# Tencent/PocketFlow

Hardware: AMD Instinct MI355X
Metric: images/sec ResNet-50 INT8 quant-aware fine-tune (whole job; per GPU = value / n_gpus) (higher is better)
Workload: dtype bf16

## Files before the change

include/pocketflow_hip.h:

```cpp
#ifndef POCKETFLOW_HIP_H_
#define POCKETFLOW_HIP_H_

#include <stdint.h>

#ifdef __cplusplus
extern "C" {
#endif

enum { PF_F32 = 0, PF_BF16 = 1 };
enum { PF_ACT_NONE = 0, PF_ACT_RELU = 1, PF_ACT_RELU6 = 2 };
enum { PF_BUCKET_TENSOR = 0, PF_BUCKET_CHANNEL = 1, PF_BUCKET_SPLIT = 2 };

typedef struct PfSeg {
  int64_t offset;
  int64_t len;
  int32_t RS;
  int32_t layout;
  int32_t I, O;
  int32_t mode;
  int32_t bits;
  int32_t bucket_size;
  int32_t n_bucket;
  int64_t slot_offset;
  int64_t cb_offset;
} PfSeg;

typedef struct PfBlock { int32_t seg; int32_t chunk; int32_t row0; int32_t nrows; } PfBlock;

#define PF_CHUNK 4096

const char* pf_error_string(int err);
int pf_version(void);
int pf_tuning_reload(void);

int pf_minmax_slots_init(uint32_t* slots, int64_t n_pairs, void* stream);
int pf_minmax_tensor(const void* x, int64_t n, int dtype, int act, uint32_t* slot, void* stream);
int pf_minmax_decode(const uint32_t* slots, int64_t n_pairs, float* alpha_beta, void* stream);

int pf_uq_apply(const void* x, void* y, int64_t n, int in_dtype, int out_dtype, int act,
                const uint32_t* slot, int bits, void* stream);
int pf_act_grad(const void* g, const void* u, void* dx, int64_t n, int dtype, int act,
                void* stream);

int pf_seg_minmax(const float* w_flat, const PfSeg* segs, const PfBlock* blocks, int n_blocks,
                  uint32_t* slots, void* stream);
int pf_seg_uq_apply(const float* w_flat, void* qw_flat, int out_dtype, const PfSeg* segs,
                    const PfBlock* blocks, int n_blocks, const uint32_t* slots, void* stream);

int pf_seg_nuq_apply(const float* w_flat, void* qw_flat, int out_dtype, uint8_t* idx_flat,
                     const float* codebooks, const PfSeg* segs, const PfBlock* blocks,
                     int n_blocks, const uint32_t* slots, void* stream);
int pf_seg_nuq_codebook_grad(const void* g_flat, int g_dtype, const uint8_t* idx_flat,
                             float* dcodebooks, int64_t* acc_ws, int64_t n_codebook, const PfSeg* segs,
                             const PfBlock* blocks, int n_blocks, const uint32_t* slots, void* stream);
int pf_seg_normalize(const float* w_flat, float* xn_out, const PfSeg* segs, int seg_index,
                     const uint32_t* slots, void* stream);

int pf_ws_bkup_merge_abs(const float* var, float* bkup, const float* mask, float* abs_out,
                         int64_t n, void* stream);
int pf_kth_largest_nonneg(const float* a, int64_t n, int64_t k_desc_index, float* out,
                          uint32_t* workspace, void* stream);
int pf_ws_mask_apply(float* var, const float* bkup, float* mask, const float* thr, int64_t n,
                     void* stream);
int pf_count_nonzero(const float* x, int64_t n, unsigned long long* out, void* stream);

int pf_cp_build_mask(float* mask, const uint8_t* keep_in, const uint8_t* keep_out, int O, int RS,
                     int I, void* stream);
int pf_cp_mask_grad(float* g, const uint8_t* keep_in, const uint8_t* keep_out, int O, int RS,
                    int I, void* stream);

int pf_adam_flat(float* p, const void* g, int g_dtype, float* m, float* v, const float* mask,
                 int64_t n, int64_t n_decay, float wd, float g_scale, float lr, float beta1,
                 float beta2, float eps, float beta1_power, float beta2_power, void* stream);
int pf_momentum_flat(float* p, const void* g, int g_dtype, float* acc, const float* mask,
                     int64_t n, int64_t n_decay, float wd, float g_scale, float lr, float momentum,
                     void* stream);
int pf_adam_flat_dev(float* p, const void* g, int g_dtype, float* m, float* v, const float* mask,
                     int64_t n, int64_t n_decay, float wd, float g_scale, const float* hp, float beta1,
                     float beta2, float eps, void* stream);
int pf_momentum_flat_dev(float* p, const void* g, int g_dtype, float* acc, const float* mask,
                         int64_t n, int64_t n_decay, float wd, float g_scale, const float* hp,
                         float momentum, void* stream);
int pf_set_floats(float* dst, float a, float b, float c, float d, void* stream);

int pf_ce_distill_fwd_bwd(const void* z_s, int zs_dtype, const float* labels, const void* z_t,
                          int zt_dtype, int B, int C, float tempr, float loss_w, float* losses,
                          void* dz_s, int dz_dtype, float* row_ws, void* stream);

int pf_bn_stats(const void* x, int dtype, int64_t rows, int C, float* partial ,
                int n_blocks, void* stream);
int pf_bn_finalize(const float* partial, int n_blocks, int64_t rows, int C, const void* x_row0,
                   int dtype, const float* gamma, const float* beta, float* moving_mean,
                   float* moving_var, float momentum, float eps, int training ,
                   int act, float* scale_shift , float* mean_invstd ,
                   uint32_t* slot , void* stream);
int pf_bn_act_quant_apply(const void* x, void* q, int dtype, int64_t rows, int C,
                          const float* scale_shift, int act, const uint32_t* slot, int bits,
                          int quantize, void* stream);
int pf_bn_bwd_stats(const void* dq, const void* x, int dtype, int64_t rows, int C,
                    const float* scale_shift, const float* mean_invstd, int act,
                    float* partial , int n_blocks, void* stream);
int pf_bn_bwd_finalize(const float* partial, int n_blocks, int C, float* dgamma, float* dbeta,
                       void* stream);
int pf_bn_bwd_apply(const void* dq, const void* x, void* dx, int dtype, int64_t rows, int C,
                    const float* scale_shift, const float* mean_invstd,
                    const float* dgamma, const float* dbeta, int act, void* stream);
int pf_bn_bwd_apply_add(const void* dq, const void* x, const void* addend, void* dx, int dtype,
                        int64_t rows, int C, const float* scale_shift, const float* mean_invstd,
                        const float* dgamma, const float* dbeta, int act, void* stream);
int pf_bn_eval_scale_shift(const float* gamma, const float* beta, const float* moving_mean,
                           const float* moving_var, float eps, int C, float* scale_shift,
                           void* stream);

int pf_conv1x1_stats_groups_k(int M, int N, int K, int prologue);
int pf_conv1x1_fwd(const void* X, const void* W, void* Y, const void* R, const float* scale_shift,
                   int act, const uint32_t* slot, int bits, float* partial, int M, int N, int K,
                   int Ho, int Wo, int H, int Wd, int stride, int ymap, void* stream);
int pf_conv1x1_fwd_affine(const void* X, const void* W, void* Y, const float* scale_shift, int act,
                          const float* out_scale_shift, int out_act, int M, int N, int K, int Ho, int Wo, int H, int Wd,
                          int stride, void* stream);
int pf_conv1x1_bwd_data_bnstats(const void* dY, const void* Wt, void* dQ, const void* bn_x,
                                const float* bn_scale_shift, const float* bn_mean_invstd, int bn_act,
                                float* partial, int M, int N, int K, void* stream);
int pf_conv1x1_join_plan(int M, int N, int K, int with_stats);
int pf_conv1x1_bwd_data_join(const void* dY, const void* Wt, void* dQ, const void* R, int r_Ho, int r_Wo, int r_H, int r_W,
                             int r_stride, const void* bn_x, const float* bn_scale_shift, const float* bn_mean_invstd,
                             int bn_act, float* partial, int M, int N, int K, void* stream);
int pf_conv1x1_wrw_splits(int M, int N, int K);
int pf_conv1x1_wrw(const void* dY, const void* X, void* dW, int dw_dtype, float* workspace,
                   const float* scale_shift, int act, const uint32_t* slot, int bits, int M, int N,
                   int K, int Ho, int Wo, int H, int Wd, int stride, void* stream);

int pf_conv2d_stats_groups_geom(int imgs, int H, int Wd, int C, int N, int th, int tw, int stride, int pad_h, int pad_w,
                                int Ho, int Wo);
int pf_conv2d_fwd(const void* X, const void* W, void* Y, const void* zero, const void* R, float* partial,
                  const void* bn_x, const float* bn_scale_shift, const float* bn_mean_invstd, int bn_act,
                  int imgs, int H, int Wd, int C, int N, int th, int tw, int stride, int pad_h, int pad_w,
                  int Ho, int Wo, void* stream);
int pf_conv2d_fwd_affine(const void* X, const void* W, void* Y, const void* zero, const float* out_scale_shift, int out_act,
                         int imgs, int H, int Wd, int C, int N, int th, int tw, int stride, int pad_h, int pad_w, int Ho, int Wo,
                         void* stream);

int pf_conv2d_wrw_splits(int M, int N, int C, int taps);
int pf_conv2d_wrw(const void* dY, const void* X, void* dW, int dw_dtype, float* workspace, int imgs, int H, int Wd, int C,
                  int N, int th, int tw, int stride, int pad_h, int pad_w, int Ho, int Wo, void* stream);

typedef struct PfTransposeTile {
  int64_t src_off, dst_off;
  int32_t O, I, src_ld, dst_ld;
  int32_t o0, i0;
  int32_t reserved0, reserved1;
} PfTransposeTile;
int pf_seg_transpose(const void* src_flat, void* dst_flat, int dtype, const void* tiles, int n_tiles, void* stream);

int pf_maxpool_fwd(const void* x, void* y, void* idx, int dtype, int B, int H, int W, int C, int k, int stride,
                   int pad_h, int pad_w, int Ho, int Wo, void* stream);
int pf_maxpool_bwd(const void* dy, const void* idx, void* dx, int dtype, int B, int H, int W, int C, int k, int stride,
                   int pad_h, int pad_w, int Ho, int Wo, void* stream);

int pf_conv_stem_supported(int H, int Wd, int C, int N, int k, int stride, int pad);
int pf_conv_stem_fwd(const void* X, const void* W, void* Y, int imgs, int H, int Wd, void* stream);
int pf_conv_stem_wrw_slabs(int imgs, int H, int Wd);
int pf_conv_stem_wrw(const void* dY, const void* X, void* dW, int dw_dtype, float* workspace, int imgs, int H, int Wd,
                     void* stream);

int pf_conv_stem3_supported(int H, int Wd, int C, int N, int k, int stride, int pad_h, int pad_w, int Ho, int Wo);
int pf_conv_stem3_fwd(const void* X, const void* W, void* Y, int imgs, int H, int Wd, int N, int pad_h, int pad_w, int Ho, int Wo,
                      void* stream);
int pf_conv_stem3_wrw_slabs(int imgs, int H, int Wd, int N, int pad_h, int pad_w, int Ho, int Wo);
int pf_conv_stem3_wrw(const void* dY, const void* X, void* dW, int dw_dtype, float* workspace, int imgs, int H, int Wd, int N,
                      int pad_h, int pad_w, int Ho, int Wo, void* stream);

int pf_depthwise_supported(int C, int k, int stride);
int pf_depthwise_groups(int B, int Ho, int Wo, int C);
int pf_depthwise_fwd(const void* X, const void* W, void* Y, int dtype, float* partial, int B, int H, int Wd, int C, int k,
                     int stride, int pad_h, int pad_w, int Ho, int Wo, void* stream);
int pf_depthwise_bwd_data(const void* dY, const void* W, void* dX, int dtype, int B, int H, int Wd, int C, int k,
                          int stride, int pad_h, int pad_w, int Ho, int Wo, void* stream);
int pf_depthwise_wrw(const void* dY, const void* X, void* dW, int dtype, int dw_dtype, float* slabs, int B, int H, int Wd,
                     int C, int k, int stride, int pad_h, int pad_w, int Ho, int Wo, void* stream);

typedef struct PfImageDesc {
  int64_t offset;
  int32_t h, w;
  float scale_y, scale_x;
  int32_t off_y, off_x;
  int32_t flip;
  int32_t reserved;
} PfImageDesc;
int pf_image_resize_bilinear(const void* src, const PfImageDesc* desc, void* out, int out_dtype, int B, int OH,
                             int OW, float mean_r, float mean_g, float mean_b, void* stream);

int pf_conv2d_bwd_data_strided(const void* dY, const void* Wt, void* dX, const void* zero, int imgs, int H, int Wd, int C, int N,
                               int R, int S, int stride, int pad_h, int pad_w, int Ho, int Wo, void* stream);
int pf_conv2d_bwd_data_strided_stats_groups(int imgs, int H, int Wd, int C, int stride);
int pf_conv2d_bwd_data_strided_bnstats(const void* dY, const void* Wt, void* dX, const void* zero, const void* bn_x,
                                       const float* bn_scale_shift, const float* bn_mean_invstd, int bn_act, float* partial,
                                       int imgs, int H, int Wd, int C, int N, int R, int S, int stride, int pad_h, int pad_w,
                                       int Ho, int Wo, void* stream);

int pf_convg_small_splits(int M, int Nc, int K);
int pf_convg_fwd(const void* x, const void* w, const float* bias, void* y, int dtype, int imgs, int H, int W, int C, int N, int R,
                 int S, int stride, int pad_h, int pad_w, int Ho, int Wo, float* slab, int64_t slab_elems, void* stream);
int pf_convg_bwd_data(const void* dy, const void* w, void* dx, int dtype, int imgs, int H, int W, int C, int N, int R, int S,
                      int stride, int pad_h, int pad_w, int Ho, int Wo, float* slab, int64_t slab_elems, void* stream);
int pf_convg_wrw_splits(int imgs, int C, int N, int R, int S, int Ho, int Wo);
int pf_convg_wrw(const void* dy, const void* x, void* dw, int dtype, int dw_dtype, float* slab, int imgs, int H, int W, int C, int N,
                 int R, int S, int stride, int pad_h, int pad_w, int Ho, int Wo, void* stream);

int pf_conv_gather_fwd(const void* x, const void* w, const int32_t* gather, const float* bias, const void* res,
                       const float* scale_shift, int act, void* y, int dtype, int imgs, int H, int W, int C, int Ck, int N, int R,
                       int S, int stride, int pad_h, int pad_w, int Ho, int Wo, void* stream);

int pf_im2col(const void* x, void* xcol, int imgs, int H, int W, int C, int R, int S, int stride, int pad_h, int pad_w, int Ho, int Wo,
              void* stream);
int pf_col2im(const void* dxcol, void* dx, int imgs, int H, int W, int C, int R, int S, int stride, int pad_h, int pad_w, int Ho, int Wo,
              void* stream);

int pf_prox_groups(int64_t rows, int I);
int pf_prox_norms(const float* w, const void* g, int g_dtype, float lr, int64_t rows, int I, float* partial, float* norms, void* stream);
int pf_prox_apply(float* w, const void* g, int g_dtype, float lr, int64_t rows, int I, const float* norms, const float* thr, void* stream);

int pf_cpr_gather(const void* x, int x_dtype, const void* y, int y_dtype, const int* pos, int crops, int B, int H, int W, int C, int OH, int OW,
                  int Co, int kh, int kw, int stride, int pad_t, int pad_l, float* P, float* Y, int64_t row0, void* stream);
int64_t pf_cpr_gram_ws(int C);
int pf_cpr_gram(const float* P, const float* Y, const int* idx, int64_t n, int kk, int C, int Co, const float* w, double* ws, int64_t ws_elems,
                float* xtx, float* xty, void* stream);
int pf_cpr_ista(const float* A, const float* b, const float* m0, float* m_ws, float* mask, int C, float gamma, float lr, int iters, int* nnz,
                void* stream);
int pf_cpr_lstsq_splits(int64_t N, int Kp, int Co);
int pf_cpr_lstsq_step(const float* P, int K, const int* kidx, const int* pos, int Kp, const float* Y, float* R, int64_t N, int Co, float* W,
                      float* m, float* v, float* part, float wd, float lr_t, float beta1, float beta2, float c1, float c2, float eps,
                      void* stream);
int pf_cpr_lstsq_resid(const float* P, int K, const int* kidx, int Kp, const float* W, const float* Y, float* R, int64_t N, int Co,
                       void* stream);

#ifdef __cplusplus
}
#endif
#endif
```

pocketflow_amd/csrc/pf_optim.hip:

```cpp
#include "pf_common.h"

template <typename TG> __device__ __forceinline__ void load4g(const TG* p, float* g);
template <> __device__ __forceinline__ void load4g<float>(const float* p, float* g) {
  float4 v = *reinterpret_cast<const float4*>(p);
  g[0] = v.x; g[1] = v.y; g[2] = v.z; g[3] = v.w;
}
template <> __device__ __forceinline__ void load4g<bf16_t>(const bf16_t* p, float* g) {
  uint2 v = *reinterpret_cast<const uint2*>(p);
  g[0] = __uint_as_float(v.x << 16); g[1] = __uint_as_float(v.x & 0xFFFF0000u);
  g[2] = __uint_as_float(v.y << 16); g[3] = __uint_as_float(v.y & 0xFFFF0000u);
}

__device__ __forceinline__ float eff_grad(float g, float p, float mask, bool decay, float wd,
                                          float g_scale) {
  float ge = g * g_scale;
  if (decay) ge = ge + wd * p;
  return ge * mask;
}

template <typename TG, bool MASK>
__global__ __launch_bounds__(PF_THREADS) void k_adam_flat(float* __restrict__ p, const TG* __restrict__ g,
                                                          float* __restrict__ m, float* __restrict__ v,
                                                          const float* __restrict__ mask, int64_t n,
                                                          int64_t n_decay, float wd, float g_scale,
                                                          float alpha_t, float omb1, float omb2,
                                                          float eps, const float* __restrict__ hp) {
  if (hp != nullptr) alpha_t = hp[0];
  const int64_t nv = n >> 2;
  for (int64_t i = (int64_t)blockIdx.x * PF_THREADS + threadIdx.x; i < nv;
       i += (int64_t)gridDim.x * PF_THREADS) {
    const int64_t e = i << 2;
    float gg[4], mk[4] = {1.f, 1.f, 1.f, 1.f};
    load4g<TG>(g + e, gg);
    float4 pp = *reinterpret_cast<float4*>(p + e);
    float4 mm = *reinterpret_cast<float4*>(m + e);
    float4 vv = *reinterpret_cast<float4*>(v + e);
    if (MASK) { float4 t = *reinterpret_cast<const float4*>(mask + e); mk[0] = t.x; mk[1] = t.y; mk[2] = t.z; mk[3] = t.w; }
    float pa[4] = {pp.x, pp.y, pp.z, pp.w}, ma[4] = {mm.x, mm.y, mm.z, mm.w}, va[4] = {vv.x, vv.y, vv.z, vv.w};
#pragma unroll
    for (int j = 0; j < 4; ++j) {
      const float ge = eff_grad(gg[j], pa[j], mk[j], (e + j) < n_decay, wd, g_scale);
      ma[j] = ma[j] + (ge - ma[j]) * omb1;
      va[j] = va[j] + (ge * ge - va[j]) * omb2;
      pa[j] = pa[j] - (ma[j] * alpha_t) / (sqrtf(va[j]) + eps);
    }
    *reinterpret_cast<float4*>(p + e) = make_float4(pa[0], pa[1], pa[2], pa[3]);
    *reinterpret_cast<float4*>(m + e) = make_float4(ma[0], ma[1], ma[2], ma[3]);
    *reinterpret_cast<float4*>(v + e) = make_float4(va[0], va[1], va[2], va[3]);
  }
  if (blockIdx.x == 0) {
    for (int64_t e = (nv << 2) + threadIdx.x; e < n; e += PF_THREADS) {
      const float mk = MASK ? mask[e] : 1.0f;
      const float ge = eff_grad(load_one<TG>(g + e), p[e], mk, e < n_decay, wd, g_scale);
      const float mn = m[e] + (ge - m[e]) * omb1;
      const float vn = v[e] + (ge * ge - v[e]) * omb2;
      m[e] = mn; v[e] = vn;
      p[e] = p[e] - (mn * alpha_t) / (sqrtf(vn) + eps);
    }
  }
}

static int adam_launch(float* p, const void* g, int g_dtype, float* m, float* v,
                       const float* mask, int64_t n, int64_t n_decay, float wd, float g_scale,
                       float lr, float beta1, float beta2, float eps, float beta1_power,
                       float beta2_power, const float* hp, void* stream) {
  if (n <= 0) return 0;
  if (!pf_aligned16(p) || !pf_aligned16(g) || !pf_aligned16(m) || !pf_aligned16(v) ||
      (mask && !pf_aligned16(mask)))
    return (int)hipErrorInvalidValue;
  const float alpha_t = lr * sqrtf(1.0f - beta2_power) / (1.0f - beta1_power);
  const float omb1 = 1.0f - beta1, omb2 = 1.0f - beta2;
  hipStream_t st = (hipStream_t)stream;
  const int grid = pf_grid_for(n, PF_THREADS * 4);
#define PF_AD(TG, MK) k_adam_flat<TG, MK><<<grid, PF_THREADS, 0, st>>>(p, (const TG*)g, m, v, mask, n, n_decay, wd, g_scale, alpha_t, omb1, omb2, eps, hp)
  if (g_dtype == PF_F32) { if (mask) PF_AD(float, true); else PF_AD(float, false); }
  else if (g_dtype == PF_BF16) { if (mask) PF_AD(bf16_t, true); else PF_AD(bf16_t, false); }
  else return (int)hipErrorInvalidValue;
#undef PF_AD
  PF_LAUNCH_CHECK();
  return 0;
}

extern "C" int pf_adam_flat(float* p, const void* g, int g_dtype, float* m, float* v,
                            const float* mask, int64_t n, int64_t n_decay, float wd, float g_scale,
                            float lr, float beta1, float beta2, float eps, float beta1_power,
                            float beta2_power, void* stream) {
  return adam_launch(p, g, g_dtype, m, v, mask, n, n_decay, wd, g_scale, lr, beta1, beta2, eps, beta1_power, beta2_power, nullptr,
                     stream);
}

extern "C" int pf_adam_flat_dev(float* p, const void* g, int g_dtype, float* m, float* v,
                                const float* mask, int64_t n, int64_t n_decay, float wd, float g_scale,
                                const float* hp, float beta1, float beta2, float eps, void* stream) {
  if (hp == nullptr) return (int)hipErrorInvalidValue;
  return adam_launch(p, g, g_dtype, m, v, mask, n, n_decay, wd, g_scale, 0.f, beta1, beta2, eps, 0.5f, 0.5f, hp, stream);
}

template <typename TG, bool MASK>
__global__ __launch_bounds__(PF_THREADS) void k_momentum_flat(float* __restrict__ p, const TG* __restrict__ g,
                                                              float* __restrict__ acc,
                                                              const float* __restrict__ mask, int64_t n,
                                                              int64_t n_decay, float wd, float g_scale,
                                                              float lr, float mu, const float* __restrict__ hp) {
  if (hp != nullptr) lr = hp[1];
  const int64_t nv = n >> 2;
  for (int64_t i = (int64_t)blockIdx.x * PF_THREADS + threadIdx.x; i < nv;
       i += (int64_t)gridDim.x * PF_THREADS) {
    const int64_t e = i << 2;
    float gg[4], mk[4] = {1.f, 1.f, 1.f, 1.f};
    load4g<TG>(g + e, gg);
    float4 pp = *reinterpret_cast<float4*>(p + e);
    float4 aa = *reinterpret_cast<float4*>(acc + e);
    if (MASK) { float4 t = *reinterpret_cast<const float4*>(mask + e); mk[0] = t.x; mk[1] = t.y; mk[2] = t.z; mk[3] = t.w; }
    float pa[4] = {pp.x, pp.y, pp.z, pp.w}, ac[4] = {aa.x, aa.y, aa.z, aa.w};
#pragma unroll
    for (int j = 0; j < 4; ++j) {
      const float ge = eff_grad(gg[j], pa[j], mk[j], (e + j) < n_decay, wd, g_scale);
      ac[j] = mu * ac[j] + ge;
      pa[j] = pa[j] - lr * ac[j];
    }
    *reinterpret_cast<float4*>(p + e) = make_float4(pa[0], pa[1], pa[2], pa[3]);
    *reinterpret_cast<float4*>(acc + e) = make_float4(ac[0], ac[1], ac[2], ac[3]);
  }
  if (blockIdx.x == 0) {
    for (int64_t e = (nv << 2) + threadIdx.x; e < n; e += PF_THREADS) {
      const float mk = MASK ? mask[e] : 1.0f;
      const float ge = eff_grad(load_one<TG>(g + e), p[e], mk, e < n_decay, wd, g_scale);
      const float a = mu * acc[e] + ge;
      acc[e] = a;
      p[e] = p[e] - lr * a;
    }
  }
}

static int momentum_launch(float* p, const void* g, int g_dtype, float* acc, const float* mask,
                           int64_t n, int64_t n_decay, float wd, float g_scale, float lr,
                           float momentum, const float* hp, void* stream) {
  if (n <= 0) return 0;
  if (!pf_aligned16(p) || !pf_aligned16(g) || !pf_aligned16(acc) || (mask && !pf_aligned16(mask)))
    return (int)hipErrorInvalidValue;
  hipStream_t st = (hipStream_t)stream;
  const int grid = pf_grid_for(n, PF_THREADS * 4);
#define PF_MO(TG, MK) k_momentum_flat<TG, MK><<<grid, PF_THREADS, 0, st>>>(p, (const TG*)g, acc, mask, n, n_decay, wd, g_scale, lr, momentum, hp)
  if (g_dtype == PF_F32) { if (mask) PF_MO(float, true); else PF_MO(float, false); }
  else if (g_dtype == PF_BF16) { if (mask) PF_MO(bf16_t, true); else PF_MO(bf16_t, false); }
  else return (int)hipErrorInvalidValue;
#undef PF_MO
  PF_LAUNCH_CHECK();
  return 0;
}

extern "C" int pf_momentum_flat(float* p, const void* g, int g_dtype, float* acc, const float* mask,
                                int64_t n, int64_t n_decay, float wd, float g_scale, float lr,
                                float momentum, void* stream) {
  return momentum_launch(p, g, g_dtype, acc, mask, n, n_decay, wd, g_scale, lr, momentum, nullptr, stream);
}

extern "C" int pf_momentum_flat_dev(float* p, const void* g, int g_dtype, float* acc, const float* mask,
                                    int64_t n, int64_t n_decay, float wd, float g_scale, const float* hp,
                                    float momentum, void* stream) {
  if (hp == nullptr) return (int)hipErrorInvalidValue;
  return momentum_launch(p, g, g_dtype, acc, mask, n, n_decay, wd, g_scale, 0.f, momentum, hp, stream);
}

__global__ void k_set_floats(float* __restrict__ dst, float a, float b, float c, float d) {
  if (threadIdx.x == 0) { dst[0] = a; dst[1] = b; dst[2] = c; dst[3] = d; }
}

extern "C" int pf_set_floats(float* dst, float a, float b, float c, float d, void* stream) {
  if (dst == nullptr) return (int)hipErrorInvalidValue;
  k_set_floats<<<1, 64, 0, (hipStream_t)stream>>>(dst, a, b, c, d);
  PF_LAUNCH_CHECK();
  return 0;
}
```

pocketflow_amd/csrc/pf_stem.hip:

```cpp
#include "pf_conv_common.h"

#define LDS_PTR(p) ((__attribute__((address_space(3))) void*)(p))
typedef short st_v4s __attribute__((ext_vector_type(4)));
typedef short st_v8s __attribute__((ext_vector_type(8)));
#if defined(__HIP_DEVICE_COMPILE__)
typedef __amdgpu_buffer_rsrc_t st_rsrc_t;
#define ST_MAKE_RSRC(p, bytes) __builtin_amdgcn_make_buffer_rsrc((void*)(p), (short)0, (int)(bytes), 0x00020000)
#define ST_BUFFER_LOAD_LDS16(rs, lds, voff) __builtin_amdgcn_raw_ptr_buffer_load_lds(rs, LDS_PTR(lds), 16, voff, 0, 0, 0)
#else
typedef int st_rsrc_t;
#define ST_MAKE_RSRC(p, bytes) 0
#define ST_BUFFER_LOAD_LDS16(rs, lds, voff) ((void)(rs), (void)(lds), (void)(voff))
#endif

#define ST_THREADS 256
#define ST_OROWS 8
#define ST_IROWS (2 * ST_OROWS + 5)
#define ST_N 64
#define ST_R 7
#define ST_WL_BYTES (ST_N * ST_R * 32 * 2)

struct StemArgs {
  const bf16_t* X;
  const bf16_t* W;
  bf16_t* Y;
  int imgs, H, Wd, Ho, Wo;
  int strips, n_items;
  int rsb;
};

__global__ __launch_bounds__(ST_THREADS) void k_stem7x7_fwd(StemArgs a) {
  extern __shared__ __attribute__((aligned(16))) unsigned char smem[];
  unsigned char* wl = smem;
  unsigned char* xs = smem + ST_WL_BYTES;
  const int tid = threadIdx.x, lane = tid & 63, wave = __builtin_amdgcn_readfirstlane(tid >> 6);
  const int l16 = lane & 15, g = lane >> 4;

  for (int ch = tid; ch < ST_N * ST_R * 4; ch += ST_THREADS) {
    const int q = ch & 3, nr = ch >> 2;
    const bf16_t* src = a.W + ((int64_t)nr * 7 + 2 * q) * 3;
    uint32_t v[4];
    const uint32_t e0 = src[0], e1 = src[1], e2 = src[2];
    v[0] = e0 | (e1 << 16); v[1] = e2;
    if (q < 3) {
      const uint32_t f0 = src[3], f1 = src[4], f2 = src[5];
      v[2] = f0 | (f1 << 16); v[3] = f2;
    } else {
      v[2] = 0u; v[3] = 0u;
    }
    *reinterpret_cast<uint4*>(wl + ((int64_t)nr * 32 + q * 8) * 2) = make_uint4(v[0], v[1], v[2], v[3]);
  }
  for (int t = tid; t < ST_IROWS * 8; t += ST_THREADS) {
    const int row = t >> 3, h = t & 7;
    const int pp = h < 3 ? h : a.Wd + h;
    *reinterpret_cast<uint2*>(xs + (int64_t)row * a.rsb + pp * 8) = make_uint2(0u, 0u);
  }
  __syncthreads();
  bf16x8 wf[4][ST_R];
#pragma unroll
  for (int nb = 0; nb < 4; ++nb) {
    const int n = 16 * (l16 >> 2) + 4 * nb + (l16 & 3);
#pragma unroll
    for (int r = 0; r < ST_R; ++r)
      wf[nb][r] = *reinterpret_cast<const bf16x8*>(wl + ((n * ST_R + r) * 32 + g * 8) * 2);
  }

  const int pairs = a.Wd >> 1;
  const int pblocks = a.Wo >> 4;
  const int units = ST_OROWS * pblocks;
  for (int item = blockIdx.x; item < a.n_items; item += gridDim.x) {
    const int img = item / a.strips, strip = item - img * a.strips;
    const int oy0 = strip * ST_OROWS, iy0 = 2 * oy0 - 3;
    __syncthreads();
    for (int row = tid >> 7; row < ST_IROWS; row += 2) {
      const int iy = iy0 + row;
      unsigned char* dst = xs + (int64_t)row * a.rsb + 3 * 8;
      const bool live = iy >= 0 && iy < a.H;
      const uint32_t* src = reinterpret_cast<const uint32_t*>(a.X + ((int64_t)img * a.H + (live ? iy : 0)) * a.Wd * 3);
      for (int j = tid & 127; j < pairs; j += 128) {
        uint32_t d0 = 0u, d1 = 0u, d2 = 0u;
        if (live) { d0 = src[3 * j]; d1 = src[3 * j + 1]; d2 = src[3 * j + 2]; }
        *reinterpret_cast<uint2*>(dst + j * 16) = make_uint2(d0, d1 & 0xFFFFu);
        *reinterpret_cast<uint2*>(dst + j * 16 + 8) = make_uint2((d1 >> 16) | (d2 << 16), d2 >> 16);
      }
    }
    __syncthreads();
    for (int u = wave; u < units; u += ST_THREADS / 64) {
      const int orow = u / pblocks, pb = u - orow * pblocks;
      const int oy = oy0 + orow;
      if (oy >= a.Ho) continue;
      const int ox = pb * 16 + l16;
      const unsigned char* base = xs + (int64_t)(2 * orow) * a.rsb + (2 * ox + 2 * g) * 8;
      f32x4 acc[4];
#pragma unroll
      for (int nb = 0; nb < 4; ++nb) acc[nb] = f32x4{0.f, 0.f, 0.f, 0.f};
#pragma unroll
      for (int r = 0; r < ST_R; ++r) {
        const bf16x8 xf = *reinterpret_cast<const bf16x8*>(base + (int64_t)r * a.rsb);
#pragma unroll
        for (int nb = 0; nb < 4; ++nb)
          acc[nb] = __builtin_amdgcn_mfma_f32_16x16x32_bf16(wf[nb][r], xf, acc[nb], 0, 0, 0);
      }
      bf16_t* out = a.Y + (((int64_t)img * a.Ho + oy) * a.Wo + ox) * ST_N + 16 * g;
      const uint4 lo = make_uint4(pack_bf16x2(acc[0][0], acc[0][1]), pack_bf16x2(acc[0][2], acc[0][3]),
                                  pack_bf16x2(acc[1][0], acc[1][1]), pack_bf16x2(acc[1][2], acc[1][3]));
      const uint4 hi = make_uint4(pack_bf16x2(acc[2][0], acc[2][1]), pack_bf16x2(acc[2][2], acc[2][3]),
                                  pack_bf16x2(acc[3][0], acc[3][1]), pack_bf16x2(acc[3][2], acc[3][3]));
      *reinterpret_cast<uint4*>(out) = lo;
      *reinterpret_cast<uint4*>(out + 8) = hi;
    }
  }
}

extern "C" int pf_conv_stem_supported(int H, int Wd, int C, int N, int k, int stride, int pad) {
  return (C == 3 && N == ST_N && k == 7 && stride == 2 && pad == 3 && H > 0 && (H % 2) == 0 && Wd >= 32 && (Wd % 32) == 0 &&
          Wd <= 1024) ? 1 : 0;
}

extern "C" int pf_conv_stem_fwd(const void* X, const void* W, void* Y, int imgs, int H, int Wd, void* stream) {
  if (!pf_conv_stem_supported(H, Wd, 3, ST_N, 7, 2, 3) || imgs <= 0) return (int)hipErrorInvalidValue;
  if (!pf_aligned16(Y) || (reinterpret_cast<uintptr_t>(X) & 3u) || (reinterpret_cast<uintptr_t>(W) & 1u))
    return (int)hipErrorInvalidValue;
  StemArgs a;
  a.X = (const bf16_t*)X; a.W = (const bf16_t*)W; a.Y = (bf16_t*)Y;
  a.imgs = imgs; a.H = H; a.Wd = Wd; a.Ho = H / 2; a.Wo = Wd / 2;
  a.strips = (a.Ho + ST_OROWS - 1) / ST_OROWS;
  a.n_items = imgs * a.strips;
  a.rsb = (Wd + 8) * 8;
  const size_t lds = (size_t)ST_WL_BYTES + (size_t)ST_IROWS * a.rsb;
  if (lds > 160 * 1024) return (int)hipErrorInvalidValue;
  if (int e = pf_require_lds(reinterpret_cast<const void*>(&k_stem7x7_fwd), lds)) return e;
  const int grid = a.n_items < 512 ? a.n_items : 512;
  k_stem7x7_fwd<<<grid, ST_THREADS, lds, (hipStream_t)stream>>>(a);
  PF_LAUNCH_CHECK();
  return 0;
}


struct StemWrwArgs {
  const bf16_t* dY;
  const bf16_t* X;
  float* slabs;
  int imgs, H, Wd, Ho, Wo;
  int strips, n_items;
  int rsb;
  int dy_bytes;
};

#define SW_OROWS 2
#define SW_IROWS (2 * SW_OROWS + 5)

__global__ __launch_bounds__(ST_THREADS) void k_stem7x7_wrw(StemWrwArgs a) {
  extern __shared__ __attribute__((aligned(16))) unsigned char smem[];
  unsigned char* xs = smem;
  unsigned char* dys = smem + SW_IROWS * a.rsb;
  const int tid = threadIdx.x, lane = tid & 63, wave = __builtin_amdgcn_readfirstlane(tid >> 6);
  const int l15 = lane & 15, q = lane >> 4;
  const int nb0 = 2 * (wave & 1);
  const int r0 = (wave >> 1) ? 4 : 0, nr = (wave >> 1) ? 3 : 4;
  const st_rsrc_t rsY = ST_MAKE_RSRC(a.dY, a.dy_bytes);
  constexpr uint32_t OOB = 0x80000000u;
  const int sb = lane >> 4, srow = (lane & 15) >> 1, sch = lane & 1;
  const int tr_off = (q & 1) * 128 + (l15 >> 2) * 32 + (l15 & 3) * 8;
  const int pg_lo = q >> 1;
  const int p_lo = 8 * pg_lo + 4 * (q & 1) + (l15 >> 2);
  const int steps = (SW_OROWS * a.Wo) >> 5;
  const int pairs = a.Wd >> 1;

  f32x4 acc[2][8];
#pragma unroll
  for (int i = 0; i < 2; ++i)
#pragma unroll
    for (int k = 0; k < 8; ++k) acc[i][k] = f32x4{0.f, 0.f, 0.f, 0.f};

  for (int t = tid; t < SW_IROWS * 8; t += ST_THREADS) {
    const int row = t >> 3, h = t & 7;
    const int pp = h < 3 ? h : a.Wd + h;
    *reinterpret_cast<uint2*>(xs + (int64_t)row * a.rsb + pp * 8) = make_uint2(0u, 0u);
  }

  for (int item = blockIdx.x; item < a.n_items; item += gridDim.x) {
    const int img = item / a.strips, strip = item - img * a.strips;
    const int oy0 = strip * SW_OROWS, iy0 = 2 * oy0 - 3;
    const int valid_px = ((a.Ho - oy0) < SW_OROWS ? (a.Ho - oy0) : SW_OROWS) * a.Wo;
    const int64_t m_base = ((int64_t)img * a.Ho + oy0) * a.Wo;
    __syncthreads();
    for (int id = wave; id < steps * 4; id += ST_THREADS / 64) {
      const int lin = id * 8 + srow;
      const uint32_t voff = (lin < valid_px) ? (uint32_t)(((m_base + lin) * ST_N + 16 * sb + 8 * sch) * 2) : OOB;
      ST_BUFFER_LOAD_LDS16(rsY, dys + id * 1024, voff);
    }
    for (int row = tid >> 7; row < SW_IROWS; row += 2) {
      const int iy = iy0 + row;
      unsigned char* dst = xs + (int64_t)row * a.rsb + 3 * 8;
      const bool live = iy >= 0 && iy < a.H;
      const uint32_t* src = reinterpret_cast<const uint32_t*>(a.X + ((int64_t)img * a.H + (live ? iy : 0)) * a.Wd * 3);
      for (int j = tid & 127; j < pairs; j += 128) {
        uint32_t d0 = 0u, d1 = 0u, d2 = 0u;
        if (live) { d0 = src[3 * j]; d1 = src[3 * j + 1]; d2 = src[3 * j + 2]; }
        *reinterpret_cast<uint2*>(dst + j * 16) = make_uint2(d0, d1 & 0xFFFFu);
        *reinterpret_cast<uint2*>(dst + j * 16 + 8) = make_uint2((d1 >> 16) | (d2 << 16), d2 >> 16);
      }
    }
    asm volatile("s_waitcnt vmcnt(0)" ::: "memory");
    __syncthreads();
    for (int st = 0; st < steps; ++st) {
      const unsigned char* dbase = dys + st * 4096;
      bf16x8 df[2];
#pragma unroll
      for (int i = 0; i < 2; ++i) {
        const st_v4s lo = __builtin_amdgcn_ds_read_tr16_b64_v4i16(
            (__attribute__((address_space(3))) st_v4s*)(dbase + (pg_lo * 4 + nb0 + i) * 256 + tr_off));
        const st_v4s hi = __builtin_amdgcn_ds_read_tr16_b64_v4i16(
            (__attribute__((address_space(3))) st_v4s*)(dbase + ((pg_lo + 2) * 4 + nb0 + i) * 256 + tr_off));
        st_v8s d8;
        d8[0] = lo[0]; d8[1] = lo[1]; d8[2] = lo[2]; d8[3] = lo[3];
        d8[4] = hi[0]; d8[5] = hi[1]; d8[6] = hi[2]; d8[7] = hi[3];
        df[i] = *reinterpret_cast<const bf16x8*>(&d8);
      }
      int lin = st * 32 + p_lo;
      int orow = lin >= a.Wo ? 1 : 0;
      const unsigned char* xlo = xs + (int64_t)(2 * orow + r0) * a.rsb + (2 * (lin - orow * a.Wo) + (l15 & 3)) * 8;
      lin += 16;
      orow = lin >= a.Wo ? 1 : 0;
      const unsigned char* xhi = xs + (int64_t)(2 * orow + r0) * a.rsb + (2 * (lin - orow * a.Wo) + (l15 & 3)) * 8;
#pragma unroll
      for (int rr = 0; rr < 4; ++rr) {
        if (rr < nr) {
#pragma unroll
          for (int h = 0; h < 2; ++h) {
            const st_v4s lo = __builtin_amdgcn_ds_read_tr16_b64_v4i16(
                (__attribute__((address_space(3))) st_v4s*)(xlo + (int64_t)rr * a.rsb + h * 32));
            const st_v4s hi = __builtin_amdgcn_ds_read_tr16_b64_v4i16(
                (__attribute__((address_space(3))) st_v4s*)(xhi + (int64_t)rr * a.rsb + h * 32));
            st_v8s x8;
            x8[0] = lo[0]; x8[1] = lo[1]; x8[2] = lo[2]; x8[3] = lo[3];
            x8[4] = hi[0]; x8[5] = hi[1]; x8[6] = hi[2]; x8[7] = hi[3];
            const bf16x8 xf = *reinterpret_cast<const bf16x8*>(&x8);
#pragma unroll
            for (int i = 0; i < 2; ++i)
              acc[i][rr * 2 + h] = __builtin_amdgcn_mfma_f32_16x16x32_bf16(df[i], xf, acc[i][rr * 2 + h], 0, 0, 0);
          }
        }
      }
    }
  }
  float* slab = a.slabs + (int64_t)blockIdx.x * (ST_N * 147);
  const int c = l15 & 3;
#pragma unroll
  for (int rr = 0; rr < 4; ++rr) {
    if (rr < nr) {
#pragma unroll
      for (int h = 0; h < 2; ++h) {
        const int s = 4 * h + (l15 >> 2);
        if (s < 7 && c < 3) {
#pragma unroll
          for (int i = 0; i < 2; ++i)
#pragma unroll
            for (int j = 0; j < 4; ++j)
              slab[(16 * (nb0 + i) + 4 * q + j) * 147 + ((r0 + rr) * 7 + s) * 3 + c] = acc[i][rr * 2 + h][j];
        }
      }
    }
  }
}

int pf_wrw_reduce(float* workspace, int S, int64_t n, void* dW, int dw_dtype, hipStream_t st);

static int stem_wrw_grid(int imgs, int H) {
  const int items = imgs * ((H / 2 + SW_OROWS - 1) / SW_OROWS);
  return items < 768 ? items : 768;
}

extern "C" int pf_conv_stem_wrw_slabs(int imgs, int H, int Wd) {
  if (!pf_conv_stem_supported(H, Wd, 3, ST_N, 7, 2, 3) || imgs <= 0 || Wd > 256) return 0;
  if ((int64_t)imgs * (H / 2) * (Wd / 2) * ST_N * 2 >= (int64_t)1 << 31) return 0;
  return stem_wrw_grid(imgs, H);
}

extern "C" int pf_conv_stem_wrw(const void* dY, const void* X, void* dW, int dw_dtype, float* workspace, int imgs, int H,
                                int Wd, void* stream) {
  const int S = pf_conv_stem_wrw_slabs(imgs, H, Wd);
  if (S <= 0 || workspace == nullptr) return (int)hipErrorInvalidValue;
  if (!pf_aligned16(dY) || (reinterpret_cast<uintptr_t>(X) & 3u)) return (int)hipErrorInvalidValue;
  StemWrwArgs a;
  a.dY = (const bf16_t*)dY; a.X = (const bf16_t*)X; a.slabs = workspace;
  a.imgs = imgs; a.H = H; a.Wd = Wd; a.Ho = H / 2; a.Wo = Wd / 2;
  a.strips = (a.Ho + SW_OROWS - 1) / SW_OROWS;
  a.n_items = imgs * a.strips;
  a.rsb = (Wd + 8) * 8;
  a.dy_bytes = (int)((int64_t)imgs * a.Ho * a.Wo * ST_N * 2);
  const size_t lds = (size_t)SW_IROWS * a.rsb + (size_t)SW_OROWS * a.Wo * ST_N * 2;
  if (int e = pf_require_lds(reinterpret_cast<const void*>(&k_stem7x7_wrw), lds)) return e;
  k_stem7x7_wrw<<<S, ST_THREADS, lds, (hipStream_t)stream>>>(a);
  PF_LAUNCH_CHECK();
  return pf_wrw_reduce(workspace, S, (int64_t)ST_N * 147, dW, dw_dtype, (hipStream_t)stream);
}
```

pocketflow_amd/graph.py:

```python
from __future__ import annotations

import contextlib
import math
import os
import weakref
import threading
from dataclasses import dataclass, field
from typing import Callable, Dict, List, Optional, Sequence, Tuple

import numpy as np
import torch
import torch.nn.functional as F

from pocketflow_amd import hip
from pocketflow_amd.hip import check_gather
from pocketflow_amd.plan import WeightDesc
from pocketflow_amd.profiling import region

ALIGN = 64
FUSE_BN_BWD_STATS = os.environ.get('PF_FUSE_BN_BWD_STATS', '1') != '0'


def _align(n: int) -> int:
  return (n + ALIGN - 1) // ALIGN * ALIGN
# ... 566 lines not shown


class LazyAct(object):

  def __init__(self, x, scale_shift, act, slot, bits, rows, C, mean_invstd=None):
    self.x, self.scale_shift, self.act, self.slot, self.bits = x, scale_shift, act, slot, bits
    self.rows, self.C = rows, C
    self.mean_invstd = mean_invstd
    self.n_consumers = 0
    self.bwd_stats = None
    self.n_grad_consumers = 0
    self.pending = None
    self.join_ok = False
    self.pending_geom = None
    self.dense_out = None
    self._q = None

  @property
  def shape(self):
    return self.x.shape

  @property
  def dtype(self):
    return self.x.dtype

  @property
  def device(self):
    return self.x.device

  def materialize(self) -> torch.Tensor:
    self.n_consumers += 2
    if self._q is None:
      self._q = _Materialize.apply(self.x, self)
    return self._q


def materialize(x):
  return x.materialize() if isinstance(x, LazyAct) else x


class _Materialize(torch.autograd.Function):
  @staticmethod
  def forward(ctx, x, lazy):
    q = torch.empty_like(x)
    quant = lazy.bits is not None
    hip.bn_act_quant_apply(x, q, lazy.rows, lazy.C, lazy.scale_shift, lazy.act, lazy.slot if quant else None,
                           lazy.bits if quant else 8, quant)
    return q

  @staticmethod
  def backward(ctx, dq):
    return dq, None


def _bn_statistics(x, rows, C, graph, st=None):
  if st is not None:
    partial, nblk = st
    return partial, nblk, graph.zero_row(C)
  nblk = _bn_blocks(rows, C)
  partial = graph.scratch(nblk * 4 * C)
  with region('bn_stats', float(x.numel() * x.element_size())):
    hip.bn_stats(x, rows, C, partial, nblk)
  return partial, nblk, x


class _BnLazy(torch.autograd.Function):

  @staticmethod
  def forward(ctx, x, gamma, beta, layer, graph, slot, bits, box, stats):
    C = gamma.numel()
    rows = x.numel() // C
    partial, nblk, piv = _bn_statistics(x, rows, C, graph, stats)
    scale_shift = torch.empty((2, C), dtype=torch.float32, device=x.device)
    mean_invstd = torch.empty((2, C), dtype=torch.float32, device=x.device)
    hip.bn_finalize(partial, nblk, rows, C, piv, gamma, beta, layer.moving_mean.tensor, layer.moving_var.tensor,
                    layer.momentum, layer.eps, True, layer.act, scale_shift, mean_invstd,
                    slot if bits is not None else None)
    ctx.save_for_backward(x, scale_shift, mean_invstd)
    ctx.meta = (layer.act, graph, rows, C)
    ctx.params = (gamma, beta)
    ctx.box = box
    ctx.set_materialize_grads(False)
    box.append(scale_shift)
    box.append(mean_invstd)
    return x.view_as(x), x.view_as(x)

  @staticmethod
  def backward(ctx, dq, dskip):
    x, scale_shift, mean_invstd = ctx.saved_tensors
    act, graph, rows, C = ctx.meta
    if dq is None:
      return dskip, None, None, None, None, None, None, None, None
    pre = None
    lazy = ctx.box[2]() if len(ctx.box) > 2 else None
    if lazy is not None and lazy.bwd_stats is not None and lazy.bwd_stats[2] == dq.data_ptr():
      pre = lazy.bwd_stats[:2]
    dx, dgamma, dbeta = _bn_backward(dq, x, scale_shift, mean_invstd, act, graph, rows, C, addend=dskip,
                                     params=ctx.params, pre=pre)
    return dx, dgamma, dbeta, None, None, None, None, None, None


def _grad_view(t: Optional[torch.Tensor], n: int):
  g = getattr(t, 'grad', None) if t is not None else None
  if g is not None and g.dtype == torch.float32 and g.is_contiguous() and g.numel() == n:
    return g
  return None


def _bn_backward(dq, x, scale_shift, mean_invstd, act, graph, rows, C, addend=None, params=None, pre=None,
                 frozen=False):
  dq = _nhwc(dq)
  if dq.dtype != x.dtype:
    dq = dq.to(x.dtype)
  if addend is not None:
    addend = _nhwc(addend)
    if addend.dtype != x.dtype:
      addend = addend.to(x.dtype)
  nbytes = float(x.numel() * x.element_size())
  if pre is not None:
    partial, nblk = pre
  else:
    nblk = _bn_blocks(rows, C)
    partial = graph.scratch(nblk * 2 * C)
    with region('bn_bwd_stats', 2 * nbytes):
      hip.bn_bwd_stats(dq, x, rows, C, scale_shift, mean_invstd, act, partial, nblk)
  gview = _grad_view(params[0], C) if params is not None else None
  bview = _grad_view(params[1], C) if params is not None else None
  direct = gview is not None and bview is not None
  dgamma = gview if direct else torch.empty(C, dtype=torch.float32, device=x.device)
  dbeta = bview if direct else torch.empty(C, dtype=torch.float32, device=x.device)
  hip.bn_bwd_finalize(partial, nblk, C, dgamma, dbeta)
  dx = torch.empty_like(x)
  with region('bn_bwd_apply', (4 if addend is not None else 3) * nbytes):
    zero = graph.zero_row(C)[:C] if frozen else None
    hip.bn_bwd_apply(dq, x, dx, rows, C, scale_shift, mean_invstd, zero if frozen else dgamma,
                     zero if frozen else dbeta, act, addend)
  return (dx, None, None) if direct else (dx, dgamma, dbeta)


def _filter_grad(graph, w, w_var, keep, name, nbytes, launch):
  gw = getattr(w, 'grad', None)
  direct = gw is not None and gw.shape == w.shape and gw.dtype == w.dtype and gw.permute(0, 2, 3, 1).is_contiguous()
  target = (gw.permute(0, 2, 3, 1) if direct
            else torch.empty((w.shape[0], w.shape[2], w.shape[3], w.shape[1]), dtype=w.dtype, device=w.device))
  with _wrw_queue(graph, direct, *keep) as scratch, region(name, nbytes):
    launch(target, scratch)
    if direct:
      graph.store.notify_grad(w_var)
  return None if direct else target.permute(0, 3, 1, 2)


def _bwd_data_weight(graph, w_var, w):
  if USE_SEG_TRANSPOSE and w_var is not None and w_var.store is graph.store and w_var.tensor is w:
    return graph.store.transposed(w_var)
  return w.detach().permute(0, 2, 3, 1).flip(1, 2).permute(3, 1, 2, 0).contiguous()


def _krsc(w, dtype):
  wk = w.detach().permute(0, 2, 3, 1)
  if not wk.is_contiguous() or wk.dtype != dtype:
    wk = wk.contiguous().to(dtype)
  return wk


def _out_size(size: int, k: int, stride: int, pad_total: int) -> int:
  return (size + pad_total - k) // stride + 1


def _apply_with_stats(fn, *args):
  box = []
  y = fn.apply(*args, box)
  if box[0] is not None:
    y._pf_stats = box[0]
  return y


def _conv1x1_geom(x_shape, stride):
  n, _, h, w = x_shape
  if stride == 1:
    return n * h * w, None, (h, w)
  ho, wo = -(-h // stride), -(-w // stride)
  return n * ho * wo, (ho, wo, h, w, stride), (ho, wo)


def _run_conv1x1(x, w2d, lazy, residual, want_stats, stride, out_bn=None):
  N, K = w2d.shape
  M, geom, (ho, wo) = _conv1x1_geom(x.shape, stride)
  y = torch.empty((x.shape[0], N, ho, wo), dtype=x.dtype, device=x.device, memory_format=torch.channels_last)
  if out_bn is not None:
    with region('conv1x1_fwd', float((M * K + M * N) * 2)):
      hip.conv1x1_fwd(x, w2d, y, M, N, K, scale_shift=lazy.scale_shift if lazy is not None else None,
                      act=lazy.act if lazy is not None else None, geom=geom, out_scale_shift=out_bn._eval_scale_shift(y),
                      out_act=out_bn.act)
    y._pf_bn_done = out_bn
    return y
  partial, G = None, 0
  if want_stats:
    G = hip.conv1x1_stats_groups(M, N, K, prologue=lazy is not None)
    partial = torch.empty((G, 4, N), dtype=torch.float32, device=x.device)
  ss = lazy.scale_shift if lazy is not None else None
  quant = lazy is not None and lazy.bits is not None
  nbytes = float((M * K + M * N * (2 if residual is not None else 1)) * 2)
  with region('conv1x1_fwd', nbytes):
    hip.conv1x1_fwd(x, w2d, y, M, N, K, R=residual, scale_shift=ss, act=lazy.act if lazy is not None else None,
                    slot=lazy.slot if quant else None, bits=lazy.bits if quant else 8, partial=partial, geom=geom)
  if want_stats:
    y._pf_stats = (partial, G)
  return y


class _FusedConv1x1(torch.autograd.Function):

  @staticmethod
  def forward(ctx, x, w, residual, lazy, want_stats, stride, graph, w_var, box):
    w2d = w.detach().permute(0, 2, 3, 1).reshape(w.shape[0], w.shape[1])
    res = _nhwc(residual) if residual is not None else None
    y = _run_conv1x1(x, w2d, lazy, res, want_stats, stride)
    ctx.save_for_backward(x, w2d)
    ctx.meta = (lazy, stride, graph, residual is not None, w.shape)
    ctx.w_leaf = w
    ctx.w_var = w_var
    box.append(getattr(y, '_pf_stats', None))
    return y

  @staticmethod
  def backward(ctx, dy):
    x, w2d = ctx.saved_tensors
    lazy, stride, graph, has_res, w_shape = ctx.meta
    dy = _nhwc(dy)
    N, K = w2d.shape
    M, geom, _ = _conv1x1_geom(x.shape, stride)
    ss = lazy.scale_shift if lazy is not None else None
    quant = lazy is not None and lazy.bits is not None
    act = lazy.act if lazy is not None else None
    dx = dw = None
    if ctx.needs_input_grad[1]:
      S = hip.conv1x1_wrw_splits(M, N, K)

      def wrw(dwk, scratch):
        hip.conv1x1_wrw(dy, x, dwk.view(N, K), scratch((S + 32) * N * K), M, N, K, scale_shift=ss, act=act,
                        slot=lazy.slot if quant else None, bits=lazy.bits if quant else 8, geom=geom)
      dw = _filter_grad(graph, ctx.w_leaf, ctx.w_var, (dy, x, w2d, ss, lazy), 'conv1x1_wrw', float((M * K + M * N) * 2), wrw)
    if ctx.needs_input_grad[0]:
      wt = _bwd_data_weight(graph, ctx.w_var, ctx.w_leaf).view(K, N)
      fuse_stats = (FUSE_BN_BWD_STATS and lazy is not None and lazy.n_consumers == 1 and geom is None
                    and lazy.mean_invstd is not None and lazy.act in ('Relu', 'Relu6'))
      join = (JOIN_TWO_CONSUMERS and lazy is not None and lazy.join_ok and lazy.n_consumers == 2
              and lazy.n_grad_consumers == 2)
      second = join and lazy.pending is not None
      res = lazy.pending if (second and geom is None) else None
      join_entry = getattr(hip, 'conv1x1_bwd_data_join', None) if PROJ_JOIN else None
      compact = (join and not second and geom is not None and join_entry is not None and lazy.dense_out is not None
                 and hip.conv1x1_join_plan(x.shape[0] * x.shape[2] * x.shape[3], lazy.dense_out, K) != 0)
      rgeom = lazy.pending_geom if res is not None else None
      join_stats = (res is not None and join_entry is not None and PROJ_JOIN_STATS and FUSE_BN_BWD_STATS
                    and lazy.mean_invstd is not None and lazy.act in ('Relu', 'Relu6')
                    and hip.conv1x1_join_plan(M, N, K, True) != 0)
      if compact:
        dx = torch.empty((x.shape[0], K, geom[0], geom[1]), dtype=x.dtype, device=x.device, memory_format=torch.channels_last)
      elif geom is None:
        dx = torch.empty_like(x)
      else:
        dx = torch.zeros_like(x)
      with region('conv1x1_bwd_data', float((M * K * (2 if (fuse_stats or res is not None) else 1) + M * N) * 2)):
        if compact:
          hip.conv1x1_fwd(dy, wt, dx, M, K, N)
        elif join_stats:
          G = hip.conv1x1_stats_groups(M, K, N)
          partial = torch.empty((G, 2, K), dtype=torch.float32, device=x.device)
          join_entry(dy, wt, dx, res, M, N, K, rgeom=rgeom, bn_x=x, bn_scale_shift=lazy.scale_shift,
                     bn_mean_invstd=lazy.mean_invstd, bn_act=lazy.act, partial=partial)
          lazy.bwd_stats = (partial, G, dx.data_ptr())
        elif rgeom is not None:
          join_entry(dy, wt, dx, res, M, N, K, rgeom=rgeom)
        elif fuse_stats:
          G = hip.conv1x1_stats_groups(M, K, N)
          partial = torch.empty((G, 2, K), dtype=torch.float32, device=x.device)
          hip.conv1x1_bwd_data_bnstats(dy, wt, dx, x, lazy.scale_shift, lazy.mean_invstd, lazy.act, partial, M, N, K)
          lazy.bwd_stats = (partial, G, dx.data_ptr())
        elif res is not None:
          hip.conv1x1_fwd(dy, wt, dx, M, K, N, R=res)
        else:
          hip.conv1x1_fwd(dy, wt, dx, M, K, N, geom=geom, ymap=geom is not None)
      if join:
        if not second:
          lazy.pending, dx = dx, None
          lazy.pending_geom = geom if compact else None
        else:
          if res is None:
            dx = dx + lazy.pending
          lazy.pending = lazy.pending_geom = None
    return dx, dw, (dy if has_res else None), None, None, None, None, None, None


JOIN_TWO_CONSUMERS = os.environ.get('PF_JOIN_TWO_CONSUMERS', '1') != '0'
PROJ_JOIN = os.environ.get('PF_PROJ_JOIN', '1') != '0'
PROJ_JOIN_STATS = os.environ.get('PF_PROJ_JOIN_STATS', '1') != '0'
USE_SEG_TRANSPOSE = os.environ.get('PF_SEG_TRANSPOSE', '1') != '0'
OWN_POOL = os.environ.get('PF_OWN_POOL', '1') != '0'
OWN_CONV2D_WRW = os.environ.get('PF_OWN_CONV2D_WRW', '1') != '0'
OWN_CONV2D_WRW_MIN_C = int(os.environ.get('PF_OWN_CONV2D_WRW_MIN_C', '64'))
OWN_CONV2D_BWD_STRIDED = os.environ.get('PF_OWN_CONV2D_BWD_STRIDED', '1') != '0'
OWN_CONV2D = os.environ.get('PF_OWN_CONV2D', '1') != '0'
OWN_STEM = os.environ.get('PF_OWN_STEM', '1') != '0'
OWN_DEPTHWISE = os.environ.get('PF_OWN_DEPTHWISE', '1') != '0'
OWN_CONV_IM2COL = os.environ.get('PF_OWN_CONV_IM2COL', '1') != '0'
CONVG_BF16_NARROW = os.environ.get('PF_CONVG_BF16_NARROW', '0') != '0'
FOLD_EVAL_BN = os.environ.get('PF_FOLD_EVAL_BN', '1') != '0'
OWN_CONV_GENERIC = os.environ.get('PF_OWN_CONV_GENERIC', '1') != '0'
DEPTHWISE_ANY_DEVICE = False


def _run_conv2d(x, w_krsc, stride, pad, want_stats, out_bn=None):
  B, C, H, W = x.shape
  N, R, S, _ = w_krsc.shape
  Ho, Wo = _out_size(H, R, stride, 2 * pad[0]), _out_size(W, S, stride, 2 * pad[1])
  y = torch.empty((B, N, Ho, Wo), dtype=x.dtype, device=x.device, memory_format=torch.channels_last)
  M = B * Ho * Wo
  if out_bn is not None:
    with region('conv2d_fwd', float((B * H * W * C + M * N) * 2)):
      hip.conv2d_fwd(x, w_krsc, y, B, H, W, C, N, R, S, stride, pad[0], pad[1], Ho, Wo,
                     out_scale_shift=out_bn._eval_scale_shift(y), out_act=out_bn.act)
    y._pf_bn_done = out_bn
    return y
  partial, G = None, 0
  if want_stats:
    G = hip.conv2d_stats_groups(M, N, geom=(B, H, W, C, N, R, S, stride, pad[0], pad[1], Ho, Wo))
    partial = torch.empty((G, 4, N), dtype=torch.float32, device=x.device)
  with region('conv2d_fwd', float((B * H * W * C + M * N) * 2)):
    hip.conv2d_fwd(x, w_krsc, y, B, H, W, C, N, R, S, stride, pad[0], pad[1], Ho, Wo, partial=partial)
  if want_stats:
    y._pf_stats = (partial, G)
  return y


class _Conv2dIgemm(torch.autograd.Function):

  @staticmethod
  def forward(ctx, x, w, stride, pad, want_stats, graph, bn_box, w_var, box):
    ctx.w_var = w_var
    w_krsc = w.detach().permute(0, 2, 3, 1)
    y = _run_conv2d(x, w_krsc, stride, pad, want_stats)
    ctx.save_for_backward(x, w)
    ctx.meta = (stride, pad, graph, bn_box)
    box.append(getattr(y, '_pf_stats', None))
    return y

  @staticmethod
  def backward(ctx, dy):
    x, w = ctx.saved_tensors
    stride, pad, graph, bn_box = ctx.meta
    dy = _nhwc(dy)
    dx = dw = None
    N, C, R, S = w.shape
    B, _, H, W = x.shape
    Ho, Wo = dy.shape[2], dy.shape[3]
    if ctx.needs_input_grad[1]:
      splits = hip.conv2d_wrw_splits(B * Ho * Wo, N, C, R * S) if (OWN_CONV2D_WRW and C >= OWN_CONV2D_WRW_MIN_C) else 0
      nbytes = float((x.numel() + dy.numel()) * 2)
      if splits > 0:
        def wrw(dwk, scratch):
          hip.conv2d_wrw(dy, x, dwk, scratch((splits + 32) * N * R * S * C), B, H, W, C, N, R, S, stride, pad[0], pad[1], Ho, Wo)
        dw = _filter_grad(graph, w, ctx.w_var, (dy, x), 'conv2d_wrw', nbytes, wrw)
      elif OWN_CONV2D_WRW and OWN_CONV_GENERIC and x.is_cuda and dy.dtype == x.dtype and w.dtype == x.dtype:
        gs = hip.convg_wrw_splits(B, C, N, R, S, Ho, Wo)
        dwk = torch.empty((N, R, S, C), dtype=w.dtype, device=x.device)
        with region('conv2d_wrw', nbytes):
          hip.convg_wrw(dy, x, dwk, graph.scratch(gs * N * R * S * C), B, H, W, C, N, R, S, stride, pad[0], pad[1], Ho, Wo)
        dw = dwk.permute(0, 3, 1, 2)
      else:
        with region('conv2d_wrw', nbytes):
          dw = torch.ops.aten.convolution_backward(dy, x, w.detach(), None, [stride, stride], list(pad), [1, 1], False,
                                                   [0, 0], 1, [False, True, False])[1]
    if ctx.needs_input_grad[0]:
      mfma = N % 64 == 0 and C % 8 == 0 and igemm_limits_ok(dy.numel(), w.numel(), R * S)
      by_classes = (OWN_CONV2D_BWD_STRIDED and stride > 1 and H % stride == 0 and W % stride == 0 and R >= stride and S >= stride
                    and dy.dtype == torch.bfloat16)
      if mfma and (stride == 1 or by_classes):
        wb = _bwd_data_weight(graph, ctx.w_var, w)
        dx = torch.empty_like(x)
        fuse = (FUSE_BN_BWD_STATS and bn_box is not None and bn_box.get('n_consumers') == 1
                and bn_box.get('act') in ('Relu', 'Relu6') and bn_box['x'].shape == x.shape)
        with region('conv2d_bwd_data', float((dy.numel() + x.numel() * (2 if fuse else 1)) * 2)):
          bn = {}
          if fuse:
            G = (hip.conv2d_stats_groups(B * H * W, C, geom=(B, H, W, N, C, R, S, 1, R - 1 - pad[0], S - 1 - pad[1], H, W))
                 if stride == 1 else hip.conv2d_bwd_data_strided_stats_groups(B, H, W, C, stride))
            partial = torch.empty((G, 2, C), dtype=torch.float32, device=x.device)
            bn = dict(partial=partial, bn_x=bn_box['x'], bn_scale_shift=bn_box['scale_shift'], bn_mean_invstd=bn_box['mean_invstd'],
                      bn_act=bn_box['act'])
          if stride == 1:
            hip.conv2d_fwd(dy, wb, dx, B, H, W, N, C, R, S, 1, R - 1 - pad[0], S - 1 - pad[1], H, W, **bn)
          else:
            hip.conv2d_bwd_data_strided(dy, wb, dx, B, H, W, C, N, R, S, stride, pad[0], pad[1], Ho, Wo, **bn)
          if fuse:
            bn_box['bwd_stats'] = (partial, G, dx.data_ptr())
      elif OWN_CONV2D and OWN_CONV_GENERIC and x.is_cuda and dy.dtype == x.dtype and w.dtype == x.dtype:
        dx = torch.empty_like(x)
        with region('conv2d_bwd_data', float((dy.numel() + x.numel()) * 2)):
          hip.convg_bwd_data(dy, _krsc(w, x.dtype), dx, B, H, W, C, N, R, S, stride, pad[0], pad[1], Ho, Wo,
                             slab=_convg_slab(graph, x.dtype, B * H * W, C, R * S * N))
      else:
        with region('conv2d_bwd_data', float((dy.numel() + x.numel()) * 2)):
          dx = torch.ops.aten.convolution_backward(dy, x, w.detach(), None, [stride, stride], list(pad), [1, 1], False,
                                                   [0, 0], 1, [True, False, False])[0]
    return dx, dw, None, None, None, None, None, None, None


class _ConvGeneric(torch.autograd.Function):

  @staticmethod
  def forward(ctx, x, w, bias, stride, pad, out_hw, graph):
    B, C, H, Wd = x.shape
    N, _, R, S = w.shape
    Ho, Wo = out_hw
    wk = _krsc(w, x.dtype)
    y = torch.empty((B, N, Ho, Wo), dtype=x.dtype, device=x.device, memory_format=torch.channels_last)
    bf = None if bias is None else bias.detach().float().contiguous()
    with region('convg_fwd', float((x.numel() + y.numel()) * x.element_size())):
      hip.convg_fwd(x, wk, bf, y, B, H, Wd, C, N, R, S, stride, pad[0], pad[1], Ho, Wo,
                    slab=_convg_slab(graph, x.dtype, B * Ho * Wo, N, R * S * C))
    ctx.save_for_backward(x, w)
    ctx.meta = (stride, pad, out_hw, graph, bias is not None)
    return y

  @staticmethod
  def backward(ctx, dy):
    x, w = ctx.saved_tensors
    stride, pad, (Ho, Wo), graph, has_bias = ctx.meta
    B, C, H, Wd = x.shape
    N, _, R, S = w.shape
    dy = _nhwc(dy)
    if dy.dtype != x.dtype:
      dy = dy.to(x.dtype)
    dx = dw = db = None
    if ctx.needs_input_grad[0]:
      wk = _krsc(w, x.dtype)
      dx = torch.empty_like(x, memory_format=torch.channels_last)
      with region('convg_bwd_data', float((dy.numel() + dx.numel()) * x.element_size())):
        hip.convg_bwd_data(dy, wk, dx, B, H, Wd, C, N, R, S, stride, pad[0], pad[1], Ho, Wo,
                           slab=_convg_slab(graph, x.dtype, B * H * Wd, C, R * S * N))
    if ctx.needs_input_grad[1]:
      splits = hip.convg_wrw_splits(B, C, N, R, S, Ho, Wo)
      dwk = torch.empty((N, R, S, C), dtype=w.dtype, device=x.device)
      with region('convg_wrw', float((dy.numel() + x.numel()) * x.element_size())):
        hip.convg_wrw(dy, x, dwk, graph.scratch(splits * N * R * S * C), B, H, Wd, C, N, R, S, stride, pad[0], pad[1], Ho, Wo)
      dw = dwk.permute(0, 3, 1, 2)
    if has_bias and ctx.needs_input_grad[2]:
      db = dy.float().sum(dim=(0, 2, 3))
    return dx, dw, db, None, None, None, None


def _convg_slab(graph, dtype, M: int, Nc: int, K: int):
  if dtype != torch.bfloat16:
    return None
  splits = hip.convg_small_splits(M, Nc, K)
  return graph.scratch(splits * M * Nc) if splits > 0 else None


def convg_ok(x: torch.Tensor, w: torch.Tensor, dense: bool = False) -> bool:
  if not (OWN_CONV_GENERIC and isinstance(x, torch.Tensor) and x.is_cuda and x.dtype in (torch.float32, torch.bfloat16)
          and w.dtype in (torch.float32, torch.bfloat16) and x.numel() > 0):
    return False
  return (x.dtype == torch.float32 or dense or x.shape[1] % 8 != 0 or CONVG_BF16_NARROW
          or (x.dim() == 4 and x.shape[2] * x.shape[3] == 1))


def conv_generic(x, w, bias, stride, pad_begin, out_hw, graph):
  return _ConvGeneric.apply(_nhwc(x), w, bias, stride, pad_begin, out_hw, graph)


class _ConvIm2col(torch.autograd.Function):

  @staticmethod
  def forward(ctx, x, w, stride, pad, out_hw, graph, w_var):
    B, C, H, Wd = x.shape
    N, _, R, S = w.shape
    Ho, Wo = out_hw
    M, K = B * Ho * Wo, R * S * C
    w2d = w.detach().permute(0, 2, 3, 1).reshape(N, K)
    xcol = torch.empty((M, K), dtype=x.dtype, device=x.device)
    y = torch.empty((B, N, Ho, Wo), dtype=x.dtype, device=x.device, memory_format=torch.channels_last)
    with region('conv_im2col_fwd', float((x.numel() + 2 * xcol.numel() + y.numel()) * 2)):
      hip.im2col(x, xcol, B, H, Wd, C, R, S, stride, pad[0], pad[1], Ho, Wo)
      hip.conv1x1_fwd(xcol, w2d, y, M, N, K)
    ctx.save_for_backward(x, w)
    ctx.meta = (stride, pad, out_hw, graph, w_var)
    return y

  @staticmethod
  def backward(ctx, dy):
    x, w = ctx.saved_tensors
    stride, pad, (Ho, Wo), graph, w_var = ctx.meta
    B, C, H, Wd = x.shape
    N, _, R, S = w.shape
    M, K = B * Ho * Wo, R * S * C
    dy = _nhwc(dy)
    dx = dw = None
    w2d = w.detach().permute(0, 2, 3, 1).reshape(N, K)
    if ctx.needs_input_grad[1]:
      xcol = torch.empty((M, K), dtype=x.dtype, device=x.device)
      hip.im2col(x, xcol, B, H, Wd, C, R, S, stride, pad[0], pad[1], Ho, Wo)
      splits = hip.conv1x1_wrw_splits(M, N, K)

      def wrw(dwk, scratch):
        hip.conv1x1_wrw(dy, xcol, dwk.view(N, K), scratch((splits + 32) * N * K), M, N, K)
      dw = _filter_grad(graph, w, w_var, (dy, xcol), 'conv_im2col_wrw', float((M * K + M * N) * 2), wrw)
    if ctx.needs_input_grad[0]:
      dxcol = torch.empty((M, K), dtype=x.dtype, device=x.device)
      dx = torch.empty_like(x)
      with region('conv_im2col_bwd_data', float((dy.numel() + 2 * dxcol.numel() + dx.numel()) * 2)):
        hip.conv1x1_fwd(dy, w2d.t().contiguous(), dxcol, M, K, N)
        hip.col2im(dxcol, dx, B, H, Wd, C, R, S, stride, pad[0], pad[1], Ho, Wo)
    return dx, dw, None, None, None, None, None


def im2col_conv_ok(x, conv, pad) -> bool:
  kh, kw, cin, cout = conv.kernel.ref_shape
  return (OWN_CONV_IM2COL and conv.k > 1 and conv.bias is None and isinstance(x, torch.Tensor) and fusable_tensor(x) and x.dim() == 4
          and cin % 8 == 0 and cin % 64 != 0 and cout % 8 == 0 and conv.graph.fuse_conv1x1
          and x.shape[0] * x.shape[2] * x.shape[3] * kh * kw * cin < (1 << 31))


def _run_stem(x, w):
  B, _, H, Wd = x.shape
  y = torch.empty((B, w.shape[0], H // 2, Wd // 2), dtype=x.dtype, device=x.device, memory_format=torch.channels_last)
  with region('conv_stem_fwd', float((x.numel() + y.numel()) * 2)):
    hip.conv_stem_fwd(x, w.detach().permute(0, 2, 3, 1), y, B, H, Wd)
  return y


class _StemConv(torch.autograd.Function):

  @staticmethod
  def forward(ctx, x, w, graph, w_var):
    ctx.save_for_backward(x, w)
    ctx.meta = (graph, w_var)
    return _run_stem(x, w)

  @staticmethod
  def backward(ctx, dy):
    x, w = ctx.saved_tensors
    graph, w_var = ctx.meta
    dy = _nhwc(dy)
    dx = dw = None
    if ctx.needs_input_grad[1]:
      B, _, H, Wd = x.shape
      S = hip.conv_stem_wrw_slabs(B, H, Wd) if OWN_CONV2D_WRW else 0
      nbytes = float((x.numel() + dy.numel()) * 2)
      if S > 0:
        def wrw(dwk, scratch):
          hip.conv_stem_wrw(dy, x, dwk, scratch((S + 32) * 64 * 147), B, H, Wd)
        dw = _filter_grad(graph, w, w_var, (dy, x), 'conv_stem_wrw', nbytes, wrw)
      else:
        with region('conv_stem_wrw', nbytes):
          dw = torch.ops.aten.convolution_backward(dy, x, w.detach(), None, [2, 2], [3, 3], [1, 1], False, [0, 0], 1,
                                                   [False, True, False])[1]
    if ctx.needs_input_grad[0]:
      dx = torch.ops.aten.convolution_backward(dy, x, w.detach(), None, [2, 2], [3, 3], [1, 1], False, [0, 0], 1,
                                               [True, False, False])[0]
    return dx, dw, None, None


def _run_stem3(x, w, pads, out_hw):
  B, _, H, Wd = x.shape
  N = w.shape[0]
  Ho, Wo = out_hw
  y = torch.empty((B, N, Ho, Wo), dtype=x.dtype, device=x.device, memory_format=torch.channels_last)
  with region('conv_stem_fwd', float((x.numel() + y.numel()) * 2)):
    hip.conv_stem3_fwd(x, w.detach().permute(0, 2, 3, 1), y, B, H, Wd, N, pads[0], pads[1], Ho, Wo)
  return y


class _Stem3Conv(torch.autograd.Function):

  @staticmethod
  def forward(ctx, x, w, graph, w_var, pads, out_hw):
    ctx.save_for_backward(x, w)
    ctx.meta = (graph, w_var, pads, out_hw)
    return _run_stem3(x, w, pads, out_hw)

  @staticmethod
  def backward(ctx, dy):
    x, w = ctx.saved_tensors
    graph, w_var, pads, (Ho, Wo) = ctx.meta
    dy = _nhwc(dy)
    dw = None
    if ctx.needs_input_grad[1]:
      B, _, H, Wd = x.shape
      N = w.shape[0]
      S = hip.conv_stem3_wrw_slabs(B, H, Wd, N, pads[0], pads[1], Ho, Wo)
      if S <= 0:
        raise RuntimeError('pf_conv_stem3_wrw does not take the shape its forward kernel took')

      def wrw(dwk, scratch):
        hip.conv_stem3_wrw(dy, x, dwk, scratch((S + 32) * N * 27), B, H, Wd, N, pads[0], pads[1], Ho, Wo)
      dw = _filter_grad(graph, w, w_var, (dy, x), 'conv_stem_wrw', float((x.numel() + dy.numel()) * 2), wrw)
    if ctx.needs_input_grad[0]:
      raise RuntimeError('the MobileNet stem kernels compute no image gradient')
    return None, dw, None, None, None, None


def own_stem3_ok(x, conv, front_pads, out_hw) -> bool:
  return (OWN_STEM and conv.bias is None and isinstance(x, torch.Tensor) and fusable_tensor(x) and x.dim() == 4 and conv.k == 3
          and conv.graph.fuse_conv1x1 and not x.requires_grad and x.is_contiguous(memory_format=torch.channels_last)
          and hip.conv_stem3_supported(x.shape[2], x.shape[3], x.shape[1], conv.kernel.ref_shape[3], conv.k, conv.stride,
                                       front_pads[0], front_pads[1], out_hw[0], out_hw[1])
          and hip.conv_stem3_wrw_slabs(x.shape[0], x.shape[2], x.shape[3], conv.kernel.ref_shape[3], front_pads[0], front_pads[1],
                                       out_hw[0], out_hw[1]) > 0)


def own_stem_ok(x, conv, pad) -> bool:
  return (OWN_STEM and conv.bias is None and isinstance(x, torch.Tensor) and fusable_tensor(x) and x.dim() == 4
          and pad[0] == pad[1] and conv.graph.fuse_conv1x1
          and x.is_contiguous(memory_format=torch.channels_last)
          and hip.conv_stem_supported(x.shape[2], x.shape[3], x.shape[1], conv.kernel.ref_shape[3], conv.k, conv.stride, pad[0]))


def igemm_limits_ok(n_in_elems: int, n_kernel_elems: int, taps: int) -> bool:
  return n_in_elems < (1 << 30) and n_kernel_elems < (1 << 30) and taps <= 32


def own_conv2d_ok(x, conv, pad) -> bool:
  kh, kw, cin, cout = conv.kernel.ref_shape
  return (OWN_CONV2D and conv.k > 1 and conv.bias is None and isinstance(x, torch.Tensor) and fusable_tensor(x)
          and x.dim() == 4 and cin % 64 == 0 and cout % 8 == 0
          and conv.graph.fuse_conv1x1 and igemm_limits_ok(x.numel(), kh * kw * cin * cout, kh * kw))


def fusable_tensor(t: torch.Tensor) -> bool:
  return t.is_cuda and t.dtype == torch.bfloat16


def fused_conv1x1_ok(x, conv) -> bool:
  t = x.x if isinstance(x, LazyAct) else x
  return (conv.k == 1 and conv.bias is None and fusable_tensor(t) and t.dim() == 4
          and conv.kernel.ref_shape[2] % 8 == 0 and conv.kernel.ref_shape[3] % 8 == 0
          and conv.padding in ('SAME', 'VALID', 0) and conv.graph.fuse_conv1x1)



def _same_pads(size: int, k: int, stride: int) -> Tuple[int, int]:
  out = -(-size // stride)
  total = max((out - 1) * stride + k - size, 0)
  return total // 2, total - total // 2


def _symmetric_pads(x: torch.Tensor, ph: Tuple[int, int], pw: Tuple[int, int]):
  if ph[0] == ph[1] and pw[0] == pw[1]:
    return x, (ph[0], pw[0])
  return F.pad(x, (pw[0], pw[1], ph[0], ph[1])), (0, 0)


def variance_scaling_init(ref_shape, fan_in: int):
  std = math.sqrt(1.0 / max(1.0, fan_in)) / .87962566103423978

  def init(rng: np.random.RandomState):
    from scipy.stats import truncnorm
    return truncnorm.rvs(-2, 2, size=ref_shape, random_state=rng).astype(np.float32) * np.float32(std)
  return init


def glorot_uniform_init(ref_shape, fan_in: int, fan_out: int):
  limit = math.sqrt(6.0 / (fan_in + fan_out))
  return lambda rng: rng.uniform(-limit, limit, size=ref_shape).astype(np.float32)


def truncated_normal_init(ref_shape, stddev: float):
  def init(rng: np.random.RandomState):
    from scipy.stats import truncnorm
    return truncnorm.rvs(-2, 2, size=ref_shape, random_state=rng).astype(np.float32) * np.float32(stddev)
  return init


def constant_init(ref_shape, value: float):
  return lambda rng: np.full(ref_shape, value, dtype=np.float32)


GATHER_MAX_CIN = 8192


def gather_pays(k: int, cin: int, kept: int, cout: int, dtype) -> bool:
  return False


class Conv2D:

  def __init__(self, graph: Graph, name: str, cin: int, cout: int, k: int, stride: int = 1,
               padding: str = 'SAME', use_bias: bool = False, kernel_name: str = 'kernel',
               bias_name: str = 'bias', init=None, l2: bool = True):
    self.graph, self.k, self.stride, self.padding = graph, k, stride, padding
    ref_shape = (k, k, cin, cout)
    init = init or variance_scaling_init(ref_shape, k * k * cin)
    self.kernel = graph.store.add(name + '/' + kernel_name, ref_shape, 'conv', True, l2, init)
    self.bias = (graph.store.add(name + '/' + bias_name, (cout,), 'bias', True, l2, constant_init((cout,), 0.0))
                 if use_bias else None)
    self.op = graph.add_matmul_op('Conv2D', name + '/Conv2D', self.kernel)

  def __call__(self, x, residual: Optional[torch.Tensor] = None, want_stats: bool = False, out_bn=None) -> torch.Tensor:
    w = self.kernel.tensor
    if out_bn is not None and (residual is not None or not out_bn.folds_into_producer()):
      out_bn = None
    if self.graph.taps is not None:
      return _tapped(self, materialize(x), residual)
    if self.kernel.gather_host is not None:
      return self._call_gathered(x, residual, out_bn)
    if fused_conv1x1_ok(x, self):
      lazy = x if isinstance(x, LazyAct) else None
      if lazy is not None:
        lazy.n_consumers += 1
      elif getattr(x, '_pf_bn', None) is not None:
        x._pf_bn['n_consumers'] += 2
      xin = lazy.x if lazy is not None else _nhwc(x)
      if torch.is_grad_enabled() and (xin.requires_grad or w.requires_grad):
        if lazy is not None and xin.requires_grad:
          lazy.n_grad_consumers += 1
          if self.stride == 1:
            lazy.dense_out = int(w.shape[0])
        return _apply_with_stats(_FusedConv1x1, xin, w, residual, lazy, want_stats, self.stride, self.graph, self.kernel)
      w2d = w.detach().permute(0, 2, 3, 1).reshape(w.shape[0], w.shape[1])
      return _run_conv1x1(xin, w2d, lazy, _nhwc(residual) if residual is not None else None, want_stats,
                          self.stride, out_bn=out_bn)
    x = materialize(x)
    b = self.bias.tensor.to(x.dtype) if self.bias is not None else None
    ph, pw, out_hw = self._geometry(x)
    if (self.padding == 'SAME' and residual is None and x.shape[1] == 3 and self.k == 3 and self.stride == 2
        and own_stem3_ok(x, self, (ph[0], pw[0]), out_hw)):
      if torch.is_grad_enabled() and w.requires_grad:
        return _Stem3Conv.apply(x, w, self.graph, self.kernel, (ph[0], pw[0]), out_hw)
      return _run_stem3(x, w, (ph[0], pw[0]), out_hw)
    x, pad = _symmetric_pads(x, ph, pw)
    if residual is None and own_stem_ok(x, self, pad):
      if torch.is_grad_enabled() and (x.requires_grad or w.requires_grad):
        return _StemConv.apply(x, w, self.graph, self.kernel)
      return _run_stem(x, w)
    if own_conv2d_ok(x, self, pad):
      bn_box = getattr(x, '_pf_bn', None)
      if bn_box is not None:
        bn_box['n_consumers'] += 1
      xin = _nhwc(x)
      if torch.is_grad_enabled() and (xin.requires_grad or w.requires_grad):
        y = _apply_with_stats(_Conv2dIgemm, xin, w, self.stride, pad, want_stats, self.graph, bn_box, self.kernel)
      else:
        y = _run_conv2d(xin, w.detach().permute(0, 2, 3, 1), self.stride, pad, want_stats, out_bn=out_bn)
      return y if residual is None else y + residual
    bn_box = getattr(x, '_pf_bn', None)
    if bn_box is not None:
      bn_box['n_consumers'] += 2
    if im2col_conv_ok(x, self, pad):
      y = _ConvIm2col.apply(_nhwc(x), w, self.stride, pad, out_hw, self.graph, self.kernel)
    elif convg_ok(x, w):
      y = conv_generic(x, w, self.bias.tensor if self.bias is not None else None, self.stride, pad, out_hw, self.graph)
    else:
      y = F.conv2d(x, w, b, stride=self.stride, padding=pad)
    return y if residual is None else y + residual

  def _geometry(self, x):
    ph = pw = (0, 0)
    if isinstance(self.padding, int):
      ph = pw = (self.padding, self.padding)
    elif self.padding == 'SAME' and self.k > 1:
      ph = _same_pads(x.shape[2], self.k, self.stride)
      pw = _same_pads(x.shape[3], self.k, self.stride)
    return ph, pw, (_out_size(x.shape[2], self.k, self.stride, ph[0] + ph[1]),
                    _out_size(x.shape[3], self.k, self.stride, pw[0] + pw[1]))

  def _call_gathered(self, x, residual, out_bn) -> torch.Tensor:
    var = self.kernel
    w = var.tensor
    x = materialize(x)
    if torch.is_grad_enabled() and (w.requires_grad or x.requires_grad):
      raise RuntimeError('%s: a shrunk (channel-gathered) convolution runs in inference only: call it under torch.no_grad() '
                         'on a graph finalised with requires_grad=False' % var.name)
    if x.dim() != 4 or x.shape[1] != var.cin_full:
      raise ValueError('%s: input of shape %s, the layer has %d input channels' % (var.name, tuple(x.shape), var.cin_full))
    ph, pw, (Ho, Wo) = self._geometry(x)
    x, pad = _symmetric_pads(x, ph, pw)
    x = _nhwc(x)
    B, C, H, Wd = x.shape
    N = w.shape[0]
    wk = _krsc(w, x.dtype)
    y = torch.empty((B, N, Ho, Wo), dtype=x.dtype, device=x.device, memory_format=torch.channels_last)
    bias = None if self.bias is None else self.bias.tensor.detach().float().contiguous()
    res = None if residual is None else _nhwc(residual).to(x.dtype)
    ss = out_bn._eval_scale_shift(y) if out_bn is not None else None
    with region('conv_gather_fwd', float((x.numel() + y.numel() * (2 if res is not None else 1)) * x.element_size())):
      hip.conv_gather_fwd(x, wk, var.gather, y, B, H, Wd, C, N, self.k, self.k, self.stride, pad[0], pad[1], Ho, Wo,
                          bias=bias, residual=res, scale_shift=ss, act=out_bn.act if out_bn is not None else None)
    if out_bn is not None:
      y._pf_bn_done = out_bn
    return y

  def plain(self, x: torch.Tensor) -> torch.Tensor:
    taps, self.graph.taps = self.graph.taps, None
    fuse, self.graph.fuse_conv1x1 = self.graph.fuse_conv1x1, False
    try:
      return self(x)
    finally:
      self.graph.taps, self.graph.fuse_conv1x1 = taps, fuse


class TapStop(Exception):
  """Raised by the tap of `graph.tap_stop`: the caller only needed the network up to that layer."""


def _tapped(layer, x, residual=None):
  g = layer.graph
  y = layer.plain(x)
  y_add = None if residual is None else y + residual
  g.taps[layer] = (x, y, getattr(x, '_pf_src', None), y_add, residual)
  if g.tap_stop is layer:
    raise TapStop()
  y._pf_src = layer
  return y if residual is None else y_add


def _pass_tag(x, y):
  src = getattr(x, '_pf_src', None)
  if src is not None:
    y._pf_src = src
  return y


def _run_depthwise(x, w, stride, ph, pw, Ho, Wo, want_stats):
  B, C, H, W = x.shape
  k = w.shape[2]
  y = torch.empty((B, C, Ho, Wo), dtype=x.dtype, device=x.device, memory_format=torch.channels_last)
  partial = None
  if want_stats:
    G = hip.depthwise_groups(B, Ho, Wo, C)
    partial = torch.empty((G, 4, C), dtype=torch.float32, device=x.device)
  with region('depthwise_fwd', float((x.numel() + y.numel()) * x.element_size())):
    hip.depthwise_fwd(x, w.detach().reshape(C, k, k), y, B, H, W, C, k, stride, ph, pw, Ho, Wo, partial=partial)
  if want_stats:
    y._pf_stats = (partial, G)
  return y


class _Depthwise(torch.autograd.Function):

  @staticmethod
  def forward(ctx, x, w, stride, ph, pw, Ho, Wo, want_stats, graph, w_var, box):
    x = _nhwc(x)
    y = _run_depthwise(x, w, stride, ph, pw, Ho, Wo, want_stats)
    ctx.save_for_backward(x, w)
    ctx.meta = (stride, ph, pw, Ho, Wo, graph, w_var)
    box.append(getattr(y, '_pf_stats', None))
    return y

  @staticmethod
  def backward(ctx, dy):
    x, w = ctx.saved_tensors
    stride, ph, pw, Ho, Wo, graph, w_var = ctx.meta
    dy = _nhwc(dy)
    if dy.dtype != x.dtype:
      dy = dy.to(x.dtype)
    B, C, H, W = x.shape
    k = w.shape[2]
    dx = dw = None
    if ctx.needs_input_grad[1]:
      G = hip.depthwise_groups(B, Ho, Wo, C)

      def wrw(dwk, scratch):
        hip.depthwise_wrw(dy, x, dwk, scratch((G + 32) * C * k * k), B, H, W, C, k, stride, ph, pw, Ho, Wo)
      dw = _filter_grad(graph, w, w_var, (dy, x), 'depthwise_wrw', float((x.numel() + dy.numel()) * x.element_size()), wrw)
    if ctx.needs_input_grad[0]:
      dx = torch.empty_like(x)
      with region('depthwise_bwd_data', float((x.numel() + dy.numel()) * x.element_size())):
        hip.depthwise_bwd_data(dy, w.detach().reshape(C, k, k), dx, B, H, W, C, k, stride, ph, pw, Ho, Wo)
    return dx, dw, None, None, None, None, None, None, None, None, None


class DepthwiseConv2D:

  def __init__(self, graph: Graph, name: str, channels: int, k: int, stride: int,
               kernel_name: str = 'depthwise_weights', init=None, l2: bool = True):
    self.graph, self.k, self.stride, self.channels = graph, k, stride, channels
    ref_shape = (k, k, channels, 1)
    init = init or truncated_normal_init(ref_shape, 0.09)
    self.kernel = graph.store.add(name + '/' + kernel_name, ref_shape, 'depthwise', True, l2, init)
    self.op = graph.add_matmul_op('DepthwiseConv2dNative', name + '/depthwise', self.kernel)

  def plain(self, x):
    taps, self.graph.taps = self.graph.taps, None
    try:
      return self(x)
    finally:
      self.graph.taps = taps

  def __call__(self, x, want_stats: bool = False) -> torch.Tensor:
    x = materialize(x)
    if self.graph.taps is not None:
      return _tapped(self, x)
    ph = _same_pads(x.shape[2], self.k, self.stride)
    pw = _same_pads(x.shape[3], self.k, self.stride)
    w = self.kernel.tensor
    if (OWN_DEPTHWISE and (x.is_cuda or DEPTHWISE_ANY_DEVICE) and x.dim() == 4 and x.dtype in (torch.float32, torch.bfloat16) and w.dtype == x.dtype
        and hip.depthwise_supported(self.channels, self.k, self.stride)):
      Ho, Wo = -(-x.shape[2] // self.stride), -(-x.shape[3] // self.stride)
      bn_box = getattr(x, '_pf_bn', None)
      if bn_box is not None:
        bn_box['n_consumers'] += 2
      if torch.is_grad_enabled() and (x.requires_grad or w.requires_grad):
        return _apply_with_stats(_Depthwise, x, w, self.stride, ph[0], pw[0], Ho, Wo, want_stats, self.graph, self.kernel)
      return _run_depthwise(_nhwc(x), w, self.stride, ph[0], pw[0], Ho, Wo, want_stats)
    x, pad = _symmetric_pads(x, ph, pw)
    return F.conv2d(x, self.kernel.tensor, None, stride=self.stride, padding=pad, groups=self.channels)


class Dense:

  def __init__(self, graph: Graph, name: str, cin: int, cout: int, init=None, l2: bool = True):
    self.graph = graph
    ref_shape = (cin, cout)
    init = init or glorot_uniform_init(ref_shape, cin, cout)
    self.kernel = graph.store.add(name + '/kernel', ref_shape, 'dense', True, l2, init)
    self.bias = graph.store.add(name + '/bias', (cout,), 'bias', True, l2, constant_init((cout,), 0.0))
    self.op = graph.add_matmul_op('MatMul', name + '/MatMul', self.kernel)

  def __call__(self, x) -> torch.Tensor:
    g = self.graph
    if g.taps is not None and g.tap_dense:
      x = materialize(x)
      y = self.plain(x)
      g.taps[self] = (x, y, None)
      if g.tap_stop is self:
        raise TapStop()
      return y + self.bias.tensor.to(x.dtype)
    x = materialize(x)
    if x.dim() == 2 and convg_ok(x, self.kernel.tensor, dense=True):
      w4 = self.kernel.tensor.view(self.kernel.tensor.shape[0], self.kernel.tensor.shape[1], 1, 1)
      y = _ConvGeneric.apply(x.contiguous().view(x.shape[0], x.shape[1], 1, 1), w4, self.bias.tensor, 1, (0, 0), (1, 1), self.graph)
      return y.view(x.shape[0], -1)
    return F.linear(x, self.kernel.tensor, self.bias.tensor.to(x.dtype))

  def plain(self, x: torch.Tensor) -> torch.Tensor:
    if x.dim() == 2 and convg_ok(x, self.kernel.tensor, dense=True):
      w4 = self.kernel.tensor.view(self.kernel.tensor.shape[0], self.kernel.tensor.shape[1], 1, 1)
      return _ConvGeneric.apply(x.contiguous().view(x.shape[0], x.shape[1], 1, 1), w4, None, 1, (0, 0), (1, 1), self.graph).view(x.shape[0], -1)
    return F.linear(x, self.kernel.tensor)


class Activation:

  def __init__(self, graph: Graph, name: str, act: str = 'Relu'):
    self.graph, self.act = graph, act
    self.op = graph.add_activation_op(act, name)

  def __call__(self, x: torch.Tensor) -> torch.Tensor:
    g = self.graph
    if self.op.bits is None:
      y = F.relu(x) if self.act == 'Relu' else F.relu6(x)
      return _pass_tag(x, y) if g.taps is not None else y
    return _ActQuant.apply(x, self.act, g.act_slots[self.op.index], self.op.bits)


class BatchNormAct:

  def __init__(self, graph: Graph, name: str, channels: int, act: Optional[str], momentum: float, eps: float,
               l2: bool = False, act_name: Optional[str] = None, names=('gamma', 'beta', 'moving_mean',
                                                                       'moving_variance'), lazy_ok: bool = False):
    self.graph, self.act, self.momentum, self.eps, self.C = graph, act, momentum, eps, channels
    self.lazy_ok = lazy_ok
    st = graph.store
    self.gamma = st.add(name + '/' + names[0], (channels,), 'bn_gamma', True, l2, constant_init((channels,), 1.0))
    self.beta = st.add(name + '/' + names[1], (channels,), 'bn_beta', True, l2, constant_init((channels,), 0.0))
    self.moving_mean = st.add(name + '/' + names[2], (channels,), 'bn_mean', False, False,
                              constant_init((channels,), 0.0))
    self.moving_var = st.add(name + '/' + names[3], (channels,), 'bn_var', False, False,
                             constant_init((channels,), 1.0))
    self.op = graph.add_activation_op(act, act_name or (name + '/' + act)) if act else None
    self._frozen_ss = None

  def folds_into_producer(self) -> bool:
    g = self.graph
    if not FOLD_EVAL_BN or g.taps is not None or not g.fuse_conv1x1:
      return False
    if g.training and torch.is_grad_enabled():
      return False
    if torch.is_grad_enabled() and not g.frozen:
      return False
    return self.op is None or self.op.bits is None

  def __call__(self, x: torch.Tensor, with_skip: bool = False):
    g = self.graph
    bits = self.op.bits if self.op is not None else None
    slot = g.act_slots[self.op.index] if (self.op is not None and bits is not None) else None
    lazy = self.lazy_ok and g.fuse_conv1x1 and fusable_tensor(x)
    skip = x
    if getattr(x, '_pf_bn_done', None) is self:
      y = x
    elif g.training and torch.is_grad_enabled():
      stats = getattr(x, '_pf_stats', None)
      if lazy:
        box = []
        alias, skip = _BnLazy.apply(_nhwc(x), self.gamma.tensor, self.beta.tensor, self, g, slot, bits, box, stats)
        y = LazyAct(alias, box[0], self.act, slot, bits, x.numel() // self.C, self.C, mean_invstd=box[1])
        box.append(weakref.ref(y))
      else:
        box = {}
        y = _BnActQuant.apply(x, self.gamma.tensor, self.beta.tensor, self, g, True, slot, bits, stats, box)
        y._pf_bn = box
    elif torch.is_grad_enabled() and not g.frozen and (x.requires_grad or self.gamma.tensor.requires_grad):
      if bits is not None:
        raise NotImplementedError('inference-mode BN with gradients and activation quantisation (no learner needs it)')
      y = _BnEvalAct.apply(materialize(x), self.gamma.tensor, self.beta.tensor, self, g)
    else:
      y = self._inference(_nhwc(x), slot, bits, lazy)
    if g.taps is not None and isinstance(y, torch.Tensor):
      y = _pass_tag(x, y)
    return (y, skip) if with_skip else y

  def _inference(self, x, slot, bits, lazy):
    C = self.C
    rows = x.numel() // C
    if bits is None and lazy:
      return LazyAct(x, self._eval_scale_shift(x), self.act, None, None, rows, C)
    q = torch.empty_like(x)
    if bits is None:
      hip.bn_act_quant_apply(x, q, rows, C, self._eval_scale_shift(x), self.act, None, 8, False)
      return q
    with torch.no_grad():
      nblk = _bn_blocks(rows, C)
      partial = self.graph.scratch(nblk * 4 * C)
      ss = torch.empty((2, C), dtype=torch.float32, device=x.device)
      mi = torch.empty((2, C), dtype=torch.float32, device=x.device)
      hip.bn_stats(x, rows, C, partial, nblk)
      hip.bn_finalize(partial, nblk, rows, C, x, self.gamma.tensor, self.beta.tensor, self.moving_mean.tensor,
                      self.moving_var.tensor, self.momentum, self.eps, self.graph.training, self.act, ss, mi, slot)
      hip.bn_act_quant_apply(x, q, rows, C, ss, self.act, slot, bits, True)
    return q

  def _eval_scale_shift(self, x):
    g = self.graph
    if g.frozen and self._frozen_ss is not None:
      return self._frozen_ss
    ss = torch.empty((2, self.C), dtype=torch.float32, device=x.device)
    hip.bn_eval_scale_shift(self.gamma.tensor, self.beta.tensor, self.moving_mean.tensor, self.moving_var.tensor,
                            self.eps, ss)
    if g.frozen:
      self._frozen_ss = ss
    return ss


class _MaxPool(torch.autograd.Function):

  @staticmethod
  def forward(ctx, x, k, stride, ph, pw):
    need_grad = ctx.needs_input_grad[0]
    x = _nhwc(x)
    B, C, H, W = x.shape
    Ho, Wo = _out_size(H, k, stride, ph[0] + ph[1]), _out_size(W, k, stride, pw[0] + pw[1])
    y = torch.empty((B, C, Ho, Wo), dtype=x.dtype, device=x.device, memory_format=torch.channels_last)
    idx = torch.empty((B, Ho, Wo, C), dtype=torch.uint8, device=x.device) if need_grad else None
    with region('maxpool_fwd', float((x.numel() + y.numel()) * x.element_size())):
      hip.maxpool_fwd(x, y, idx, B, H, W, C, k, stride, ph[0], pw[0], Ho, Wo)
    ctx.meta = (k, stride, ph[0], pw[0], x.shape)
    if need_grad:
      ctx.save_for_backward(idx)
    return y

  @staticmethod
  def backward(ctx, dy):
    (idx,) = ctx.saved_tensors
    k, stride, ph0, pw0, xshape = ctx.meta
    dy = _nhwc(dy)
    B, C, H, W = xshape
    dx = torch.empty(xshape, dtype=dy.dtype, device=dy.device, memory_format=torch.channels_last)
    with region('maxpool_bwd', float((dx.numel() + dy.numel()) * dy.element_size())):
      hip.maxpool_bwd(dy, idx, dx, B, H, W, C, k, stride, ph0, pw0, dy.shape[2], dy.shape[3])
    return dx, None, None, None, None


def max_pool_same(x: torch.Tensor, k: int, stride: int) -> torch.Tensor:
  ph = _same_pads(x.shape[2], k, stride)
  pw = _same_pads(x.shape[3], k, stride)
  if x.is_cuda and x.dim() == 4 and x.shape[1] % 8 == 0 and x.dtype in (torch.float32, torch.bfloat16) and OWN_POOL:
    return _MaxPool.apply(x, k, stride, ph, pw)
  if ph[0] == 0 and pw[0] == 0:
    return F.max_pool2d(x, k, stride, ceil_mode=True)
  if any(ph) or any(pw):
    x = F.pad(x, (pw[0], pw[1], ph[0], ph[1]), value=float('-inf'))
  return F.max_pool2d(x, k, stride)


def fixed_padding(x: torch.Tensor, k: int) -> torch.Tensor:
  pad_total = k - 1
  pb = pad_total // 2
  pe = pad_total - pb
  if pad_total == 0:
    return x
  return F.pad(x, (pb, pe, pb, pe))


def to_device_images(images, graph: Graph) -> torch.Tensor:
  if isinstance(images, np.ndarray):
    images = torch.from_numpy(images)
  x = images.to(graph.device, non_blocking=True)
  if x.dim() == 4:
    x = x.permute(0, 3, 1, 2)
  return x.to(graph.compute_dtype)
```

pocketflow_amd/hip.py:

```python
from __future__ import annotations

import ctypes
import os
from ctypes import c_float, c_int, c_int64, c_void_p

import numpy as np
import torch

_LIB_PATH = os.environ.get('PF_HIP_LIB') or os.path.join(os.path.dirname(os.path.abspath(__file__)), 'csrc', 'libpocketflow_hip.so')

PF_F32, PF_BF16 = 0, 1
PF_ACT_NONE, PF_ACT_RELU, PF_ACT_RELU6 = 0, 1, 2
PF_BUCKET_TENSOR, PF_BUCKET_CHANNEL, PF_BUCKET_SPLIT = 0, 1, 2
PF_CHUNK = 4096

SEG_DTYPE = np.dtype([('offset', '<i8'), ('len', '<i8'), ('RS', '<i4'), ('layout', '<i4'),
                      ('I', '<i4'), ('O', '<i4'), ('mode', '<i4'), ('bits', '<i4'),
                      ('bucket_size', '<i4'), ('n_bucket', '<i4'), ('slot_offset', '<i8'),
                      ('cb_offset', '<i8')])
BLOCK_DTYPE = np.dtype([('seg', '<i4'), ('chunk', '<i4'), ('row0', '<i4'), ('nrows', '<i4')])
assert SEG_DTYPE.itemsize == 64 and BLOCK_DTYPE.itemsize == 16

ACT_CODES = {None: PF_ACT_NONE, 'none': PF_ACT_NONE, 'Relu': PF_ACT_RELU, 'relu': PF_ACT_RELU,
             'Relu6': PF_ACT_RELU6, 'relu6': PF_ACT_RELU6}

SYMBOLS = [
    'pf_error_string', 'pf_version', 'pf_minmax_slots_init', 'pf_minmax_tensor', 'pf_minmax_decode',
    'pf_uq_apply', 'pf_act_grad', 'pf_seg_minmax', 'pf_seg_uq_apply', 'pf_seg_nuq_apply',
    'pf_seg_nuq_codebook_grad', 'pf_seg_normalize', 'pf_ws_bkup_merge_abs', 'pf_kth_largest_nonneg',
    'pf_ws_mask_apply', 'pf_count_nonzero', 'pf_cp_build_mask', 'pf_cp_mask_grad', 'pf_adam_flat',
    'pf_momentum_flat', 'pf_ce_distill_fwd_bwd', 'pf_bn_stats', 'pf_bn_finalize',
    'pf_bn_act_quant_apply', 'pf_bn_bwd_stats', 'pf_bn_bwd_finalize', 'pf_bn_bwd_apply', 'pf_bn_bwd_apply_add',
    'pf_bn_eval_scale_shift',
    'pf_conv1x1_stats_groups_k', 'pf_conv1x1_fwd', 'pf_conv1x1_bwd_data_bnstats', 'pf_conv1x1_wrw_splits',
    'pf_conv1x1_wrw', 'pf_conv2d_fwd', 'pf_conv2d_wrw_splits', 'pf_conv2d_wrw', 'pf_maxpool_fwd', 'pf_maxpool_bwd', 'pf_seg_transpose', 'pf_conv_stem_supported', 'pf_conv_stem_fwd', 'pf_conv_stem_wrw_slabs', 'pf_conv_stem_wrw',
    'pf_image_resize_bilinear', 'pf_depthwise_supported', 'pf_depthwise_groups', 'pf_depthwise_fwd', 'pf_depthwise_bwd_data',
    'pf_depthwise_wrw', 'pf_conv2d_stats_groups_geom', 'pf_tuning_reload',
    'pf_adam_flat_dev', 'pf_momentum_flat_dev', 'pf_set_floats',
    'pf_convg_fwd', 'pf_convg_bwd_data', 'pf_convg_small_splits', 'pf_convg_wrw_splits', 'pf_convg_wrw', 'pf_conv2d_bwd_data_strided',
    'pf_prox_groups', 'pf_prox_norms', 'pf_prox_apply', 'pf_im2col', 'pf_col2im',
    'pf_conv_stem3_supported', 'pf_conv_stem3_fwd', 'pf_conv_stem3_wrw_slabs', 'pf_conv_stem3_wrw',
    'pf_conv1x1_fwd_affine', 'pf_conv2d_fwd_affine', 'pf_conv2d_bwd_data_strided_stats_groups',
    'pf_conv2d_bwd_data_strided_bnstats',
    'pf_cpr_gather', 'pf_cpr_gram_ws', 'pf_cpr_gram', 'pf_cpr_ista', 'pf_cpr_lstsq_splits', 'pf_cpr_lstsq_step', 'pf_cpr_lstsq_resid',
    'pf_conv_gather_fwd',
    'pf_conv1x1_join_plan', 'pf_conv1x1_bwd_data_join',
]


class HipLibraryMissing(RuntimeError):
  pass


def lib_path() -> str:
  return _LIB_PATH


def _load() -> ctypes.CDLL:
  if not os.path.exists(_LIB_PATH):
    raise HipLibraryMissing(
        'pocketflow_amd: %s not found -- build it with `python -c "import __graft_entry__ as g; '
        'g.build()"` or pocketflow_amd/csrc/build.sh.  There is no CPU fallback.' % _LIB_PATH)
  lib = ctypes.CDLL(_LIB_PATH)
  lib.pf_error_string.restype = ctypes.c_char_p
  lib.pf_error_string.argtypes = [c_int]
  lib.pf_version.restype = c_int
  for name in SYMBOLS:
    fn = getattr(lib, name)
    if name not in ('pf_error_string',):
      fn.restype = c_int
  lib.pf_cpr_gram_ws.restype = c_int64
  return lib


_lib = _load()


def _check(err: int, what: str) -> None:
  if err != 0:
    raise RuntimeError('%s failed: hipError %d (%s)' % (what, err, _lib.pf_error_string(err).decode()))


_raw_stream = getattr(torch._C, '_cuda_getCurrentRawStream', None)
_get_device = getattr(torch._C, '_cuda_getDevice', None)


def _stream() -> c_void_p:
  if _raw_stream is not None and _get_device is not None:
    return c_void_p(_raw_stream(_get_device()))
  return c_void_p(torch.cuda.current_stream().cuda_stream)


def _ptr(t) -> c_void_p:
  if t is None:
    return c_void_p(0)
  return c_void_p(t.data_ptr())


def dtype_code(t: torch.Tensor) -> int:
  if t.dtype == torch.float32:
    return PF_F32
  if t.dtype == torch.bfloat16:
    return PF_BF16
  raise TypeError('unsupported dtype %s (float32 / bfloat16 only)' % t.dtype)


def _dev(t: torch.Tensor) -> None:
  if not t.is_cuda:
    raise RuntimeError('pocketflow_amd kernels run on the GPU only (got a %s tensor)' % t.device)


def version() -> int:
  return int(_lib.pf_version())


def tuning_reload() -> None:
  _check(_lib.pf_tuning_reload(), 'pf_tuning_reload')



def minmax_slots_init(slots: torch.Tensor) -> None:
  _dev(slots)
  _check(_lib.pf_minmax_slots_init(_ptr(slots), c_int64(slots.numel() // 2), _stream()), 'pf_minmax_slots_init')


def minmax_tensor(x: torch.Tensor, slot: torch.Tensor, act=None) -> None:
  _dev(x)
  _check(_lib.pf_minmax_tensor(_ptr(x), c_int64(x.numel()), c_int(dtype_code(x)), c_int(ACT_CODES[act]),
                               _ptr(slot), _stream()), 'pf_minmax_tensor')


def minmax_decode(slots: torch.Tensor) -> torch.Tensor:
  n = slots.numel() // 2
  out = torch.empty((n, 2), dtype=torch.float32, device=slots.device)
  _check(_lib.pf_minmax_decode(_ptr(slots), c_int64(n), _ptr(out), _stream()), 'pf_minmax_decode')
  return out


def uq_apply(x: torch.Tensor, y: torch.Tensor, slot: torch.Tensor, bits: int, act=None) -> None:
  _dev(x)
  _check(_lib.pf_uq_apply(_ptr(x), _ptr(y), c_int64(x.numel()), c_int(dtype_code(x)), c_int(dtype_code(y)),
                          c_int(ACT_CODES[act]), _ptr(slot), c_int(int(bits)), _stream()), 'pf_uq_apply')


def act_grad(g: torch.Tensor, u: torch.Tensor, dx: torch.Tensor, act) -> None:
  _dev(g)
  assert g.dtype == u.dtype == dx.dtype
  _check(_lib.pf_act_grad(_ptr(g), _ptr(u), _ptr(dx), c_int64(g.numel()), c_int(dtype_code(g)),
                          c_int(ACT_CODES[act]), _stream()), 'pf_act_grad')



def seg_minmax(w_flat, segs, blocks, n_blocks, slots) -> None:
  _check(_lib.pf_seg_minmax(_ptr(w_flat), _ptr(segs), _ptr(blocks), c_int(n_blocks), _ptr(slots), _stream()),
         'pf_seg_minmax')


def seg_uq_apply(w_flat, qw_flat, segs, blocks, n_blocks, slots) -> None:
  _check(_lib.pf_seg_uq_apply(_ptr(w_flat), _ptr(qw_flat), c_int(dtype_code(qw_flat)), _ptr(segs), _ptr(blocks),
                              c_int(n_blocks), _ptr(slots), _stream()), 'pf_seg_uq_apply')


def seg_nuq_apply(w_flat, qw_flat, idx_flat, codebooks, segs, blocks, n_blocks, slots) -> None:
  _check(_lib.pf_seg_nuq_apply(_ptr(w_flat), _ptr(qw_flat), c_int(dtype_code(qw_flat)), _ptr(idx_flat),
                               _ptr(codebooks), _ptr(segs), _ptr(blocks), c_int(n_blocks), _ptr(slots),
                               _stream()), 'pf_seg_nuq_apply')


def seg_nuq_codebook_grad(g_flat, idx_flat, dcodebooks, acc_ws, segs, blocks, n_blocks, slots) -> None:
  assert acc_ws.dtype == torch.int64 and acc_ws.numel() >= dcodebooks.numel()
  _check(_lib.pf_seg_nuq_codebook_grad(_ptr(g_flat), c_int(dtype_code(g_flat)), _ptr(idx_flat), _ptr(dcodebooks),
                                       _ptr(acc_ws), c_int64(dcodebooks.numel()), _ptr(segs), _ptr(blocks),
                                       c_int(n_blocks), _ptr(slots), _stream()),
         'pf_seg_nuq_codebook_grad')


def seg_normalize(w_flat, xn_out, segs, seg_index, slots) -> None:
  _check(_lib.pf_seg_normalize(_ptr(w_flat), _ptr(xn_out), _ptr(segs), c_int(seg_index), _ptr(slots), _stream()),
         'pf_seg_normalize')



def ws_bkup_merge_abs(var, bkup, mask, abs_out) -> None:
  _check(_lib.pf_ws_bkup_merge_abs(_ptr(var), _ptr(bkup), _ptr(mask), _ptr(abs_out), c_int64(var.numel()),
                                   _stream()), 'pf_ws_bkup_merge_abs')


def kth_largest_nonneg(a, k_desc_index: int, out, workspace) -> None:
  _check(_lib.pf_kth_largest_nonneg(_ptr(a), c_int64(a.numel()), c_int64(int(k_desc_index)), _ptr(out),
                                    _ptr(workspace), _stream()), 'pf_kth_largest_nonneg')


def ws_mask_apply(var, bkup, mask, thr) -> None:
  _check(_lib.pf_ws_mask_apply(_ptr(var), _ptr(bkup), _ptr(mask), _ptr(thr), c_int64(var.numel()), _stream()),
         'pf_ws_mask_apply')


def count_nonzero(x, out_u64) -> None:
  _check(_lib.pf_count_nonzero(_ptr(x), c_int64(x.numel()), _ptr(out_u64), _stream()), 'pf_count_nonzero')


def cp_build_mask(mask, keep_in, keep_out, O: int, RS: int, I: int) -> None:
  _check(_lib.pf_cp_build_mask(_ptr(mask), _ptr(keep_in), _ptr(keep_out), c_int(O), c_int(RS), c_int(I),
                               _stream()), 'pf_cp_build_mask')


def cp_mask_grad(g, keep_in, keep_out, O: int, RS: int, I: int) -> None:
  _check(_lib.pf_cp_mask_grad(_ptr(g), _ptr(keep_in), _ptr(keep_out), c_int(O), c_int(RS), c_int(I), _stream()),
         'pf_cp_mask_grad')



def adam_flat(p, g, m, v, mask, n_decay: int, wd: float, g_scale: float, lr: float, beta1: float,
              beta2: float, eps: float, beta1_power: float, beta2_power: float) -> None:
  _check(_lib.pf_adam_flat(_ptr(p), _ptr(g), c_int(dtype_code(g)), _ptr(m), _ptr(v), _ptr(mask),
                           c_int64(p.numel()), c_int64(int(n_decay)), c_float(wd), c_float(g_scale), c_float(lr),
                           c_float(beta1), c_float(beta2), c_float(eps), c_float(beta1_power),
                           c_float(beta2_power), _stream()), 'pf_adam_flat')


def momentum_flat(p, g, acc, mask, n_decay: int, wd: float, g_scale: float, lr: float,
                  momentum: float) -> None:
  _check(_lib.pf_momentum_flat(_ptr(p), _ptr(g), c_int(dtype_code(g)), _ptr(acc), _ptr(mask), c_int64(p.numel()),
                               c_int64(int(n_decay)), c_float(wd), c_float(g_scale), c_float(lr),
                               c_float(momentum), _stream()), 'pf_momentum_flat')


def adam_flat_dev(p, g, m, v, mask, n_decay: int, wd: float, g_scale: float, hp, beta1: float, beta2: float,
                  eps: float) -> None:
  _check(_lib.pf_adam_flat_dev(_ptr(p), _ptr(g), c_int(dtype_code(g)), _ptr(m), _ptr(v), _ptr(mask),
                               c_int64(p.numel()), c_int64(int(n_decay)), c_float(wd), c_float(g_scale), _ptr(hp),
                               c_float(beta1), c_float(beta2), c_float(eps), _stream()), 'pf_adam_flat_dev')


def momentum_flat_dev(p, g, acc, mask, n_decay: int, wd: float, g_scale: float, hp, momentum: float) -> None:
  _check(_lib.pf_momentum_flat_dev(_ptr(p), _ptr(g), c_int(dtype_code(g)), _ptr(acc), _ptr(mask), c_int64(p.numel()),
                                   c_int64(int(n_decay)), c_float(wd), c_float(g_scale), _ptr(hp),
                                   c_float(momentum), _stream()), 'pf_momentum_flat_dev')


def set_floats(dst, a: float, b: float = 0.0, c: float = 0.0, d: float = 0.0) -> None:
  assert dst.dtype == torch.float32 and dst.numel() >= 4
  _check(_lib.pf_set_floats(_ptr(dst), c_float(a), c_float(b), c_float(c), c_float(d), _stream()), 'pf_set_floats')


def prox_groups(rows: int, I: int) -> int:
  return int(_lib.pf_prox_groups(c_int64(rows), c_int(I)))


def prox_norms(w, g, lr: float, rows: int, I: int, partial, norms) -> None:
  _dev(w)
  if w.dtype != torch.float32 or partial.numel() < prox_groups(rows, I) * I or norms.numel() < I:
    raise TypeError('prox_norms: float32 master kernel, workspace of prox_groups(rows, I) * I floats')
  _check(_lib.pf_prox_norms(_ptr(w), _ptr(g), c_int(dtype_code(g)), c_float(lr), c_int64(rows), c_int(I), _ptr(partial), _ptr(norms),
                            _stream()), 'pf_prox_norms')


def prox_apply(w, g, lr: float, rows: int, I: int, norms, thr) -> None:
  _dev(w)
  _check(_lib.pf_prox_apply(_ptr(w), _ptr(g), c_int(dtype_code(g)), c_float(lr), c_int64(rows), c_int(I), _ptr(norms), _ptr(thr),
                            _stream()), 'pf_prox_apply')



def _f32_dev(*ts) -> None:
  for t in ts:
    _dev(t)
    if t.dtype != torch.float32 or not t.is_contiguous():
      raise TypeError('pf_cpr: contiguous float32 tensors expected (got %s)' % t.dtype)


def _i32_dev(*ts) -> None:
  for t in ts:
    _dev(t)
    if t.dtype != torch.int32 or not t.is_contiguous():
      raise TypeError('pf_cpr: contiguous int32 tensors expected (got %s)' % t.dtype)


def cpr_gather(x, y, pos, kh: int, kw: int, stride: int, pad_t: int, pad_l: int, P, Y, row0: int) -> None:
  _dev(x)
  _dev(y)
  _i32_dev(pos)
  _f32_dev(P, Y)
  B, C, H, W = x.shape
  By, Co, OH, OW = y.shape
  crops = pos.shape[0]
  if By != B or not x.is_contiguous(memory_format=torch.channels_last) or not y.is_contiguous(memory_format=torch.channels_last):
    raise TypeError('cpr_gather: channels-last taps of one batch expected')
  if pos.numel() != 2 * crops or int(pos[:, 0].min()) < 0 or int(pos[:, 0].max()) >= OH or int(pos[:, 1].min()) < 0 or int(pos[:, 1].max()) >= OW:
    raise ValueError('cpr_gather: positions outside the %d x %d output' % (OH, OW))
  rows = row0 + crops * B
  if P.numel() < rows * kh * kw * C or Y.numel() < rows * Co:
    raise ValueError('cpr_gather: P / Y hold fewer than %d rows' % rows)
  _check(_lib.pf_cpr_gather(_ptr(x), c_int(dtype_code(x)), _ptr(y), c_int(dtype_code(y)), _ptr(pos), c_int(crops), c_int(B), c_int(H), c_int(W),
                            c_int(C), c_int(OH), c_int(OW), c_int(Co), c_int(kh), c_int(kw), c_int(stride), c_int(pad_t), c_int(pad_l), _ptr(P),
                            _ptr(Y), c_int64(row0), _stream()), 'pf_cpr_gather')


def cpr_gram_ws(C: int) -> int:
  return int(_lib.pf_cpr_gram_ws(c_int(C)))


def cpr_gram(P, Y, idx, kk: int, C: int, Co: int, w_krsc, ws, xtx, xty) -> None:
  _f32_dev(P, Y, w_krsc, xtx, xty)
  _i32_dev(idx)
  _dev(ws)
  rows = P.numel() // (kk * C)
  if ws.dtype != torch.float64 or ws.numel() < cpr_gram_ws(C) or w_krsc.numel() != Co * kk * C or xtx.numel() < C * C or xty.numel() < C:
    raise ValueError('cpr_gram: buffer sizes')
  if idx.numel() and (int(idx.min()) < 0 or int(idx.max()) >= rows or Y.numel() < rows * Co):
    raise ValueError('cpr_gram: row indices outside the %d sampled rows' % rows)
  _check(_lib.pf_cpr_gram(_ptr(P), _ptr(Y), _ptr(idx), c_int64(idx.numel()), c_int(kk), c_int(C), c_int(Co), _ptr(w_krsc), _ptr(ws),
                          c_int64(ws.numel()), _ptr(xtx), _ptr(xty), _stream()), 'pf_cpr_gram')


def cpr_ista(A, b, m0, m_ws, mask, gamma: float, lr: float, iters: int, nnz) -> None:
  C = b.numel()
  _f32_dev(A, b, m0, m_ws, mask)
  _i32_dev(nnz)
  if A.numel() != C * C or m0.numel() != C or m_ws.numel() < 2 * C or mask.numel() != C:
    raise ValueError('cpr_ista: buffer sizes')
  _check(_lib.pf_cpr_ista(_ptr(A), _ptr(b), _ptr(m0), _ptr(m_ws), _ptr(mask), c_int(C), c_float(gamma), c_float(lr), c_int(iters), _ptr(nnz),
                          _stream()), 'pf_cpr_ista')


def cpr_lstsq_splits(N: int, Kp: int, Co: int) -> int:
  return int(_lib.pf_cpr_lstsq_splits(c_int64(N), c_int(Kp), c_int(Co)))


def _lstsq_check(P, kidx, Y, R, W, N, Co):
  _f32_dev(P, Y, R, W)
  _i32_dev(kidx)
  K = W.numel() // Co
  if P.numel() < N * K or Y.numel() < N * Co or R.numel() < N * Co or W.numel() != K * Co:
    raise ValueError('cpr_lstsq: buffer sizes')
  if kidx.numel() and (int(kidx.min()) < 0 or int(kidx.max()) >= K):
    raise ValueError('cpr_lstsq: kept rows outside the kernel')
  return K


def cpr_lstsq_step(P, kidx, pos, Y, R, W, m, v, part, N: int, Co: int, wd: float, lr_t: float, beta1: float, beta2: float, c1: float,
                   c2: float, eps: float) -> None:
  K = _lstsq_check(P, kidx, Y, R, W, N, Co)
  _f32_dev(m, v, part)
  _i32_dev(pos)
  Kp = kidx.numel()
  if pos.numel() != K or m.numel() != K * Co or v.numel() != K * Co or part.numel() < cpr_lstsq_splits(N, Kp, Co) * Kp * Co:
    raise ValueError('cpr_lstsq_step: buffer sizes')
  _check(_lib.pf_cpr_lstsq_step(_ptr(P), c_int(K), _ptr(kidx), _ptr(pos), c_int(Kp), _ptr(Y), _ptr(R), c_int64(N), c_int(Co), _ptr(W), _ptr(m),
                                _ptr(v), _ptr(part), c_float(wd), c_float(lr_t), c_float(beta1), c_float(beta2), c_float(c1), c_float(c2),
                                c_float(eps), _stream()), 'pf_cpr_lstsq_step')


def cpr_lstsq_resid(P, kidx, W, Y, R, N: int, Co: int) -> None:
  K = _lstsq_check(P, kidx, Y, R, W, N, Co)
  _check(_lib.pf_cpr_lstsq_resid(_ptr(P), c_int(K), _ptr(kidx), c_int(kidx.numel()), _ptr(W), _ptr(Y), _ptr(R), c_int64(N), c_int(Co),
                                 _stream()), 'pf_cpr_lstsq_resid')



def ce_distill_fwd_bwd(z_s, labels, z_t, tempr: float, loss_w: float, losses, dz_s, row_ws) -> None:
  B, C = z_s.shape
  _check(_lib.pf_ce_distill_fwd_bwd(_ptr(z_s), c_int(dtype_code(z_s)), _ptr(labels), _ptr(z_t),
                                    c_int(dtype_code(z_t) if z_t is not None else 0), c_int(B), c_int(C),
                                    c_float(tempr), c_float(loss_w), _ptr(losses), _ptr(dz_s),
                                    c_int(dtype_code(dz_s)), _ptr(row_ws), _stream()), 'pf_ce_distill_fwd_bwd')



def bn_stats(x, rows: int, C: int, partial, n_blocks: int) -> None:
  _check(_lib.pf_bn_stats(_ptr(x), c_int(dtype_code(x)), c_int64(rows), c_int(C), _ptr(partial), c_int(n_blocks),
                          _stream()), 'pf_bn_stats')


def bn_finalize(partial, n_blocks, rows, C, x, gamma, beta, moving_mean, moving_var, momentum, eps,
                training: bool, act, scale_shift, mean_invstd, slot) -> None:
  _check(_lib.pf_bn_finalize(_ptr(partial), c_int(n_blocks), c_int64(rows), c_int(C), _ptr(x),
                             c_int(dtype_code(x)), _ptr(gamma), _ptr(beta), _ptr(moving_mean), _ptr(moving_var),
                             c_float(momentum), c_float(eps), c_int(1 if training else 0), c_int(ACT_CODES[act]),
                             _ptr(scale_shift), _ptr(mean_invstd), _ptr(slot), _stream()), 'pf_bn_finalize')


def bn_act_quant_apply(x, q, rows, C, scale_shift, act, slot, bits: int, quantize: bool) -> None:
  _check(_lib.pf_bn_act_quant_apply(_ptr(x), _ptr(q), c_int(dtype_code(x)), c_int64(rows), c_int(C),
                                    _ptr(scale_shift), c_int(ACT_CODES[act]), _ptr(slot), c_int(int(bits)),
                                    c_int(1 if quantize else 0), _stream()), 'pf_bn_act_quant_apply')


def bn_bwd_stats(dq, x, rows, C, scale_shift, mean_invstd, act, partial, n_blocks) -> None:
  _check(_lib.pf_bn_bwd_stats(_ptr(dq), _ptr(x), c_int(dtype_code(x)), c_int64(rows), c_int(C), _ptr(scale_shift),
                              _ptr(mean_invstd), c_int(ACT_CODES[act]), _ptr(partial), c_int(n_blocks),
                              _stream()), 'pf_bn_bwd_stats')


def bn_bwd_finalize(partial, n_blocks, C, dgamma, dbeta) -> None:
  _check(_lib.pf_bn_bwd_finalize(_ptr(partial), c_int(n_blocks), c_int(C), _ptr(dgamma), _ptr(dbeta), _stream()),
         'pf_bn_bwd_finalize')


def bn_bwd_apply(dq, x, dx, rows, C, scale_shift, mean_invstd, dgamma, dbeta, act, addend=None) -> None:
  _check(_lib.pf_bn_bwd_apply_add(_ptr(dq), _ptr(x), _ptr(addend), _ptr(dx), c_int(dtype_code(x)), c_int64(rows),
                                  c_int(C), _ptr(scale_shift), _ptr(mean_invstd), _ptr(dgamma), _ptr(dbeta),
                                  c_int(ACT_CODES[act]), _stream()), 'pf_bn_bwd_apply_add')


def bn_eval_scale_shift(gamma, beta, moving_mean, moving_var, eps: float, scale_shift) -> None:
  _check(_lib.pf_bn_eval_scale_shift(_ptr(gamma), _ptr(beta), _ptr(moving_mean), _ptr(moving_var), c_float(eps),
                                     c_int(gamma.numel()), _ptr(scale_shift), _stream()), 'pf_bn_eval_scale_shift')



def conv1x1_stats_groups(M: int, N: int, K: int, prologue: bool = False) -> int:
  return int(_lib.pf_conv1x1_stats_groups_k(c_int(M), c_int(N), c_int(K), c_int(1 if prologue else 0)))


def conv1x1_wrw_splits(M: int, N: int, K: int) -> int:
  return int(_lib.pf_conv1x1_wrw_splits(c_int(M), c_int(N), c_int(K)))


def conv1x1_fwd(X, W, Y, M: int, N: int, K: int, R=None, scale_shift=None, act=None, slot=None, bits: int = 8,
                partial=None, geom=None, ymap: bool = False, out_scale_shift=None, out_act=None) -> None:
  _dev(X)
  Ho, Wo, H, Wd, stride = geom if geom is not None else (0, 0, 0, 0, 1)
  if out_scale_shift is not None:
    if R is not None or partial is not None or slot is not None or ymap:
      raise ValueError('the folded output pass takes no residual, statistics, quantiser or row map')
    _check(_lib.pf_conv1x1_fwd_affine(_ptr(X), _ptr(W), _ptr(Y), _ptr(scale_shift), c_int(ACT_CODES[act]), _ptr(out_scale_shift),
                                      c_int(ACT_CODES[out_act]), c_int(M), c_int(N), c_int(K), c_int(Ho), c_int(Wo), c_int(H),
                                      c_int(Wd), c_int(stride), _stream()), 'pf_conv1x1_fwd_affine')
    return
  _check(_lib.pf_conv1x1_fwd(_ptr(X), _ptr(W), _ptr(Y), _ptr(R), _ptr(scale_shift), c_int(ACT_CODES[act]),
                             _ptr(slot), c_int(int(bits)), _ptr(partial), c_int(M), c_int(N), c_int(K), c_int(Ho),
                             c_int(Wo), c_int(H), c_int(Wd), c_int(stride), c_int(1 if ymap else 0), _stream()),
         'pf_conv1x1_fwd')


def conv1x1_wrw(dY, X, dW, workspace, M: int, N: int, K: int, scale_shift=None, act=None, slot=None,
                bits: int = 8, geom=None) -> None:
  _dev(X)
  Ho, Wo, H, Wd, stride = geom if geom is not None else (0, 0, 0, 0, 1)
  _check(_lib.pf_conv1x1_wrw(_ptr(dY), _ptr(X), _ptr(dW), c_int(dtype_code(dW)), _ptr(workspace), _ptr(scale_shift),
                             c_int(ACT_CODES[act]), _ptr(slot), c_int(int(bits)), c_int(M), c_int(N), c_int(K),
                             c_int(Ho), c_int(Wo), c_int(H), c_int(Wd), c_int(stride), _stream()), 'pf_conv1x1_wrw')


def conv1x1_bwd_data_bnstats(dY, Wt, dQ, bn_x, bn_scale_shift, bn_mean_invstd, bn_act, partial, M: int, N: int,
                             K: int) -> None:
  _dev(dY)
  _check(_lib.pf_conv1x1_bwd_data_bnstats(_ptr(dY), _ptr(Wt), _ptr(dQ), _ptr(bn_x), _ptr(bn_scale_shift),
                                          _ptr(bn_mean_invstd), c_int(ACT_CODES[bn_act]), _ptr(partial), c_int(M),
                                          c_int(N), c_int(K), _stream()), 'pf_conv1x1_bwd_data_bnstats')


def conv1x1_join_plan(M: int, N: int, K: int, with_stats: bool = False) -> int:
  return int(_lib.pf_conv1x1_join_plan(c_int(M), c_int(N), c_int(K), c_int(1 if with_stats else 0)))


def conv1x1_bwd_data_join(dY, Wt, dQ, R, M: int, N: int, K: int, rgeom=None, bn_x=None, bn_scale_shift=None,
                          bn_mean_invstd=None, bn_act=None, partial=None) -> None:
  _dev(dY)
  Ho, Wo, H, Wd, stride = rgeom if rgeom is not None else (0, 0, 0, 0, 1)
  _check(_lib.pf_conv1x1_bwd_data_join(_ptr(dY), _ptr(Wt), _ptr(dQ), _ptr(R), c_int(Ho), c_int(Wo), c_int(H), c_int(Wd),
                                       c_int(stride), _ptr(bn_x), _ptr(bn_scale_shift), _ptr(bn_mean_invstd),
                                       c_int(ACT_CODES[bn_act]), _ptr(partial), c_int(M), c_int(N), c_int(K), _stream()),
         'pf_conv1x1_bwd_data_join')



_zero_page = {}


def zero_page(device):
  key = str(device)
  z = _zero_page.get(key)
  if z is None:
    z = _zero_page[key] = torch.zeros(256, dtype=torch.bfloat16, device=device)
  return z


def conv2d_stats_groups(M: int, N: int, geom=None) -> int:
  if geom is None:
    raise ValueError('conv2d_stats_groups: pass geom = (imgs, H, Wd, C, N, th, tw, stride, pad_h, pad_w, Ho, Wo) of the pf_conv2d_fwd call')
  return int(_lib.pf_conv2d_stats_groups_geom(*[c_int(int(v)) for v in geom]))


def conv2d_fwd(X, W, Y, imgs: int, H: int, Wd: int, C: int, N: int, th: int, tw: int, stride: int, pad_h: int,
               pad_w: int, Ho: int, Wo: int, R=None, partial=None, bn_x=None, bn_scale_shift=None,
               bn_mean_invstd=None, bn_act=None, out_scale_shift=None, out_act=None) -> None:
  _dev(X)
  if out_scale_shift is not None:
    if R is not None or partial is not None or bn_x is not None:
      raise ValueError('the folded output pass takes no residual or statistics')
    _check(_lib.pf_conv2d_fwd_affine(_ptr(X), _ptr(W), _ptr(Y), _ptr(zero_page(X.device)), _ptr(out_scale_shift),
                                     c_int(ACT_CODES[out_act]), c_int(imgs), c_int(H), c_int(Wd), c_int(C), c_int(N), c_int(th),
                                     c_int(tw), c_int(stride), c_int(pad_h), c_int(pad_w), c_int(Ho), c_int(Wo), _stream()),
           'pf_conv2d_fwd_affine')
    return
  _check(_lib.pf_conv2d_fwd(_ptr(X), _ptr(W), _ptr(Y), _ptr(zero_page(X.device)), _ptr(R), _ptr(partial), _ptr(bn_x),
                            _ptr(bn_scale_shift), _ptr(bn_mean_invstd), c_int(ACT_CODES[bn_act]), c_int(imgs), c_int(H),
                            c_int(Wd), c_int(C), c_int(N), c_int(th), c_int(tw), c_int(stride), c_int(pad_h),
                            c_int(pad_w), c_int(Ho), c_int(Wo), _stream()), 'pf_conv2d_fwd')


def conv2d_wrw_splits(M: int, N: int, C: int, taps: int) -> int:
  return int(_lib.pf_conv2d_wrw_splits(c_int(M), c_int(N), c_int(C), c_int(taps)))


def conv2d_wrw(dY, X, dW, workspace, imgs: int, H: int, Wd: int, C: int, N: int, th: int, tw: int, stride: int,
               pad_h: int, pad_w: int, Ho: int, Wo: int) -> None:
  _dev(X)
  _check(_lib.pf_conv2d_wrw(_ptr(dY), _ptr(X), _ptr(dW), c_int(dtype_code(dW)), _ptr(workspace), c_int(imgs), c_int(H),
                            c_int(Wd), c_int(C), c_int(N), c_int(th), c_int(tw), c_int(stride), c_int(pad_h),
                            c_int(pad_w), c_int(Ho), c_int(Wo), _stream()), 'pf_conv2d_wrw')


def depthwise_supported(C: int, k: int, stride: int) -> bool:
  return bool(_lib.pf_depthwise_supported(c_int(C), c_int(k), c_int(stride)))


def depthwise_groups(B: int, Ho: int, Wo: int, C: int) -> int:
  return int(_lib.pf_depthwise_groups(c_int(B), c_int(Ho), c_int(Wo), c_int(C)))


def depthwise_fwd(X, W, Y, B: int, H: int, Wd: int, C: int, k: int, stride: int, pad_h: int, pad_w: int, Ho: int, Wo: int,
                  partial=None) -> None:
  _dev(X)
  _check(_lib.pf_depthwise_fwd(_ptr(X), _ptr(W), _ptr(Y), c_int(dtype_code(X)), _ptr(partial), c_int(B), c_int(H), c_int(Wd),
                               c_int(C), c_int(k), c_int(stride), c_int(pad_h), c_int(pad_w), c_int(Ho), c_int(Wo),
                               _stream()), 'pf_depthwise_fwd')


def depthwise_bwd_data(dY, W, dX, B: int, H: int, Wd: int, C: int, k: int, stride: int, pad_h: int, pad_w: int, Ho: int,
                       Wo: int) -> None:
  _dev(dY)
  _check(_lib.pf_depthwise_bwd_data(_ptr(dY), _ptr(W), _ptr(dX), c_int(dtype_code(dY)), c_int(B), c_int(H), c_int(Wd), c_int(C),
                                    c_int(k), c_int(stride), c_int(pad_h), c_int(pad_w), c_int(Ho), c_int(Wo), _stream()),
         'pf_depthwise_bwd_data')


def depthwise_wrw(dY, X, dW, slabs, B: int, H: int, Wd: int, C: int, k: int, stride: int, pad_h: int, pad_w: int, Ho: int,
                  Wo: int) -> None:
  _dev(X)
  if slabs.dtype != torch.float32 or slabs.numel() < (depthwise_groups(B, Ho, Wo, C) + 32) * C * k * k:
    raise TypeError('depthwise_wrw: float32 workspace of (groups + 32) * C * k * k elements')
  _check(_lib.pf_depthwise_wrw(_ptr(dY), _ptr(X), _ptr(dW), c_int(dtype_code(X)), c_int(dtype_code(dW)), _ptr(slabs), c_int(B),
                               c_int(H), c_int(Wd), c_int(C), c_int(k), c_int(stride), c_int(pad_h), c_int(pad_w), c_int(Ho),
                               c_int(Wo), _stream()), 'pf_depthwise_wrw')


def conv2d_bwd_data_strided_stats_groups(B: int, H: int, Wd: int, C: int, stride: int) -> int:
  return int(_lib.pf_conv2d_bwd_data_strided_stats_groups(c_int(B), c_int(H), c_int(Wd), c_int(C), c_int(stride)))


def conv2d_bwd_data_strided(dY, Wt, dX, B: int, H: int, Wd: int, C: int, N: int, R: int, S: int, stride: int, pad_h: int,
                            pad_w: int, Ho: int, Wo: int, partial=None, bn_x=None, bn_scale_shift=None, bn_mean_invstd=None,
                            bn_act=None) -> None:
  _dev(dY)
  if dY.dtype != torch.bfloat16 or Wt.dtype != torch.bfloat16 or dX.dtype != torch.bfloat16:
    raise TypeError('conv2d_bwd_data_strided: bf16 tensors')
  if bn_x is not None:
    _check(_lib.pf_conv2d_bwd_data_strided_bnstats(_ptr(dY), _ptr(Wt), _ptr(dX), _ptr(zero_page(dY.device)), _ptr(bn_x),
                                                   _ptr(bn_scale_shift), _ptr(bn_mean_invstd), c_int(ACT_CODES[bn_act]),
                                                   _ptr(partial), c_int(B), c_int(H), c_int(Wd), c_int(C), c_int(N), c_int(R),
                                                   c_int(S), c_int(stride), c_int(pad_h), c_int(pad_w), c_int(Ho), c_int(Wo),
                                                   _stream()), 'pf_conv2d_bwd_data_strided_bnstats')
    return
  _check(_lib.pf_conv2d_bwd_data_strided(_ptr(dY), _ptr(Wt), _ptr(dX), _ptr(zero_page(dY.device)), c_int(B), c_int(H), c_int(Wd),
                                         c_int(C), c_int(N), c_int(R), c_int(S), c_int(stride), c_int(pad_h), c_int(pad_w), c_int(Ho),
                                         c_int(Wo), _stream()), 'pf_conv2d_bwd_data_strided')


def im2col(X, Xcol, B: int, H: int, Wd: int, C: int, R: int, S: int, stride: int, pad_h: int, pad_w: int, Ho: int, Wo: int) -> None:
  _dev(X)
  if X.dtype != torch.bfloat16 or Xcol.dtype != torch.bfloat16 or Xcol.numel() < B * Ho * Wo * R * S * C:
    raise TypeError('im2col: bf16 tensors, Xcol of B*Ho*Wo*R*S*C elements')
  _check(_lib.pf_im2col(_ptr(X), _ptr(Xcol), c_int(B), c_int(H), c_int(Wd), c_int(C), c_int(R), c_int(S), c_int(stride), c_int(pad_h),
                        c_int(pad_w), c_int(Ho), c_int(Wo), _stream()), 'pf_im2col')


def col2im(dXcol, dX, B: int, H: int, Wd: int, C: int, R: int, S: int, stride: int, pad_h: int, pad_w: int, Ho: int, Wo: int) -> None:
  _dev(dXcol)
  if dXcol.dtype != torch.bfloat16 or dX.dtype != torch.bfloat16:
    raise TypeError('col2im: bf16 tensors')
  _check(_lib.pf_col2im(_ptr(dXcol), _ptr(dX), c_int(B), c_int(H), c_int(Wd), c_int(C), c_int(R), c_int(S), c_int(stride), c_int(pad_h),
                        c_int(pad_w), c_int(Ho), c_int(Wo), _stream()), 'pf_col2im')



def convg_fwd(X, Wk, bias, Y, B: int, H: int, Wd: int, C: int, N: int, R: int, S: int, stride: int, pad_h: int, pad_w: int,
              Ho: int, Wo: int, slab=None) -> None:
  _dev(X)
  if Wk.dtype != X.dtype or Y.dtype != X.dtype or (bias is not None and bias.dtype != torch.float32):
    raise TypeError('convg_fwd: X / Wk / Y share one dtype, the bias is float32')
  _check(_lib.pf_convg_fwd(_ptr(X), _ptr(Wk), _ptr(bias), _ptr(Y), c_int(dtype_code(X)), c_int(B), c_int(H), c_int(Wd), c_int(C),
                           c_int(N), c_int(R), c_int(S), c_int(stride), c_int(pad_h), c_int(pad_w), c_int(Ho), c_int(Wo), _ptr(slab),
                           c_int64(slab.numel() if slab is not None else 0), _stream()), 'pf_convg_fwd')


def check_gather(gather, C: int, Ck: int, what: str = 'gather') -> np.ndarray:
  g = np.asarray(gather)
  if g.ndim != 1 or g.size != Ck or not np.issubdtype(g.dtype, np.integer):
    raise ValueError('%s: expected an integer vector of %d kept channels, got shape %s dtype %s' % (what, Ck, g.shape, g.dtype))
  g = g.astype(np.int64)
  if g.size == 0 or g[0] < 0 or g[-1] >= C or np.any(np.diff(g) <= 0):
    raise ValueError('%s: kept channels must be strictly ascending and lie in [0, %d)' % (what, C))
  return np.ascontiguousarray(g.astype(np.int32))


def conv_gather_fwd(X, Wk, gather, Y, B: int, H: int, Wd: int, C: int, N: int, R: int, S: int, stride: int, pad_h: int, pad_w: int,
                    Ho: int, Wo: int, bias=None, residual=None, scale_shift=None, act=None) -> None:
  _dev(X)
  Ck = int(gather.numel())
  if Wk.dtype != X.dtype or Y.dtype != X.dtype or (residual is not None and residual.dtype != X.dtype):
    raise TypeError('conv_gather_fwd: X / Wk / Y / residual share one dtype')
  if gather.dtype != torch.int32 or (bias is not None and bias.dtype != torch.float32) or (
      scale_shift is not None and scale_shift.dtype != torch.float32):
    raise TypeError('conv_gather_fwd: gather is int32, bias and scale_shift are float32')
  if X.numel() != B * H * Wd * C or Wk.numel() != N * R * S * Ck or Y.numel() != B * Ho * Wo * N or not 1 <= Ck <= C or (
      residual is not None and residual.numel() != Y.numel()) or (bias is not None and bias.numel() != N) or (
      scale_shift is not None and scale_shift.numel() != 2 * N):
    raise ValueError('conv_gather_fwd: operand sizes do not match B=%d H=%d W=%d C=%d Ck=%d N=%d R=%d S=%d Ho=%d Wo=%d'
                     % (B, H, Wd, C, Ck, N, R, S, Ho, Wo))
  if (Ho - 1) * stride + R - 2 * pad_h > H or (Wo - 1) * stride + S - 2 * pad_w > Wd:
    raise ValueError('conv_gather_fwd: the output extends beyond the symmetrically padded input')
  _check(_lib.pf_conv_gather_fwd(_ptr(X), _ptr(Wk), _ptr(gather), _ptr(bias), _ptr(residual), _ptr(scale_shift),
                                 c_int(ACT_CODES[act]), _ptr(Y), c_int(dtype_code(X)), c_int(B), c_int(H), c_int(Wd), c_int(C),
                                 c_int(Ck), c_int(N), c_int(R), c_int(S), c_int(stride), c_int(pad_h), c_int(pad_w), c_int(Ho),
                                 c_int(Wo), _stream()), 'pf_conv_gather_fwd')


def convg_bwd_data(dY, Wk, dX, B: int, H: int, Wd: int, C: int, N: int, R: int, S: int, stride: int, pad_h: int, pad_w: int,
                   Ho: int, Wo: int, slab=None) -> None:
  _dev(dY)
  if Wk.dtype != dY.dtype or dX.dtype != dY.dtype:
    raise TypeError('convg_bwd_data: dY / Wk / dX share one dtype')
  _check(_lib.pf_convg_bwd_data(_ptr(dY), _ptr(Wk), _ptr(dX), c_int(dtype_code(dY)), c_int(B), c_int(H), c_int(Wd), c_int(C),
                                c_int(N), c_int(R), c_int(S), c_int(stride), c_int(pad_h), c_int(pad_w), c_int(Ho), c_int(Wo),
                                _ptr(slab), c_int64(slab.numel() if slab is not None else 0), _stream()), 'pf_convg_bwd_data')


def convg_small_splits(M: int, Nc: int, K: int) -> int:
  return int(_lib.pf_convg_small_splits(c_int(M), c_int(Nc), c_int(K)))


def convg_wrw_splits(B: int, C: int, N: int, R: int, S: int, Ho: int, Wo: int) -> int:
  return int(_lib.pf_convg_wrw_splits(c_int(B), c_int(C), c_int(N), c_int(R), c_int(S), c_int(Ho), c_int(Wo)))


def convg_wrw(dY, X, dW, slab, B: int, H: int, Wd: int, C: int, N: int, R: int, S: int, stride: int, pad_h: int, pad_w: int,
              Ho: int, Wo: int) -> None:
  _dev(X)
  if dY.dtype != X.dtype or slab.dtype != torch.float32 or slab.numel() < convg_wrw_splits(B, C, N, R, S, Ho, Wo) * N * R * S * C:
    raise TypeError('convg_wrw: dY / X share one dtype; float32 workspace of splits * N * R * S * C elements')
  _check(_lib.pf_convg_wrw(_ptr(dY), _ptr(X), _ptr(dW), c_int(dtype_code(X)), c_int(dtype_code(dW)), _ptr(slab), c_int(B), c_int(H),
                           c_int(Wd), c_int(C), c_int(N), c_int(R), c_int(S), c_int(stride), c_int(pad_h), c_int(pad_w), c_int(Ho),
                           c_int(Wo), _stream()), 'pf_convg_wrw')


TILE_DTYPE = np.dtype([('src_off', '<i8'), ('dst_off', '<i8'), ('O', '<i4'), ('I', '<i4'), ('src_ld', '<i4'),
                       ('dst_ld', '<i4'), ('o0', '<i4'), ('i0', '<i4'), ('r0', '<i4'), ('r1', '<i4')])
assert TILE_DTYPE.itemsize == 48


def seg_transpose(src_flat, dst_flat, tiles, n_tiles: int) -> None:
  _dev(src_flat)
  _check(_lib.pf_seg_transpose(_ptr(src_flat), _ptr(dst_flat), c_int(dtype_code(src_flat)), _ptr(tiles), c_int(n_tiles),
                               _stream()), 'pf_seg_transpose')



def conv_stem_supported(H: int, Wd: int, C: int, N: int, k: int, stride: int, pad: int) -> bool:
  return bool(_lib.pf_conv_stem_supported(c_int(H), c_int(Wd), c_int(C), c_int(N), c_int(k), c_int(stride), c_int(pad)))


def conv_stem_fwd(X, W, Y, imgs: int, H: int, Wd: int) -> None:
  _dev(X)
  _check(_lib.pf_conv_stem_fwd(_ptr(X), _ptr(W), _ptr(Y), c_int(imgs), c_int(H), c_int(Wd), _stream()), 'pf_conv_stem_fwd')


def conv_stem_wrw_slabs(imgs: int, H: int, Wd: int) -> int:
  return int(_lib.pf_conv_stem_wrw_slabs(c_int(imgs), c_int(H), c_int(Wd)))


def conv_stem_wrw(dY, X, dW, workspace, imgs: int, H: int, Wd: int) -> None:
  _dev(dY)
  _check(_lib.pf_conv_stem_wrw(_ptr(dY), _ptr(X), _ptr(dW), c_int(dtype_code(dW)), _ptr(workspace), c_int(imgs), c_int(H),
                               c_int(Wd), _stream()), 'pf_conv_stem_wrw')


def conv_stem3_supported(H: int, Wd: int, C: int, N: int, k: int, stride: int, pad_h: int, pad_w: int, Ho: int, Wo: int) -> bool:
  return bool(_lib.pf_conv_stem3_supported(c_int(H), c_int(Wd), c_int(C), c_int(N), c_int(k), c_int(stride), c_int(pad_h), c_int(pad_w),
                                           c_int(Ho), c_int(Wo)))


def conv_stem3_fwd(X, W, Y, imgs: int, H: int, Wd: int, N: int, pad_h: int, pad_w: int, Ho: int, Wo: int) -> None:
  _dev(X)
  _check(_lib.pf_conv_stem3_fwd(_ptr(X), _ptr(W), _ptr(Y), c_int(imgs), c_int(H), c_int(Wd), c_int(N), c_int(pad_h), c_int(pad_w),
                                c_int(Ho), c_int(Wo), _stream()), 'pf_conv_stem3_fwd')


def conv_stem3_wrw_slabs(imgs: int, H: int, Wd: int, N: int, pad_h: int, pad_w: int, Ho: int, Wo: int) -> int:
  return int(_lib.pf_conv_stem3_wrw_slabs(c_int(imgs), c_int(H), c_int(Wd), c_int(N), c_int(pad_h), c_int(pad_w), c_int(Ho), c_int(Wo)))


def conv_stem3_wrw(dY, X, dW, workspace, imgs: int, H: int, Wd: int, N: int, pad_h: int, pad_w: int, Ho: int, Wo: int) -> None:
  _dev(dY)
  _check(_lib.pf_conv_stem3_wrw(_ptr(dY), _ptr(X), _ptr(dW), c_int(dtype_code(dW)), _ptr(workspace), c_int(imgs), c_int(H), c_int(Wd),
                                c_int(N), c_int(pad_h), c_int(pad_w), c_int(Ho), c_int(Wo), _stream()), 'pf_conv_stem3_wrw')



def maxpool_fwd(x, y, idx, B: int, H: int, W: int, C: int, k: int, stride: int, pad_h: int, pad_w: int, Ho: int,
                Wo: int) -> None:
  _dev(x)
  _check(_lib.pf_maxpool_fwd(_ptr(x), _ptr(y), _ptr(idx), c_int(dtype_code(x)), c_int(B), c_int(H), c_int(W), c_int(C),
                             c_int(k), c_int(stride), c_int(pad_h), c_int(pad_w), c_int(Ho), c_int(Wo), _stream()),
         'pf_maxpool_fwd')


def maxpool_bwd(dy, idx, dx, B: int, H: int, W: int, C: int, k: int, stride: int, pad_h: int, pad_w: int, Ho: int,
                Wo: int) -> None:
  _dev(dy)
  _check(_lib.pf_maxpool_bwd(_ptr(dy), _ptr(idx), _ptr(dx), c_int(dtype_code(dy)), c_int(B), c_int(H), c_int(W), c_int(C),
                             c_int(k), c_int(stride), c_int(pad_h), c_int(pad_w), c_int(Ho), c_int(Wo), _stream()),
         'pf_maxpool_bwd')



IMAGE_DESC_DTYPE = np.dtype([('offset', '<i8'), ('h', '<i4'), ('w', '<i4'), ('scale_y', '<f4'), ('scale_x', '<f4'),
                             ('off_y', '<i4'), ('off_x', '<i4'), ('flip', '<i4'), ('reserved', '<i4')])


def image_resize_bilinear(src_u8, desc_u8, out, mean) -> None:
  B, OH, OW, C = out.shape
  assert C == 3 and out.is_contiguous() and desc_u8.numel() == B * IMAGE_DESC_DTYPE.itemsize
  _check(_lib.pf_image_resize_bilinear(_ptr(src_u8), _ptr(desc_u8), _ptr(out), c_int(dtype_code(out)), c_int(B),
                                       c_int(OH), c_int(OW), c_float(mean[0]), c_float(mean[1]), c_float(mean[2]),
                                       _stream()), 'pf_image_resize_bilinear')
```

pocketflow_amd/optim.py:

```python
from __future__ import annotations

from typing import List, Optional

import numpy as np
import torch
import torch.distributed as dist

from pocketflow_amd import hip
from pocketflow_amd.graph import VarStore


class FlatOptimizer(object):
  def __init__(self, store: VarStore, kind: str = 'adam', momentum: float = 0.9, beta1: float = 0.9,
               beta2: float = 0.999, epsilon: float = 1e-8, weight_decay: float = 0.0):
    if kind not in ('adam', 'momentum'):
      raise ValueError('unknown optimizer kind: ' + kind)
    self.store, self.kind = store, kind
    self.momentum, self.beta1, self.beta2, self.epsilon = momentum, beta1, beta2, epsilon
    self.weight_decay = weight_decay
    dev = store.device
    self.slots_w = [torch.zeros_like(store.w_master) for _ in range(2 if kind == 'adam' else 1)]
    self.slots_o = [torch.zeros_like(store.o_master) for _ in range(2 if kind == 'adam' else 1)]
    self.beta1_power = np.float32(beta1)
    self.beta2_power = np.float32(beta2)
    self.w_mask: Optional[torch.Tensor] = None
    self.o_mask: Optional[torch.Tensor] = None
    self.g_scale = 1.0
    self.w_grad_src: Optional[torch.Tensor] = None
    self.o_grad_src: Optional[torch.Tensor] = None
    self.hp: Optional[torch.Tensor] = None
    self.hyper_external = False

  def enable_device_hyper(self) -> None:
    if self.hp is None:
      self.hp = torch.zeros(4, dtype=torch.float32, device=self.store.device)

  def feed_hyper(self, lrn_rate: float) -> None:
    one = np.float32(1.0)
    alpha_t = 0.0
    if self.kind == 'adam':
      alpha_t = float(np.float32(np.float32(lrn_rate) * np.sqrt(one - np.float32(self.beta2_power))) / (one - np.float32(self.beta1_power)))
      self.beta1_power = np.float32(self.beta1_power * np.float32(self.beta1))
      self.beta2_power = np.float32(self.beta2_power * np.float32(self.beta2))
    hip.set_floats(self.hp, alpha_t, float(lrn_rate))

  def state_tensors(self) -> List[torch.Tensor]:
    return self.slots_w + self.slots_o

  def reset_slots(self) -> None:
    for t in self.state_tensors():
      t.zero_()
    self.beta1_power = np.float32(self.beta1)
    self.beta2_power = np.float32(self.beta2)

  def backward(self, loss: torch.Tensor) -> None:
    from pocketflow_amd import graph as G
    with G.wrw_side_armed(self.store):
      loss.backward()

  def compute_gradients(self) -> None:
    self.g_scale = 1.0
    self.w_grad_src = self.o_grad_src = None

  def apply_gradients(self, lrn_rate: float) -> None:
    st = self.store
    wd = float(self.weight_decay)
    w_grad = self.w_grad_src if self.w_grad_src is not None else st.w_grad
    o_grad = self.o_grad_src if self.o_grad_src is not None else st.o_grad
    if self.hp is not None:
      if not self.hyper_external:
        self.feed_hyper(lrn_rate)
      if self.kind == 'adam':
        if st.w_size:
          hip.adam_flat_dev(st.w_master, w_grad, self.slots_w[0], self.slots_w[1], self.w_mask, st.w_decay, wd, self.g_scale,
                            self.hp, self.beta1, self.beta2, self.epsilon)
        if st.o_size:
          hip.adam_flat_dev(st.o_master, o_grad, self.slots_o[0], self.slots_o[1], self.o_mask, st.o_decay, wd, self.g_scale,
                            self.hp, self.beta1, self.beta2, self.epsilon)
      else:
        if st.w_size:
          hip.momentum_flat_dev(st.w_master, w_grad, self.slots_w[0], self.w_mask, st.w_decay, wd, self.g_scale, self.hp,
                                self.momentum)
        if st.o_size:
          hip.momentum_flat_dev(st.o_master, o_grad, self.slots_o[0], self.o_mask, st.o_decay, wd, self.g_scale, self.hp,
                                self.momentum)
      st.w_t_fresh = False
      st.zero_grad()
      return
    if self.kind == 'adam':
      b1p, b2p = float(self.beta1_power), float(self.beta2_power)
      if st.w_size:
        hip.adam_flat(st.w_master, w_grad, self.slots_w[0], self.slots_w[1], self.w_mask, st.w_decay, wd,
                      self.g_scale, lrn_rate, self.beta1, self.beta2, self.epsilon, b1p, b2p)
      if st.o_size:
        hip.adam_flat(st.o_master, o_grad, self.slots_o[0], self.slots_o[1], self.o_mask, st.o_decay, wd,
                      self.g_scale, lrn_rate, self.beta1, self.beta2, self.epsilon, b1p, b2p)
      self.beta1_power = np.float32(self.beta1_power * np.float32(self.beta1))
      self.beta2_power = np.float32(self.beta2_power * np.float32(self.beta2))
    else:
      if st.w_size:
        hip.momentum_flat(st.w_master, w_grad, self.slots_w[0], self.w_mask, st.w_decay, wd, self.g_scale,
                          lrn_rate, self.momentum)
      if st.o_size:
        hip.momentum_flat(st.o_master, o_grad, self.slots_o[0], self.o_mask, st.o_decay, wd, self.g_scale,
                          lrn_rate, self.momentum)
    st.w_t_fresh = False
    st.zero_grad()


class GradReducer(object):

  def __init__(self, store: VarStore, bucket_elems: int = 8 << 20, reduce_dtype: Optional[torch.dtype] = torch.float32,
               overlap: bool = True):
    self.store = store
    self.overlap = overlap
    self.reduce_dtype = reduce_dtype
    self.buckets = []
    self.var_bucket = {}
    self._build_buckets(bucket_elems)
    self._stage_w: Optional[torch.Tensor] = None
    self._stage_o: Optional[torch.Tensor] = None
    self._reset_cycle()
    self.armed = False
    store.grad_hook = self._on_grad
    self.n_overlapped = 0
    self.recorder = None

  def _build_buckets(self, bucket_elems: int) -> None:
    ws = sorted([v for v in self.store.vars if v.group == 'W' and v.trainable], key=lambda v: v.offset)
    lo, cnt = 0, 0
    for i, v in enumerate(ws):
      self.var_bucket[v.name] = len(self.buckets)
      cnt += 1
      end = v.offset + v.numel
      last = i == len(ws) - 1
      if last:
        end = self.store.w_size
      if end - lo >= bucket_elems or last:
        self.buckets.append([lo, end, cnt])
        lo, cnt = end, 0

  def _reset_cycle(self) -> None:
    self.pending = [b[2] for b in self.buckets]
    self.seen = set()
    self.launched = [False] * len(self.buckets)
    self.handles = []
    self.dirty = False

  def _active(self) -> bool:
    return dist.is_initialized() and dist.get_world_size() > 1

  def _stage(self, which: str) -> torch.Tensor:
    st = self.store
    src = st.w_grad if which == 'w' else st.o_grad
    dt = self.reduce_dtype or src.dtype
    buf = self._stage_w if which == 'w' else self._stage_o
    if buf is None or buf.dtype != dt:
      buf = torch.empty(src.numel(), dtype=dt, device=src.device)
      if which == 'w':
        self._stage_w = buf
      else:
        self._stage_o = buf
    return buf

  def _stage_bucket(self, b: int):
    lo, hi, _ = self.buckets[b]
    piece = self._stage('w')[lo:hi]
    side = getattr(self.store, 'wrw_side', None)
    if side is not None and side.forks and self.store.w_grad.is_cuda:
      cur = torch.cuda.current_stream(self.store.w_grad.device)
      if cur != side.stream:
        cur.wait_stream(side.stream)
    piece.copy_(self.store.w_grad[lo:hi])
    self.launched[b] = True
    return lambda: self.handles.append(dist.all_reduce(piece, op=dist.ReduceOp.SUM, async_op=True))

  def _launch(self, b: int) -> None:
    self._stage_bucket(b)()

  def _recording(self) -> bool:
    return self.recorder is not None and getattr(self.recorder, 'capturing', False)

  def arm(self) -> None:
    for h in self.handles:
      h.wait()
    self._reset_cycle()
    self.armed = True

  def disarm(self) -> None:
    self.armed = False

  def _on_grad(self, var) -> None:
    if not (self.overlap and self._active()) or var.group != 'W' or self._recording():
      return
    if not self.armed:
      if any(self.launched):
        self.dirty = True
      return
    b = self.var_bucket.get(var.name)
    if b is None:
      return
    if var.name in self.seen:
      return
    self.seen.add(var.name)
    self.pending[b] -= 1
    if self.pending[b] == 0 and not self.launched[b]:
      self._launch(b)
      self.n_overlapped += 1

  def finish(self):
    st = self.store
    self.armed = False
    if not self._active():
      self._reset_cycle()
      return st.w_grad, st.o_grad, 1.0
    n_over = sum(self.launched)
    if self.dirty:
      for h in self.handles:
        h.wait()
      self.handles = []
      self.launched = [False] * len(self.buckets)
      n_over = 0
    calls = []
    if st.w_size:
      calls = [self._stage_bucket(b) for b in range(len(self.buckets)) if not self.launched[b]]
    w_src = self._stage('w') if st.w_size else st.w_grad
    o_src = st.o_grad
    if st.o_size:
      o_src = self._stage('o')
      o_src.copy_(st.o_grad)
    o_piece = o_src if st.o_size else None

    def exchange():
      for call in calls:
        call()
      if o_piece is not None:
        self.handles.append(dist.all_reduce(o_piece, op=dist.ReduceOp.SUM, async_op=True))
      for h in self.handles:
        h.wait()
      self.handles = []
    if self.recorder is not None:
      self.recorder.cut(exchange)
    else:
      exchange()
    self._reset_cycle()
    self.n_overlapped = n_over
    return w_src, o_src, 1.0 / dist.get_world_size()


def grad_reducer_of(store: VarStore) -> GradReducer:
  r = getattr(store, 'reducer', None)
  if r is None:
    import os
    from pocketflow_amd.flags import FLAGS
    rd = {'float32': torch.float32, 'compute': None}[FLAGS.allreduce_dtype if 'allreduce_dtype' in FLAGS else 'float32']
    r = GradReducer(store, bucket_elems=int(os.environ.get('PF_ALLREDUCE_BUCKET', 8 << 20)), reduce_dtype=rd,
                    overlap=os.environ.get('PF_OVERLAP_ALLREDUCE', '1') != '0')
    store.reducer = r
  return r


class DistributedFlatOptimizer(object):

  _OWN = ('opt', 'reducer')

  def __init__(self, optimizer: FlatOptimizer):
    object.__setattr__(self, 'opt', optimizer)
    object.__setattr__(self, 'reducer', grad_reducer_of(optimizer.store))

  def __getattr__(self, name):
    return getattr(self.opt, name)

  def __setattr__(self, name, value):
    if name in DistributedFlatOptimizer._OWN:
      object.__setattr__(self, name, value)
    else:
      setattr(self.opt, name, value)

  def backward(self, loss: torch.Tensor) -> None:
    from pocketflow_amd import graph as G
    self.reducer.arm()
    try:
      with G.wrw_side_armed(self.opt.store):
        loss.backward()
    finally:
      self.reducer.disarm()

  def compute_gradients(self) -> None:
    w_src, o_src, scale = self.reducer.finish()
    self.opt.w_grad_src, self.opt.o_grad_src = w_src, o_src
    self.opt.g_scale = scale

  def apply_gradients(self, lrn_rate: float) -> None:
    self.opt.apply_gradients(lrn_rate)
```

pocketflow_amd/utils/external/resnet_model.py:

```python
from __future__ import annotations

from typing import List, Optional


import torch

from pocketflow_amd.graph import (Activation, BatchNormAct, Conv2D, Dense, Graph, fixed_padding,
                                  materialize, max_pool_same)

_BATCH_NORM_DECAY = 0.997
_BATCH_NORM_EPSILON = 1e-5
DEFAULT_VERSION = 2


class _ConvFixedPadding:

  def __init__(self, graph: Graph, cin: int, filters: int, kernel_size: int, strides: int):
    self.k, self.strides = kernel_size, strides
    name = graph.unique_name('resnet_model/conv2d')
    self.explicit_pad = strides > 1 and kernel_size % 2 == 0
    if strides == 1:
      padding = 'SAME'
    elif self.explicit_pad:
      padding = 'VALID'
    else:
      padding = (kernel_size - 1) // 2
    self.conv = Conv2D(graph, name, cin, filters, kernel_size, strides, padding=padding, use_bias=False)

  def __call__(self, x, residual=None, want_stats=False, out_bn=None) -> torch.Tensor:
    if self.explicit_pad:
      x = fixed_padding(materialize(x), self.k)
    elif self.strides > 1 and self.conv.graph.taps is not None:
      x = materialize(x)
      x = x.view(x.shape)
    return self.conv(x, residual=residual, want_stats=want_stats, out_bn=out_bn)


def _batch_norm_relu(graph: Graph, channels: int, relu: bool = True, lazy_ok: bool = False) -> BatchNormAct:
  name = graph.unique_name('resnet_model/batch_normalization')
  act_name = graph.unique_name('resnet_model/Relu') if relu else None
  return BatchNormAct(graph, name, channels, 'Relu' if relu else None, _BATCH_NORM_DECAY,
                      _BATCH_NORM_EPSILON, l2=False, act_name=act_name, lazy_ok=lazy_ok)


class _BuildingBlockV2:

  def __init__(self, graph, cin, filters, projection, strides):
    self.bn1 = _batch_norm_relu(graph, cin)
    self.proj = _ConvFixedPadding(graph, cin, filters, 1, strides) if projection else None
    self.conv1 = _ConvFixedPadding(graph, cin, filters, 3, strides)
    self.bn2 = _batch_norm_relu(graph, filters)
    self.conv2 = _ConvFixedPadding(graph, filters, filters, 3, 1)
    self.cout = filters

  def __call__(self, x):
    shortcut = x
    y = self.bn1(x)
    if self.proj is not None:
      shortcut = self.proj(y)
    y = self.conv1(y)
    y = self.bn2(y)
    return self.conv2(y, residual=shortcut)


class _BottleneckBlockV2:

  def __init__(self, graph, cin, filters, projection, strides):
    self.bn1 = _batch_norm_relu(graph, cin, lazy_ok=True)
    self.proj = _ConvFixedPadding(graph, cin, 4 * filters, 1, strides) if projection else None
    self.conv1 = _ConvFixedPadding(graph, cin, filters, 1, 1)
    self.bn2 = _batch_norm_relu(graph, filters)
    self.conv2 = _ConvFixedPadding(graph, filters, filters, 3, strides)
    self.bn3 = _batch_norm_relu(graph, filters, lazy_ok=True)
    self.conv3 = _ConvFixedPadding(graph, filters, 4 * filters, 1, 1)
    self.cout = 4 * filters

  def __call__(self, x):
    pre, shortcut = self.bn1(x, with_skip=True)
    y = self.conv1(pre, want_stats=True, out_bn=self.bn2)
    if self.proj is not None:
      shortcut = self.proj(pre)
      if hasattr(pre, 'join_ok'):
        pre.join_ok = True
    y = self.bn2(y)
    y = self.conv2(y, want_stats=True, out_bn=self.bn3)
    y = self.bn3(y)
    return self.conv3(y, residual=shortcut, want_stats=True)


class _BuildingBlockV1:

  def __init__(self, graph, cin, filters, projection, strides):
    self.proj = _ConvFixedPadding(graph, cin, filters, 1, strides) if projection else None
    self.proj_bn = _batch_norm_relu(graph, filters, relu=False) if projection else None
    self.conv1 = _ConvFixedPadding(graph, cin, filters, 3, strides)
    self.bn1 = _batch_norm_relu(graph, filters)
    self.conv2 = _ConvFixedPadding(graph, filters, filters, 3, 1)
    self.bn2 = _batch_norm_relu(graph, filters, relu=False)
    self.relu = Activation(graph, graph.unique_name('resnet_model/Relu'), 'Relu')
    self.cout = filters

  def __call__(self, x):
    shortcut = x
    if self.proj is not None:
      shortcut = self.proj_bn(self.proj(x))
    y = self.bn1(self.conv1(x))
    y = self.bn2(self.conv2(y))
    return self.relu(y + shortcut)


class Model(object):

  def __init__(self, resnet_size, bottleneck, num_classes, num_filters, kernel_size, conv_stride,
               first_pool_size, first_pool_stride, block_sizes, block_strides,
               resnet_version=DEFAULT_VERSION, data_format=None, graph: Optional[Graph] = None,
               in_channels: int = 3):
    if resnet_version not in (1, 2):
      raise ValueError('Resnet version should be 1 or 2. See README for citations.')
    if data_format not in (None, 'channels_last'):
      raise ValueError('the MI355X executor is NHWC (channels_last) only')
    if bottleneck and resnet_version == 1:
      raise NotImplementedError('bottleneck v1 is not on the hot path (reference default is v2)')
    self.graph = graph
    self.resnet_version = resnet_version
    self.first_pool_size, self.first_pool_stride = first_pool_size, first_pool_stride
    self.pre_activation = resnet_version == 2
    g = graph
    self.initial_conv = _ConvFixedPadding(g, in_channels, num_filters, kernel_size, conv_stride)
    self.initial_bn = _batch_norm_relu(g, num_filters) if resnet_version == 1 else None
    if bottleneck:
      block_cls = _BottleneckBlockV2
    else:
      block_cls = _BuildingBlockV2 if resnet_version == 2 else _BuildingBlockV1
    self.blocks: List = []
    cin = num_filters
    for i, num_blocks in enumerate(block_sizes):
      filters = num_filters * (2 ** i)
      blk = block_cls(g, cin, filters, True, block_strides[i])
      self.blocks.append(blk)
      cin = blk.cout
      for _ in range(1, num_blocks):
        blk = block_cls(g, cin, filters, False, 1)
        self.blocks.append(blk)
        cin = blk.cout
    self.final_bn = _batch_norm_relu(g, cin) if self.pre_activation else None
    self.dense = Dense(g, 'resnet_model/dense', cin, num_classes)
    self.num_classes = num_classes

  def __call__(self, inputs: torch.Tensor, training: bool) -> torch.Tensor:
    g = self.graph
    g.training = bool(training)
    x = self.initial_conv(inputs)
    if self.initial_bn is not None:
      x = self.initial_bn(x)
    if self.first_pool_size:
      x = max_pool_same(x, self.first_pool_size, self.first_pool_stride)
    for blk in self.blocks:
      x = blk(x)
    if self.final_bn is not None:
      x = self.final_bn(x)
    x = x.float().mean(dim=(2, 3)).to(x.dtype)
    return self.dense(x)
```

Before: 11460.

## Fuse stem conv with maxpool and zero gradients inside optimizer kernels

Adds a fused 7x7 stem convolution plus 3x3 max-pool forward that writes pooled output and argmax indices, and a weight-gradient path that scatters pooled gradients through those indices straight into the stem wrw kernel's shared-memory staging. This avoids materialising the full-resolution stem output and skips separate maxpool forward/backward passes. It also adds optimizer kernel variants that zero the gradient buffer while reading it, replacing a separate zero_grad memset pass. The risks are extra index traffic and branchy scatter logic in the wrw kernel, plus correctness edge cases around padding and aliasing of gradient buffers.

```diff
diff --git a/include/pocketflow_hip.h b/include/pocketflow_hip.h
--- a/include/pocketflow_hip.h
+++ b/include/pocketflow_hip.h
@@ -82,6 +82,18 @@
                          int64_t n, int64_t n_decay, float wd, float g_scale, const float* hp,
                          float momentum, void* stream);
 int pf_set_floats(float* dst, float a, float b, float c, float d, void* stream);
+int pf_adam_flat_zero(float* p, void* g, int g_dtype, float* m, float* v, const float* mask,
+                      int64_t n, int64_t n_decay, float wd, float g_scale, float lr, float beta1,
+                      float beta2, float eps, float beta1_power, float beta2_power, void* stream);
+int pf_momentum_flat_zero(float* p, void* g, int g_dtype, float* acc, const float* mask,
+                          int64_t n, int64_t n_decay, float wd, float g_scale, float lr, float momentum,
+                          void* stream);
+int pf_adam_flat_dev_zero(float* p, void* g, int g_dtype, float* m, float* v, const float* mask,
+                          int64_t n, int64_t n_decay, float wd, float g_scale, const float* hp, float beta1,
+                          float beta2, float eps, void* stream);
+int pf_momentum_flat_dev_zero(float* p, void* g, int g_dtype, float* acc, const float* mask,
+                              int64_t n, int64_t n_decay, float wd, float g_scale, const float* hp,
+                              float momentum, void* stream);
 
 int pf_ce_distill_fwd_bwd(const void* z_s, int zs_dtype, const float* labels, const void* z_t,
                           int zt_dtype, int B, int C, float tempr, float loss_w, float* losses,
@@ -163,6 +175,10 @@
 int pf_conv_stem_wrw_slabs(int imgs, int H, int Wd);
 int pf_conv_stem_wrw(const void* dY, const void* X, void* dW, int dw_dtype, float* workspace, int imgs, int H, int Wd,
                      void* stream);
+int pf_conv_stem_pool_supported(int imgs, int H, int Wd);
+int pf_conv_stem_pool_fwd(const void* X, const void* W, void* Y, void* idx, int imgs, int H, int Wd, int pad_h, void* stream);
+int pf_conv_stem_pool_wrw(const void* dP, const void* idx, const void* X, void* dW, int dw_dtype, float* workspace, int imgs,
+                          int H, int Wd, int pad_h, void* stream);
 
 int pf_conv_stem3_supported(int H, int Wd, int C, int N, int k, int stride, int pad_h, int pad_w, int Ho, int Wo);
 int pf_conv_stem3_fwd(const void* X, const void* W, void* Y, int imgs, int H, int Wd, int N, int pad_h, int pad_w, int Ho, int Wo,
diff --git a/pocketflow_amd/csrc/pf_optim.hip b/pocketflow_amd/csrc/pf_optim.hip
--- a/pocketflow_amd/csrc/pf_optim.hip
+++ b/pocketflow_amd/csrc/pf_optim.hip
@@ -10,6 +10,10 @@
   g[0] = __uint_as_float(v.x << 16); g[1] = __uint_as_float(v.x & 0xFFFF0000u);
   g[2] = __uint_as_float(v.y << 16); g[3] = __uint_as_float(v.y & 0xFFFF0000u);
 }
+
+template <typename TG> __device__ __forceinline__ void zero4g(TG* p);
+template <> __device__ __forceinline__ void zero4g<float>(float* p) { *reinterpret_cast<float4*>(p) = make_float4(0.f, 0.f, 0.f, 0.f); }
+template <> __device__ __forceinline__ void zero4g<bf16_t>(bf16_t* p) { *reinterpret_cast<uint2*>(p) = make_uint2(0u, 0u); }
 
 __device__ __forceinline__ float eff_grad(float g, float p, float mask, bool decay, float wd,
                                           float g_scale) {
@@ -18,8 +22,8 @@
   return ge * mask;
 }
 
-template <typename TG, bool MASK>
-__global__ __launch_bounds__(PF_THREADS) void k_adam_flat(float* __restrict__ p, const TG* __restrict__ g,
+template <typename TG, bool MASK, bool ZERO>
+__global__ __launch_bounds__(PF_THREADS) void k_adam_flat(float* __restrict__ p, TG* __restrict__ g,
                                                           float* __restrict__ m, float* __restrict__ v,
                                                           const float* __restrict__ mask, int64_t n,
                                                           int64_t n_decay, float wd, float g_scale,
@@ -32,6 +36,7 @@
     const int64_t e = i << 2;
     float gg[4], mk[4] = {1.f, 1.f, 1.f, 1.f};
     load4g<TG>(g + e, gg);
+    if (ZERO) zero4g<TG>(g + e);
     float4 pp = *reinterpret_cast<float4*>(p + e);
     float4 mm = *reinterpret_cast<float4*>(m + e);
     float4 vv = *reinterpret_cast<float4*>(v + e);
@@ -52,6 +57,7 @@
     for (int64_t e = (nv << 2) + threadIdx.x; e < n; e += PF_THREADS) {
       const float mk = MASK ? mask[e] : 1.0f;
       const float ge = eff_grad(load_one<TG>(g + e), p[e], mk, e < n_decay, wd, g_scale);
+      if (ZERO) store_one<TG>(g + e, 0.f);
       const float mn = m[e] + (ge - m[e]) * omb1;
       const float vn = v[e] + (ge * ge - v[e]) * omb2;
       m[e] = mn; v[e] = vn;
@@ -60,7 +66,7 @@
   }
 }
 
-static int adam_launch(float* p, const void* g, int g_dtype, float* m, float* v,
+static int adam_launch(float* p, void* g, bool zero, int g_dtype, float* m, float* v,
                        const float* mask, int64_t n, int64_t n_decay, float wd, float g_scale,
                        float lr, float beta1, float beta2, float eps, float beta1_power,
                        float beta2_power, const float* hp, void* stream) {
@@ -72,7 +78,8 @@
   const float omb1 = 1.0f - beta1, omb2 = 1.0f - beta2;
   hipStream_t st = (hipStream_t)stream;
   const int grid = pf_grid_for(n, PF_THREADS * 4);
-#define PF_AD(TG, MK) k_adam_flat<TG, MK><<<grid, PF_THREADS, 0, st>>>(p, (const TG*)g, m, v, mask, n, n_decay, wd, g_scale, alpha_t, omb1, omb2, eps, hp)
+#define PF_AD(TG, MK) do { if (zero) k_adam_flat<TG, MK, true><<<grid, PF_THREADS, 0, st>>>(p, (TG*)g, m, v, mask, n, n_decay, wd, g_scale, alpha_t, omb1, omb2, eps, hp); \
+                           else k_adam_flat<TG, MK, false><<<grid, PF_THREADS, 0, st>>>(p, (TG*)g, m, v, mask, n, n_decay, wd, g_scale, alpha_t, omb1, omb2, eps, hp); } while (0)
   if (g_dtype == PF_F32) { if (mask) PF_AD(float, true); else PF_AD(float, false); }
   else if (g_dtype == PF_BF16) { if (mask) PF_AD(bf16_t, true); else PF_AD(bf16_t, false); }
   else return (int)hipErrorInvalidValue;
@@ -85,19 +92,19 @@
                             const float* mask, int64_t n, int64_t n_decay, float wd, float g_scale,
                             float lr, float beta1, float beta2, float eps, float beta1_power,
                             float beta2_power, void* stream) {
-  return adam_launch(p, g, g_dtype, m, v, mask, n, n_decay, wd, g_scale, lr, beta1, beta2, eps, beta1_power, beta2_power, nullptr,
-                     stream);
+  return adam_launch(p, const_cast<void*>(g), false, g_dtype, m, v, mask, n, n_decay, wd, g_scale, lr, beta1, beta2, eps, beta1_power,
+                     beta2_power, nullptr, stream);
 }
 
 extern "C" int pf_adam_flat_dev(float* p, const void* g, int g_dtype, float* m, float* v,
                                 const float* mask, int64_t n, int64_t n_decay, float wd, float g_scale,
                                 const float* hp, float beta1, float beta2, float eps, void* stream) {
   if (hp == nullptr) return (int)hipErrorInvalidValue;
-  return adam_launch(p, g, g_dtype, m, v, mask, n, n_decay, wd, g_scale, 0.f, beta1, beta2, eps, 0.5f, 0.5f, hp, stream);
-}
-
-template <typename TG, bool MASK>
-__global__ __launch_bounds__(PF_THREADS) void k_momentum_flat(float* __restrict__ p, const TG* __restrict__ g,
+  return adam_launch(p, const_cast<void*>(g), false, g_dtype, m, v, mask, n, n_decay, wd, g_scale, 0.f, beta1, beta2, eps, 0.5f, 0.5f, hp, stream);
+}
+
+template <typename TG, bool MASK, bool ZERO>
+__global__ __launch_bounds__(PF_THREADS) void k_momentum_flat(float* __restrict__ p, TG* __restrict__ g,
                                                               float* __restrict__ acc,
                                                               const float* __restrict__ mask, int64_t n,
                                                               int64_t n_decay, float wd, float g_scale,
@@ -109,6 +116,7 @@
     const int64_t e = i << 2;
     float gg[4], mk[4] = {1.f, 1.f, 1.f, 1.f};
     load4g<TG>(g + e, gg);
+    if (ZERO) zero4g<TG>(g + e);
     float4 pp = *reinterpret_cast<float4*>(p + e);
     float4 aa = *reinterpret_cast<float4*>(acc + e);
     if (MASK) { float4 t = *reinterpret_cast<const float4*>(mask + e); mk[0] = t.x; mk[1] = t.y; mk[2] = t.z; mk[3] = t.w; }
@@ -126,6 +134,7 @@
     for (int64_t e = (nv << 2) + threadIdx.x; e < n; e += PF_THREADS) {
       const float mk = MASK ? mask[e] : 1.0f;
       const float ge = eff_grad(load_one<TG>(g + e), p[e], mk, e < n_decay, wd, g_scale);
+      if (ZERO) store_one<TG>(g + e, 0.f);
       const float a = mu * acc[e] + ge;
       acc[e] = a;
       p[e] = p[e] - lr * a;
@@ -133,7 +142,7 @@
   }
 }
 
-static int momentum_launch(float* p, const void* g, int g_dtype, float* acc, const float* mask,
+static int momentum_launch(float* p, void* g, bool zero, int g_dtype, float* acc, const float* mask,
                            int64_t n, int64_t n_decay, float wd, float g_scale, float lr,
                            float momentum, const float* hp, void* stream) {
   if (n <= 0) return 0;
@@ -141,7 +150,8 @@
     return (int)hipErrorInvalidValue;
   hipStream_t st = (hipStream_t)stream;
   const int grid = pf_grid_for(n, PF_THREADS * 4);
-#define PF_MO(TG, MK) k_momentum_flat<TG, MK><<<grid, PF_THREADS, 0, st>>>(p, (const TG*)g, acc, mask, n, n_decay, wd, g_scale, lr, momentum, hp)
+#define PF_MO(TG, MK) do { if (zero) k_momentum_flat<TG, MK, true><<<grid, PF_THREADS, 0, st>>>(p, (TG*)g, acc, mask, n, n_decay, wd, g_scale, lr, momentum, hp); \
+                           else k_momentum_flat<TG, MK, false><<<grid, PF_THREADS, 0, st>>>(p, (TG*)g, acc, mask, n, n_decay, wd, g_scale, lr, momentum, hp); } while (0)
   if (g_dtype == PF_F32) { if (mask) PF_MO(float, true); else PF_MO(float, false); }
   else if (g_dtype == PF_BF16) { if (mask) PF_MO(bf16_t, true); else PF_MO(bf16_t, false); }
   else return (int)hipErrorInvalidValue;
@@ -153,14 +163,40 @@
 extern "C" int pf_momentum_flat(float* p, const void* g, int g_dtype, float* acc, const float* mask,
                                 int64_t n, int64_t n_decay, float wd, float g_scale, float lr,
                                 float momentum, void* stream) {
-  return momentum_launch(p, g, g_dtype, acc, mask, n, n_decay, wd, g_scale, lr, momentum, nullptr, stream);
+  return momentum_launch(p, const_cast<void*>(g), false, g_dtype, acc, mask, n, n_decay, wd, g_scale, lr, momentum, nullptr, stream);
 }
 
 extern "C" int pf_momentum_flat_dev(float* p, const void* g, int g_dtype, float* acc, const float* mask,
                                     int64_t n, int64_t n_decay, float wd, float g_scale, const float* hp,
                                     float momentum, void* stream) {
   if (hp == nullptr) return (int)hipErrorInvalidValue;
-  return momentum_launch(p, g, g_dtype, acc, mask, n, n_decay, wd, g_scale, 0.f, momentum, hp, stream);
+  return momentum_launch(p, const_cast<void*>(g), false, g_dtype, acc, mask, n, n_decay, wd, g_scale, 0.f, momentum, hp, stream);
+}
+
+extern "C" int pf_adam_flat_zero(float* p, void* g, int g_dtype, float* m, float* v, const float* mask, int64_t n,
+                                 int64_t n_decay, float wd, float g_scale, float lr, float beta1, float beta2, float eps,
+                                 float beta1_power, float beta2_power, void* stream) {
+  return adam_launch(p, g, true, g_dtype, m, v, mask, n, n_decay, wd, g_scale, lr, beta1, beta2, eps, beta1_power, beta2_power,
+                     nullptr, stream);
+}
+
+extern "C" int pf_adam_flat_dev_zero(float* p, void* g, int g_dtype, float* m, float* v, const float* mask, int64_t n,
+                                     int64_t n_decay, float wd, float g_scale, const float* hp, float beta1, float beta2,
+                                     float eps, void* stream) {
+  if (hp == nullptr) return (int)hipErrorInvalidValue;
+  return adam_launch(p, g, true, g_dtype, m, v, mask, n, n_decay, wd, g_scale, 0.f, beta1, beta2, eps, 0.5f, 0.5f, hp, stream);
+}
+
+extern "C" int pf_momentum_flat_zero(float* p, void* g, int g_dtype, float* acc, const float* mask, int64_t n,
+                                     int64_t n_decay, float wd, float g_scale, float lr, float momentum, void* stream) {
+  return momentum_launch(p, g, true, g_dtype, acc, mask, n, n_decay, wd, g_scale, lr, momentum, nullptr, stream);
+}
+
+extern "C" int pf_momentum_flat_dev_zero(float* p, void* g, int g_dtype, float* acc, const float* mask, int64_t n,
+                                         int64_t n_decay, float wd, float g_scale, const float* hp, float momentum,
+                                         void* stream) {
+  if (hp == nullptr) return (int)hipErrorInvalidValue;
+  return momentum_launch(p, g, true, g_dtype, acc, mask, n, n_decay, wd, g_scale, 0.f, momentum, hp, stream);
 }
 
 __global__ void k_set_floats(float* __restrict__ dst, float a, float b, float c, float d) {
diff --git a/pocketflow_amd/csrc/pf_stem.hip b/pocketflow_amd/csrc/pf_stem.hip
--- a/pocketflow_amd/csrc/pf_stem.hip
+++ b/pocketflow_amd/csrc/pf_stem.hip
@@ -139,17 +139,20 @@
 
 struct StemWrwArgs {
   const bf16_t* dY;
+  const uint8_t* idx;
   const bf16_t* X;
   float* slabs;
   int imgs, H, Wd, Ho, Wo;
   int strips, n_items;
   int rsb;
   int dy_bytes;
+  int Po, Qo, pad_h;
 };
 
 #define SW_OROWS 2
 #define SW_IROWS (2 * SW_OROWS + 5)
 
+template <bool POOL>
 __global__ __launch_bounds__(ST_THREADS) void k_stem7x7_wrw(StemWrwArgs a) {
   extern __shared__ __attribute__((aligned(16))) unsigned char smem[];
   unsigned char* xs = smem;
@@ -185,10 +188,57 @@
     const int valid_px = ((a.Ho - oy0) < SW_OROWS ? (a.Ho - oy0) : SW_OROWS) * a.Wo;
     const int64_t m_base = ((int64_t)img * a.Ho + oy0) * a.Wo;
     __syncthreads();
-    for (int id = wave; id < steps * 4; id += ST_THREADS / 64) {
-      const int lin = id * 8 + srow;
-      const uint32_t voff = (lin < valid_px) ? (uint32_t)(((m_base + lin) * ST_N + 16 * sb + 8 * sch) * 2) : OOB;
-      ST_BUFFER_LOAD_LDS16(rsY, dys + id * 1024, voff);
+    if constexpr (!POOL) {
+      for (int id = wave; id < steps * 4; id += ST_THREADS / 64) {
+        const int lin = id * 8 + srow;
+        const uint32_t voff = (lin < valid_px) ? (uint32_t)(((m_base + lin) * ST_N + 16 * sb + 8 * sch) * 2) : OOB;
+        ST_BUFFER_LOAD_LDS16(rsY, dys + id * 1024, voff);
+      }
+    } else {
+      for (int t = tid; t < SW_OROWS * a.Qo * 8; t += ST_THREADS) {
+        const int c8 = t & 7, pr = t >> 3;
+        const int orow = pr >= a.Qo ? 1 : 0, bb = pr - orow * a.Qo;
+        const int hi = oy0 + orow;
+        const int u = hi + a.pad_h, wa = u >> 1, du = u & 1;
+        float d[2][2][8];
+        uint2 pk[2][2];
+#pragma unroll
+        for (int i = 0; i < 2; ++i)
+#pragma unroll
+          for (int k = 0; k < 2; ++k) {
+            const int ho = wa - i, wo = bb - k;
+            const bool ok = hi < a.Ho && (unsigned)ho < (unsigned)a.Po && (unsigned)wo < (unsigned)a.Qo;
+            const int hoc = ho < 0 ? 0 : (ho >= a.Po ? a.Po - 1 : ho), woc = wo < 0 ? 0 : wo;
+            const int64_t o = (((int64_t)img * a.Po + hoc) * a.Qo + woc) * ST_N + (c8 << 3);
+            const uint2 pki = *reinterpret_cast<const uint2*>(a.idx + o);
+            load8<bf16_t>(a.dY + o, d[i][k]);
+            pk[i][k] = ok ? pki : make_uint2(0xFFFFFFFFu, 0xFFFFFFFFu);
+          }
+#pragma unroll
+        for (int dv = 0; dv < 2; ++dv) {
+          float gs[8];
+#pragma unroll
+          for (int j = 0; j < 8; ++j) gs[j] = 0.f;
+#pragma unroll
+          for (int i = 0; i < 2; ++i) {
+            const int r = du + 2 * i;
+            if (r > 2) continue;
+#pragma unroll
+            for (int k = 0; k < 2; ++k) {
+              const int s = dv + 2 * k;
+              if (s > 2) continue;
+              const uint32_t want = (uint32_t)(r * 3 + s);
+#pragma unroll
+              for (int j = 0; j < 8; ++j) {
+                const uint32_t tp = ((j < 4 ? pk[i][k].x : pk[i][k].y) >> ((j & 3) * 8)) & 0xFFu;
+                if (tp == want) gs[j] += d[i][k][j];
+              }
+            }
+          }
+          const int lin = orow * a.Wo + 2 * bb + dv;
+          store8<bf16_t>(reinterpret_cast<bf16_t*>(dys + (lin >> 3) * 1024 + (c8 >> 1) * 256 + (lin & 7) * 32 + (c8 & 1) * 16), gs);
+        }
+      }
     }
     for (int row = tid >> 7; row < SW_IROWS; row += 2) {
       const int iy = iy0 + row;
@@ -278,21 +328,253 @@
   return stem_wrw_grid(imgs, H);
 }
 
-extern "C" int pf_conv_stem_wrw(const void* dY, const void* X, void* dW, int dw_dtype, float* workspace, int imgs, int H,
-                                int Wd, void* stream) {
+static int stem_wrw_launch(const void* dY, const void* idx, int pad_h, const void* X, void* dW, int dw_dtype, float* workspace,
+                           int imgs, int H, int Wd, void* stream) {
   const int S = pf_conv_stem_wrw_slabs(imgs, H, Wd);
   if (S <= 0 || workspace == nullptr) return (int)hipErrorInvalidValue;
   if (!pf_aligned16(dY) || (reinterpret_cast<uintptr_t>(X) & 3u)) return (int)hipErrorInvalidValue;
   StemWrwArgs a;
-  a.dY = (const bf16_t*)dY; a.X = (const bf16_t*)X; a.slabs = workspace;
+  a.dY = (const bf16_t*)dY; a.idx = (const uint8_t*)idx; a.X = (const bf16_t*)X; a.slabs = workspace;
   a.imgs = imgs; a.H = H; a.Wd = Wd; a.Ho = H / 2; a.Wo = Wd / 2;
+  a.Po = (a.Ho + 1) / 2; a.Qo = a.Wo / 2; a.pad_h = pad_h;
   a.strips = (a.Ho + SW_OROWS - 1) / SW_OROWS;
   a.n_items = imgs * a.strips;
   a.rsb = (Wd + 8) * 8;
   a.dy_bytes = (int)((int64_t)imgs * a.Ho * a.Wo * ST_N * 2);
   const size_t lds = (size_t)SW_IROWS * a.rsb + (size_t)SW_OROWS * a.Wo * ST_N * 2;
-  if (int e = pf_require_lds(reinterpret_cast<const void*>(&k_stem7x7_wrw), lds)) return e;
-  k_stem7x7_wrw<<<S, ST_THREADS, lds, (hipStream_t)stream>>>(a);
+  if (idx != nullptr) {
+    if (int e = pf_require_lds(reinterpret_cast<const void*>(&k_stem7x7_wrw<true>), lds)) return e;
+    k_stem7x7_wrw<true><<<S, ST_THREADS, lds, (hipStream_t)stream>>>(a);
+  } else {
+    if (int e = pf_require_lds(reinterpret_cast<const void*>(&k_stem7x7_wrw<false>), lds)) return e;
+    k_stem7x7_wrw<false><<<S, ST_THREADS, lds, (hipStream_t)stream>>>(a);
+  }
   PF_LAUNCH_CHECK();
   return pf_wrw_reduce(workspace, S, (int64_t)ST_N * 147, dW, dw_dtype, (hipStream_t)stream);
 }
+
+extern "C" int pf_conv_stem_wrw(const void* dY, const void* X, void* dW, int dw_dtype, float* workspace, int imgs, int H,
+                                int Wd, void* stream) {
+  return stem_wrw_launch(dY, nullptr, 0, X, dW, dw_dtype, workspace, imgs, H, Wd, stream);
+}
+
+extern "C" int pf_conv_stem_pool_wrw(const void* dP, const void* idx, const void* X, void* dW, int dw_dtype, float* workspace,
+                                     int imgs, int H, int Wd, int pad_h, void* stream) {
+  if (idx == nullptr || (reinterpret_cast<uintptr_t>(idx) & 7u) || H <= 0 || pad_h != ((H / 2) & 1))
+    return (int)hipErrorInvalidValue;
+  return stem_wrw_launch(dP, idx, pad_h, X, dW, dw_dtype, workspace, imgs, H, Wd, stream);
+}
+
+
+struct StemPoolArgs {
+  const bf16_t* X;
+  const bf16_t* W;
+  bf16_t* Y;
+  uint8_t* idx;
+  int imgs, H, Wd, Ho, Wo, Po, Qo, pad_h;
+  int P, strips, n_items;
+  int rsb;
+  int ring_bytes;
+};
+
+#define SP_XSLOTS 16
+#define SP_PF 4
+#define SP_PIX(p) ((p) ^ (((p) >> 1) & 1))
+
+__global__ __launch_bounds__(ST_THREADS) void k_stem7x7_pool_fwd(StemPoolArgs a) {
+  extern __shared__ __attribute__((aligned(16))) unsigned char smem[];
+  unsigned char* wl = smem;
+  unsigned char* ring = smem;
+  unsigned char* xs = smem + a.ring_bytes;
+  const int tid = threadIdx.x, lane = tid & 63, wave = __builtin_amdgcn_readfirstlane(tid >> 6);
+  const int l16 = lane & 15, g = lane >> 4;
+
+  for (int ch = tid; ch < ST_N * ST_R * 4; ch += ST_THREADS) {
+    const int q = ch & 3, nr = ch >> 2;
+    const bf16_t* src = a.W + ((int64_t)nr * 7 + 2 * q) * 3;
+    uint32_t v[4];
+    const uint32_t e0 = src[0], e1 = src[1], e2 = src[2];
+    v[0] = e0 | (e1 << 16); v[1] = e2;
+    if (q < 3) {
+      const uint32_t f0 = src[3], f1 = src[4], f2 = src[5];
+      v[2] = f0 | (f1 << 16); v[3] = f2;
+    } else {
+      v[2] = 0u; v[3] = 0u;
+    }
+    *reinterpret_cast<uint4*>(wl + ((int64_t)nr * 32 + q * 8) * 2) = make_uint4(v[0], v[1], v[2], v[3]);
+  }
+  for (int t = tid; t < SP_XSLOTS * 8; t += ST_THREADS) {
+    const int row = t >> 3, h = t & 7;
+    const int pp = h < 3 ? h : a.Wd + h;
+    *reinterpret_cast<uint2*>(xs + (int64_t)row * a.rsb + pp * 8) = make_uint2(0u, 0u);
+  }
+  __syncthreads();
+  bf16x8 wf[4][ST_R];
+#pragma unroll
+  for (int nb = 0; nb < 4; ++nb) {
+    const int n = 16 * (l16 >> 2) + 4 * nb + (l16 & 3);
+#pragma unroll
+    for (int r = 0; r < ST_R; ++r)
+      wf[nb][r] = *reinterpret_cast<const bf16x8*>(wl + ((n * ST_R + r) * 32 + g * 8) * 2);
+  }
+
+  const int pairs = a.Wd >> 1;
+  const int pblocks = a.Wo >> 4;
+  const int row_bytes = a.Wo * (ST_N * 2);
+  const int ptasks = a.Qo * 8;
+  uint32_t pf[SP_PF][3];
+  int pf_row[SP_PF], pf_j[SP_PF];
+#pragma unroll
+  for (int k = 0; k < SP_PF; ++k) {
+    const int q = tid + k * ST_THREADS;
+    pf_row[k] = q / pairs;
+    pf_j[k] = q - pf_row[k] * pairs;
+    pf[k][0] = pf[k][1] = pf[k][2] = 0u;
+  }
+  for (int item = blockIdx.x; item < a.n_items; item += gridDim.x) {
+    const int img = item / a.strips, strip = item - img * a.strips;
+    const int po0 = strip * a.P;
+    const int po1 = (po0 + a.P) < a.Po ? (po0 + a.P) : a.Po;
+    for (int po = po0; po < po1; ++po) {
+      const int c0 = 2 * po - a.pad_h;
+      const bool head = po == po0;
+      const int cfirst = head ? c0 : c0 + 1;
+      if (head) {
+        for (int iy = 2 * c0 - 3 + (tid >> 7); iy < 2 * c0 + 8; iy += 2) {
+          unsigned char* dst = xs + (int64_t)((iy + 3) & (SP_XSLOTS - 1)) * a.rsb + 3 * 8;
+          const bool live = iy >= 0 && iy < a.H;
+          const uint32_t* src = reinterpret_cast<const uint32_t*>(a.X + ((int64_t)img * a.H + (live ? iy : 0)) * a.Wd * 3);
+          for (int j = tid & 127; j < pairs; j += 128) {
+            uint32_t d0 = 0u, d1 = 0u, d2 = 0u;
+            if (live) { d0 = src[3 * j]; d1 = src[3 * j + 1]; d2 = src[3 * j + 2]; }
+            *reinterpret_cast<uint2*>(dst + j * 16) = make_uint2(d0, d1 & 0xFFFFu);
+            *reinterpret_cast<uint2*>(dst + j * 16 + 8) = make_uint2((d1 >> 16) | (d2 << 16), d2 >> 16);
+          }
+        }
+      } else {
+#pragma unroll
+        for (int k = 0; k < SP_PF; ++k) {
+          if (pf_row[k] < 4) {
+            unsigned char* dst = xs + (int64_t)((2 * c0 + 7 + pf_row[k]) & (SP_XSLOTS - 1)) * a.rsb + 3 * 8 + pf_j[k] * 16;
+            *reinterpret_cast<uint2*>(dst) = make_uint2(pf[k][0], pf[k][1] & 0xFFFFu);
+            *reinterpret_cast<uint2*>(dst + 8) = make_uint2((pf[k][1] >> 16) | (pf[k][2] << 16), pf[k][2] >> 16);
+          }
+        }
+      }
+      __syncthreads();
+      if (po + 1 < po1) {
+#pragma unroll
+        for (int k = 0; k < SP_PF; ++k) {
+          const int iy = 2 * c0 + 8 + pf_row[k];
+          const bool live = pf_row[k] < 4 && iy < a.H;
+          const uint32_t* src = reinterpret_cast<const uint32_t*>(a.X + ((int64_t)img * a.H + (live ? iy : 0)) * a.Wd * 3) + 3 * pf_j[k];
+          pf[k][0] = pf[k][1] = pf[k][2] = 0u;
+          if (live) { pf[k][0] = src[0]; pf[k][1] = src[1]; pf[k][2] = src[2]; }
+        }
+      }
+      const int units = (c0 + 3 - cfirst) * pblocks;
+      for (int u = wave; u < units; u += ST_THREADS / 64) {
+        const int orow = u / pblocks, pb = u - orow * pblocks;
+        const int oy = cfirst + orow;
+        if (oy < 0 || oy >= a.Ho) continue;
+        const int ox = pb * 16 + l16;
+        const unsigned char* base = xs + (2 * ox + 2 * g) * 8;
+        f32x4 acc[4];
+#pragma unroll
+        for (int nb = 0; nb < 4; ++nb) acc[nb] = f32x4{0.f, 0.f, 0.f, 0.f};
+#pragma unroll
+        for (int r = 0; r < ST_R; ++r) {
+          const bf16x8 xf = *reinterpret_cast<const bf16x8*>(base + (int64_t)((2 * oy + r) & (SP_XSLOTS - 1)) * a.rsb);
+#pragma unroll
+          for (int nb = 0; nb < 4; ++nb)
+            acc[nb] = __builtin_amdgcn_mfma_f32_16x16x32_bf16(wf[nb][r], xf, acc[nb], 0, 0, 0);
+        }
+        unsigned char* out = ring + (oy % 3) * row_bytes + SP_PIX(ox) * (ST_N * 2);
+        const uint4 lo = make_uint4(pack_bf16x2(acc[0][0], acc[0][1]), pack_bf16x2(acc[0][2], acc[0][3]),
+                                    pack_bf16x2(acc[1][0], acc[1][1]), pack_bf16x2(acc[1][2], acc[1][3]));
+        const uint4 hi = make_uint4(pack_bf16x2(acc[2][0], acc[2][1]), pack_bf16x2(acc[2][2], acc[2][3]),
+                                    pack_bf16x2(acc[3][0], acc[3][1]), pack_bf16x2(acc[3][2], acc[3][3]));
+        *reinterpret_cast<uint4*>(out + (((2 * g) ^ (ox & 7)) << 4)) = lo;
+        *reinterpret_cast<uint4*>(out + (((2 * g + 1) ^ (ox & 7)) << 4)) = hi;
+      }
+      __syncthreads();
+      for (int t = tid; t < ptasks; t += ST_THREADS) {
+        const int cv = t & 7, wo = t >> 3;
+        const int w0 = wo * 2;
+        float best[8];
+        int arg[8];
+#pragma unroll
+        for (int j = 0; j < 8; ++j) { best[j] = -INFINITY; arg[j] = 0; }
+        const bool last_col = w0 + 2 >= a.Wo;
+        const int w2 = last_col ? a.Wo - 1 : w0 + 2;
+#pragma unroll
+        for (int r = 0; r < 3; ++r) {
+          const int hr = c0 + r;
+          if ((unsigned)hr >= (unsigned)a.Ho) continue;
+          const unsigned char* rowp = ring + (hr % 3) * row_bytes;
+          float v[3][8];
+#pragma unroll
+          for (int s = 0; s < 3; ++s) {
+            const int wc = s < 2 ? w0 + s : w2;
+            load8<bf16_t>(reinterpret_cast<const bf16_t*>(rowp + SP_PIX(wc) * (ST_N * 2) + ((cv ^ (wc & 7)) << 4)), v[s]);
+          }
+#pragma unroll
+          for (int j = 0; j < 8; ++j) v[2][j] = last_col ? -INFINITY : v[2][j];
+#pragma unroll
+          for (int s = 0; s < 3; ++s)
+#pragma unroll
+            for (int j = 0; j < 8; ++j)
+              if (v[s][j] > best[j] || v[s][j] != v[s][j]) { best[j] = v[s][j]; arg[j] = r * 3 + s; }
+        }
+        const int64_t o = (((int64_t)img * a.Po + po) * a.Qo + wo) * ST_N + (cv << 3);
+        store8<bf16_t>(a.Y + o, best);
+        if (a.idx != nullptr) {
+          uint2 pk;
+          pk.x = (uint32_t)arg[0] | ((uint32_t)arg[1] << 8) | ((uint32_t)arg[2] << 16) | ((uint32_t)arg[3] << 24);
+          pk.y = (uint32_t)arg[4] | ((uint32_t)arg[5] << 8) | ((uint32_t)arg[6] << 16) | ((uint32_t)arg[7] << 24);
+          *reinterpret_cast<uint2*>(a.idx + o) = pk;
+        }
+      }
+    }
+  }
+}
+
+static bool stem_pool_plan(int imgs, int H, int Wd, StemPoolArgs* a, size_t* lds) {
+  if (!pf_conv_stem_supported(H, Wd, 3, ST_N, 7, 2, 3) || imgs <= 0) return false;
+  a->imgs = imgs; a->H = H; a->Wd = Wd; a->Ho = H / 2; a->Wo = Wd / 2;
+  a->Po = (a->Ho + 1) / 2; a->Qo = a->Wo / 2;
+  a->pad_h = a->Ho & 1;
+  if ((int64_t)imgs * a->Po * a->Qo * ST_N >= (int64_t)1 << 31) return false;
+  a->rsb = (Wd + 8) * 8;
+  const int ring = 3 * a->Wo * ST_N * 2;
+  a->ring_bytes = ring > ST_WL_BYTES ? ring : ST_WL_BYTES;
+  *lds = (size_t)a->ring_bytes + (size_t)SP_XSLOTS * a->rsb;
+  if (*lds > 160 * 1024) return false;
+  int P = (int)(((int64_t)imgs * a->Po) / 512);
+  if (P < 1) P = 1;
+  if (P > a->Po) P = a->Po;
+  a->P = P;
+  a->strips = (a->Po + P - 1) / P;
+  a->n_items = imgs * a->strips;
+  return true;
+}
+
+extern "C" int pf_conv_stem_pool_supported(int imgs, int H, int Wd) {
+  StemPoolArgs a; size_t lds;
+  return stem_pool_plan(imgs, H, Wd, &a, &lds) ? 1 : 0;
+}
+
+extern "C" int pf_conv_stem_pool_fwd(const void* X, const void* W, void* Y, void* idx, int imgs, int H, int Wd, int pad_h,
+                                     void* stream) {
+  StemPoolArgs a; size_t lds;
+  if (!stem_pool_plan(imgs, H, Wd, &a, &lds) || pad_h != a.pad_h) return (int)hipErrorInvalidValue;
+  if (!pf_aligned16(Y) || (idx && (reinterpret_cast<uintptr_t>(idx) & 7u)) || (reinterpret_cast<uintptr_t>(X) & 3u) ||
+      (reinterpret_cast<uintptr_t>(W) & 1u))
+    return (int)hipErrorInvalidValue;
+  a.X = (const bf16_t*)X; a.W = (const bf16_t*)W; a.Y = (bf16_t*)Y; a.idx = (uint8_t*)idx;
+  if (int e = pf_require_lds(reinterpret_cast<const void*>(&k_stem7x7_pool_fwd), lds)) return e;
+  const int grid = a.n_items < 512 ? a.n_items : 512;
+  k_stem7x7_pool_fwd<<<grid, ST_THREADS, lds, (hipStream_t)stream>>>(a);
+  PF_LAUNCH_CHECK();
+  return 0;
+}
diff --git a/pocketflow_amd/graph.py b/pocketflow_amd/graph.py
--- a/pocketflow_amd/graph.py
+++ b/pocketflow_amd/graph.py
@@ -892,6 +892,8 @@
 OWN_CONV2D_WRW_MIN_C = int(os.environ.get('PF_OWN_CONV2D_WRW_MIN_C', '64'))
 OWN_CONV2D_BWD_STRIDED = os.environ.get('PF_OWN_CONV2D_BWD_STRIDED', '1') != '0'
 OWN_CONV2D = os.environ.get('PF_OWN_CONV2D', '1') != '0'
+STEM_POOL = os.environ.get('PF_STEM_POOL', '1') != '0'
+STEM_POOL_WRW = os.environ.get('PF_STEM_POOL_WRW', '1') != '0'
 OWN_STEM = os.environ.get('PF_OWN_STEM', '1') != '0'
 OWN_DEPTHWISE = os.environ.get('PF_OWN_DEPTHWISE', '1') != '0'
 OWN_CONV_IM2COL = os.environ.get('PF_OWN_CONV_IM2COL', '1') != '0'
@@ -1135,21 +1137,65 @@
     dy = _nhwc(dy)
     dx = dw = None
     if ctx.needs_input_grad[1]:
-      B, _, H, Wd = x.shape
-      S = hip.conv_stem_wrw_slabs(B, H, Wd) if OWN_CONV2D_WRW else 0
-      nbytes = float((x.numel() + dy.numel()) * 2)
-      if S > 0:
-        def wrw(dwk, scratch):
-          hip.conv_stem_wrw(dy, x, dwk, scratch((S + 32) * 64 * 147), B, H, Wd)
-        dw = _filter_grad(graph, w, w_var, (dy, x), 'conv_stem_wrw', nbytes, wrw)
-      else:
-        with region('conv_stem_wrw', nbytes):
-          dw = torch.ops.aten.convolution_backward(dy, x, w.detach(), None, [2, 2], [3, 3], [1, 1], False, [0, 0], 1,
-                                                   [False, True, False])[1]
+      dw = _stem_filter_grad(graph, w, w_var, dy, x)
     if ctx.needs_input_grad[0]:
       dx = torch.ops.aten.convolution_backward(dy, x, w.detach(), None, [2, 2], [3, 3], [1, 1], False, [0, 0], 1,
                                                [True, False, False])[0]
     return dx, dw, None, None
+
+
+def _stem_filter_grad(graph, w, w_var, dy, x):
+  B, _, H, Wd = x.shape
+  S = hip.conv_stem_wrw_slabs(B, H, Wd) if OWN_CONV2D_WRW else 0
+  nbytes = float((x.numel() + dy.numel()) * 2)
+  if S > 0:
+    def wrw(dwk, scratch):
+      hip.conv_stem_wrw(dy, x, dwk, scratch((S + 32) * 64 * 147), B, H, Wd)
+    return _filter_grad(graph, w, w_var, (dy, x), 'conv_stem_wrw', nbytes, wrw)
+  with region('conv_stem_wrw', nbytes):
+    return torch.ops.aten.convolution_backward(dy, x, w.detach(), None, [2, 2], [3, 3], [1, 1], False, [0, 0], 1,
+                                               [False, True, False])[1]
+
+
+def _run_stem_pool(x, w, pad_h, want_idx):
+  B, _, H, Wd = x.shape
+  Po, Qo = (H // 2 + 1) // 2, Wd // 4
+  y = torch.empty((B, w.shape[0], Po, Qo), dtype=x.dtype, device=x.device, memory_format=torch.channels_last)
+  idx = torch.empty((B, Po, Qo, w.shape[0]), dtype=torch.uint8, device=x.device) if want_idx else None
+  with region('conv_stem_fwd', float((x.numel() + y.numel()) * 2 + (idx.numel() if want_idx else 0))):
+    hip.conv_stem_pool_fwd(x, w.detach().permute(0, 2, 3, 1), y, idx, B, H, Wd, pad_h)
+  return y, idx
+
+
+class _StemConvPool(torch.autograd.Function):
+
+  @staticmethod
+  def forward(ctx, x, w, graph, w_var, pad_h):
+    y, idx = _run_stem_pool(x, w, pad_h, True)
+    ctx.save_for_backward(x, w, idx)
+    ctx.meta = (graph, w_var, pad_h)
+    return y
+
+  @staticmethod
+  def backward(ctx, dp):
+    x, w, idx = ctx.saved_tensors
+    graph, w_var, pad_h = ctx.meta
+    if not ctx.needs_input_grad[1]:
+      return None, None, None, None, None
+    dp = _nhwc(dp)
+    B, _, H, Wd = x.shape
+    entry = getattr(hip, 'conv_stem_pool_wrw', None) if STEM_POOL_WRW and OWN_CONV2D_WRW else None
+    S = hip.conv_stem_wrw_slabs(B, H, Wd) if entry is not None else 0
+    if S > 0:
+      def wrw(dwk, scratch):
+        entry(dp, idx, x, dwk, scratch((S + 32) * 64 * 147), B, H, Wd, pad_h)
+      dw = _filter_grad(graph, w, w_var, (dp, idx, x), 'conv_stem_wrw', float((x.numel() + dp.numel()) * 2 + idx.numel()), wrw)
+    else:
+      dy = torch.empty((B, w.shape[0], H // 2, Wd // 2), dtype=dp.dtype, device=dp.device, memory_format=torch.channels_last)
+      with region('maxpool_bwd', float((dy.numel() + dp.numel()) * dp.element_size())):
+        hip.maxpool_bwd(dp, idx, dy, B, H // 2, Wd // 2, w.shape[0], 3, 2, pad_h, 0, dp.shape[2], dp.shape[3])
+      dw = _stem_filter_grad(graph, w, w_var, dy, x)
+    return None, dw, None, None, None
 
 
 def _run_stem3(x, w, pads, out_hw):
@@ -1674,6 +1720,26 @@
   return F.max_pool2d(x, k, stride)
 
 
+def stem_conv_pool(conv, x, pool_k: int, pool_stride: int, bn=None) -> torch.Tensor:
+  c2d = getattr(conv, 'conv', conv)
+  fused = getattr(hip, 'conv_stem_pool_fwd', None)
+  query = getattr(hip, 'conv_stem_pool_supported', None)
+  if (STEM_POOL and OWN_POOL and fused is not None and query is not None and bn is None and pool_k == 3 and pool_stride == 2
+      and isinstance(c2d, Conv2D) and not getattr(conv, 'explicit_pad', False) and c2d.graph.taps is None
+      and c2d.kernel.gather_host is None and isinstance(c2d.padding, int) and isinstance(x, torch.Tensor) and x.dim() == 4
+      and not (torch.is_grad_enabled() and x.requires_grad)
+      and own_stem_ok(x, c2d, (c2d.padding, c2d.padding)) and query(x.shape[0], x.shape[2], x.shape[3])):
+    w = c2d.kernel.tensor
+    pad_h = _same_pads(x.shape[2] // 2, 3, 2)[0]
+    if torch.is_grad_enabled() and w.requires_grad:
+      return _StemConvPool.apply(x, w, c2d.graph, c2d.kernel, pad_h)
+    return _run_stem_pool(x, w, pad_h, False)[0]
+  x = conv(x)
+  if bn is not None:
+    x = bn(x)
+  return max_pool_same(x, pool_k, pool_stride) if pool_k else x
+
+
 def fixed_padding(x: torch.Tensor, k: int) -> torch.Tensor:
   pad_total = k - 1
   pb = pad_total // 2
diff --git a/pocketflow_amd/hip.py b/pocketflow_amd/hip.py
--- a/pocketflow_amd/hip.py
+++ b/pocketflow_amd/hip.py
@@ -45,6 +45,8 @@
     'pf_cpr_gather', 'pf_cpr_gram_ws', 'pf_cpr_gram', 'pf_cpr_ista', 'pf_cpr_lstsq_splits', 'pf_cpr_lstsq_step', 'pf_cpr_lstsq_resid',
     'pf_conv_gather_fwd',
     'pf_conv1x1_join_plan', 'pf_conv1x1_bwd_data_join',
+    'pf_conv_stem_pool_supported', 'pf_conv_stem_pool_fwd', 'pf_conv_stem_pool_wrw',
+    'pf_adam_flat_zero', 'pf_momentum_flat_zero', 'pf_adam_flat_dev_zero', 'pf_momentum_flat_dev_zero',
 ]
 
 
@@ -237,6 +239,34 @@
   _check(_lib.pf_momentum_flat_dev(_ptr(p), _ptr(g), c_int(dtype_code(g)), _ptr(acc), _ptr(mask), c_int64(p.numel()),
                                    c_int64(int(n_decay)), c_float(wd), c_float(g_scale), _ptr(hp),
                                    c_float(momentum), _stream()), 'pf_momentum_flat_dev')
+
+
+def adam_flat_zero(p, g, m, v, mask, n_decay: int, wd: float, g_scale: float, lr: float, beta1: float,
+                   beta2: float, eps: float, beta1_power: float, beta2_power: float) -> None:
+  _check(_lib.pf_adam_flat_zero(_ptr(p), _ptr(g), c_int(dtype_code(g)), _ptr(m), _ptr(v), _ptr(mask),
+                                c_int64(p.numel()), c_int64(int(n_decay)), c_float(wd), c_float(g_scale), c_float(lr),
+                                c_float(beta1), c_float(beta2), c_float(eps), c_float(beta1_power),
+                                c_float(beta2_power), _stream()), 'pf_adam_flat_zero')
+
+
+def momentum_flat_zero(p, g, acc, mask, n_decay: int, wd: float, g_scale: float, lr: float,
+                       momentum: float) -> None:
+  _check(_lib.pf_momentum_flat_zero(_ptr(p), _ptr(g), c_int(dtype_code(g)), _ptr(acc), _ptr(mask), c_int64(p.numel()),
+                                    c_int64(int(n_decay)), c_float(wd), c_float(g_scale), c_float(lr),
+                                    c_float(momentum), _stream()), 'pf_momentum_flat_zero')
+
+
+def adam_flat_dev_zero(p, g, m, v, mask, n_decay: int, wd: float, g_scale: float, hp, beta1: float, beta2: float,
+                       eps: float) -> None:
+  _check(_lib.pf_adam_flat_dev_zero(_ptr(p), _ptr(g), c_int(dtype_code(g)), _ptr(m), _ptr(v), _ptr(mask),
+                                    c_int64(p.numel()), c_int64(int(n_decay)), c_float(wd), c_float(g_scale), _ptr(hp),
+                                    c_float(beta1), c_float(beta2), c_float(eps), _stream()), 'pf_adam_flat_dev_zero')
+
+
+def momentum_flat_dev_zero(p, g, acc, mask, n_decay: int, wd: float, g_scale: float, hp, momentum: float) -> None:
+  _check(_lib.pf_momentum_flat_dev_zero(_ptr(p), _ptr(g), c_int(dtype_code(g)), _ptr(acc), _ptr(mask), c_int64(p.numel()),
+                                        c_int64(int(n_decay)), c_float(wd), c_float(g_scale), _ptr(hp),
+                                        c_float(momentum), _stream()), 'pf_momentum_flat_dev_zero')
 
 
 def set_floats(dst, a: float, b: float = 0.0, c: float = 0.0, d: float = 0.0) -> None:
@@ -688,6 +718,22 @@
                                c_int(Wd), _stream()), 'pf_conv_stem_wrw')
 
 
+def conv_stem_pool_supported(imgs: int, H: int, Wd: int) -> bool:
+  return bool(_lib.pf_conv_stem_pool_supported(c_int(imgs), c_int(H), c_int(Wd)))
+
+
+def conv_stem_pool_fwd(X, W, Y, idx, imgs: int, H: int, Wd: int, pad_h: int) -> None:
+  _dev(X)
+  _check(_lib.pf_conv_stem_pool_fwd(_ptr(X), _ptr(W), _ptr(Y), _ptr(idx), c_int(imgs), c_int(H), c_int(Wd), c_int(pad_h), _stream()),
+         'pf_conv_stem_pool_fwd')
+
+
+def conv_stem_pool_wrw(dP, idx, X, dW, workspace, imgs: int, H: int, Wd: int, pad_h: int) -> None:
+  _dev(dP)
+  _check(_lib.pf_conv_stem_pool_wrw(_ptr(dP), _ptr(idx), _ptr(X), _ptr(dW), c_int(dtype_code(dW)), _ptr(workspace), c_int(imgs),
+                                    c_int(H), c_int(Wd), c_int(pad_h), _stream()), 'pf_conv_stem_pool_wrw')
+
+
 def conv_stem3_supported(H: int, Wd: int, C: int, N: int, k: int, stride: int, pad_h: int, pad_w: int, Ho: int, Wo: int) -> bool:
   return bool(_lib.pf_conv_stem3_supported(c_int(H), c_int(Wd), c_int(C), c_int(N), c_int(k), c_int(stride), c_int(pad_h), c_int(pad_w),
                                            c_int(Ho), c_int(Wo)))
diff --git a/pocketflow_amd/optim.py b/pocketflow_amd/optim.py
--- a/pocketflow_amd/optim.py
+++ b/pocketflow_amd/optim.py
@@ -1,5 +1,6 @@
 from __future__ import annotations
 
+import os
 from typing import List, Optional
 
 import numpy as np
@@ -8,6 +9,8 @@
 
 from pocketflow_amd import hip
 from pocketflow_amd.graph import VarStore
+
+OPT_ZERO = os.environ.get('PF_OPT_ZERO', '1') != '0'
 
 
 class FlatOptimizer(object):
@@ -67,45 +70,62 @@
     wd = float(self.weight_decay)
     w_grad = self.w_grad_src if self.w_grad_src is not None else st.w_grad
     o_grad = self.o_grad_src if self.o_grad_src is not None else st.o_grad
+    zero_w, zero_o = self._zeroing_entry(w_grad, st.w_grad, st.w_size), self._zeroing_entry(o_grad, st.o_grad, st.o_size)
     if self.hp is not None:
       if not self.hyper_external:
         self.feed_hyper(lrn_rate)
       if self.kind == 'adam':
         if st.w_size:
-          hip.adam_flat_dev(st.w_master, w_grad, self.slots_w[0], self.slots_w[1], self.w_mask, st.w_decay, wd, self.g_scale,
-                            self.hp, self.beta1, self.beta2, self.epsilon)
+          (zero_w or hip.adam_flat_dev)(st.w_master, w_grad, self.slots_w[0], self.slots_w[1], self.w_mask, st.w_decay, wd, self.g_scale,
+                                        self.hp, self.beta1, self.beta2, self.epsilon)
         if st.o_size:
-          hip.adam_flat_dev(st.o_master, o_grad, self.slots_o[0], self.slots_o[1], self.o_mask, st.o_decay, wd, self.g_scale,
-                            self.hp, self.beta1, self.beta2, self.epsilon)
+          (zero_o or hip.adam_flat_dev)(st.o_master, o_grad, self.slots_o[0], self.slots_o[1], self.o_mask, st.o_decay, wd, self.g_scale,
+                                        self.hp, self.beta1, self.beta2, self.epsilon)
       else:
         if st.w_size:
-          hip.momentum_flat_dev(st.w_master, w_grad, self.slots_w[0], self.w_mask, st.w_decay, wd, self.g_scale, self.hp,
-                                self.momentum)
+          (zero_w or hip.momentum_flat_dev)(st.w_master, w_grad, self.slots_w[0], self.w_mask, st.w_decay, wd, self.g_scale, self.hp,
+                                            self.momentum)
         if st.o_size:
-          hip.momentum_flat_dev(st.o_master, o_grad, self.slots_o[0], self.o_mask, st.o_decay, wd, self.g_scale, self.hp,
-                                self.momentum)
+          (zero_o or hip.momentum_flat_dev)(st.o_master, o_grad, self.slots_o[0], self.o_mask, st.o_decay, wd, self.g_scale, self.hp,
+                                            self.momentum)
       st.w_t_fresh = False
-      st.zero_grad()
+      self._zero_grads(zero_w, zero_o)
       return
     if self.kind == 'adam':
       b1p, b2p = float(self.beta1_power), float(self.beta2_power)
       if st.w_size:
-        hip.adam_flat(st.w_master, w_grad, self.slots_w[0], self.slots_w[1], self.w_mask, st.w_decay, wd,
-                      self.g_scale, lrn_rate, self.beta1, self.beta2, self.epsilon, b1p, b2p)
+        (zero_w or hip.adam_flat)(st.w_master, w_grad, self.slots_w[0], self.slots_w[1], self.w_mask, st.w_decay, wd,
+                                  self.g_scale, lrn_rate, self.beta1, self.beta2, self.epsilon, b1p, b2p)
       if st.o_size:
-        hip.adam_flat(st.o_master, o_grad, self.slots_o[0], self.slots_o[1], self.o_mask, st.o_decay, wd,
-                      self.g_scale, lrn_rate, self.beta1, self.beta2, self.epsilon, b1p, b2p)
+        (zero_o or hip.adam_flat)(st.o_master, o_grad, self.slots_o[0], self.slots_o[1], self.o_mask, st.o_decay, wd,
+                                  self.g_scale, lrn_rate, self.beta1, self.beta2, self.epsilon, b1p, b2p)
       self.beta1_power = np.float32(self.beta1_power * np.float32(self.beta1))
       self.beta2_power = np.float32(self.beta2_power * np.float32(self.beta2))
     else:
       if st.w_size:
-        hip.momentum_flat(st.w_master, w_grad, self.slots_w[0], self.w_mask, st.w_decay, wd, self.g_scale,
-                          lrn_rate, self.momentum)
+        (zero_w or hip.momentum_flat)(st.w_master, w_grad, self.slots_w[0], self.w_mask, st.w_decay, wd, self.g_scale,
+                                      lrn_rate, self.momentum)
       if st.o_size:
-        hip.momentum_flat(st.o_master, o_grad, self.slots_o[0], self.o_mask, st.o_decay, wd, self.g_scale,
-                          lrn_rate, self.momentum)
+        (zero_o or hip.momentum_flat)(st.o_master, o_grad, self.slots_o[0], self.o_mask, st.o_decay, wd, self.g_scale,
+                                      lrn_rate, self.momentum)
     st.w_t_fresh = False
-    st.zero_grad()
+    self._zero_grads(zero_w, zero_o)
+
+  def _zeroing_entry(self, grad: torch.Tensor, own: Optional[torch.Tensor], size: int):
+    if not (OPT_ZERO and size and grad is own):
+      return None
+    name = ('adam_flat' if self.kind == 'adam' else 'momentum_flat') + ('_dev' if self.hp is not None else '') + '_zero'
+    return getattr(hip, name, None)
+
+  def _zero_grads(self, zero_w, zero_o) -> None:
+    st = self.store
+    if zero_w is None and zero_o is None:
+      st.zero_grad()
+    elif st.w_grad is not None:
+      if zero_w is None:
+        st.w_grad.zero_()
+      if zero_o is None:
+        st.o_grad.zero_()
 
 
 class GradReducer(object):
diff --git a/pocketflow_amd/utils/external/resnet_model.py b/pocketflow_amd/utils/external/resnet_model.py
--- a/pocketflow_amd/utils/external/resnet_model.py
+++ b/pocketflow_amd/utils/external/resnet_model.py
@@ -6,7 +6,7 @@
 import torch
 
 from pocketflow_amd.graph import (Activation, BatchNormAct, Conv2D, Dense, Graph, fixed_padding,
-                                  materialize, max_pool_same)
+                                  materialize, stem_conv_pool)
 
 _BATCH_NORM_DECAY = 0.997
 _BATCH_NORM_EPSILON = 1e-5
@@ -150,11 +150,7 @@
   def __call__(self, inputs: torch.Tensor, training: bool) -> torch.Tensor:
     g = self.graph
     g.training = bool(training)
-    x = self.initial_conv(inputs)
-    if self.initial_bn is not None:
-      x = self.initial_bn(x)
-    if self.first_pool_size:
-      x = max_pool_same(x, self.first_pool_size, self.first_pool_stride)
+    x = stem_conv_pool(self.initial_conv, inputs, self.first_pool_size or 0, self.first_pool_stride, self.initial_bn)
     for blk in self.blocks:
       x = blk(x)
     if self.final_bn is not None:
```

Result: no change. 11550 (median of 6 runs) (+0.8%).
